# ipc-sim/IPC

Hardware: AMD Instinct MI355X
Metric: newton_iterations_per_sec (higher is better)
Workload: dtype f64

## Files before the change

### ipc_amd/csrc/hip_ipc.h

```cpp
#pragma once
#include "common.h"
#include "mf_numeric.h"
#include "mf_symbolic.h"
#include "nh_kernels.h"
#include "patch_assembly.h"
#include "hip_contact.h"
#include "hip_halfspace.h"
#include "pcg.h"
#include <map>
#include <memory>
#include <string>

struct ipcgpu_ctx;
typedef int (*ipcgpu_allreduce_fn_t)(void* user, void* buf_dev, long long count, int op);
typedef int (*ipcgpu_allreduce_stream_fn_t)(void* user, void* buf_dev, long long count, int op, void* hipStream);

namespace ipcgpu {

class HipMesh {
public:
    int nV = 0, nT = 0;
    int nElemNodes = 0;
    std::vector<double> V_rest;
    std::vector<int> F;
    std::vector<double> restTriInv;
    std::vector<double> triArea, mass, mu, lam;
    std::vector<int> dbcType;
    std::vector<int> nbPtr, nb;
    double avgEdgeLen = 0, bboxDiag2 = 0, bboxLo[3] = { 0, 0, 0 }, bboxHi[3] = { 0, 0, 0 };
    DevBuf<double> d_x, d_xTilde, d_mass, d_A, d_vol, d_mu, d_lam;
    DevBuf<int> d_dbc;
    DevBuf<int4> d_tet;

    unsigned featuresVersion = 0;
    void computeFeatures(int nV, int nT, const double* Vrest, const int* F, double YM, double PR, double density, hipStream_t s);
    std::vector<char> inMesh;
    void addSurfaceEdges(int nSF, const int* SF_colmajor, int nCE = 0, const int* CE_pairs = nullptr);
    void setCodimNodes(int n, const int* ids, const double* nodeMass, hipStream_t s);
    void meshBBox();
    void uploadDBC(hipStream_t s);
    int energyType = 0;
    double density = 0;
    void setComponentMaterial(int nodeBegin, int nodeEnd, int tetBegin, int tetEnd, double rho, double YM, double PR, hipStream_t s);
    bool isDBCVertex(int v) const { return dbcType[v] != 0; }
    bool isProjectDBCVertex(int v, bool projectDBC) const { return dbcType[v] == 1 || (dbcType[v] == 2 && projectDBC); }
};

class HipLinSysSolver {
public:
    explicit HipLinSysSolver(hipStream_t s);
    ~HipLinSysSolver();
    int numRows = 0;
    std::vector<int> ia, ja;
    DevBuf<int> d_ia, d_ja;
    DevBuf<double> d_a;
    DevBuf<double> hostDelta, hostSetVal;
    DevBuf<unsigned char> hostSetMask;
    std::vector<int> rowBase, rowLen;
    DevBuf<int> d_rowBase, d_rowLen, d_edgeP0;
    int solverType = 0;
    int patternVersion = 0;
    hipStream_t stream;

    void set_pattern(const HipMesh& mesh, int nExtra, const int* extraPairs);
    void set_pattern_csr(int nRows, const int* ia, const int* ja);
    void buildElementMap(const HipMesh& mesh);
    void setZero();
    int findEntry(int row, int col) const;
    void analyze_pattern(const HipMesh* meshForCoords);
    bool factorize();
    bool solve(const double* rhs_dev, double* x_dev);
    bool factorizeSolve(const double* rhs_dev, double* x_dev, bool wait = true);
    bool lastPivotsOk() const;
    bool lastSyncOk_ = true;
    void multiply(const double* x_dev, double* y_dev);
    void precondition_diag(const double* in_dev, double* out_dev);
    double pcgRelTol = 1e-5;
    int pcgMaxIter = 1000;
    int pcgPrecond = 0, pcgMaxFactorAge = 1;
    void setIterative(double relTol, int maxIter, int precond, int maxFactorAge);
    void iterStats(double* out6) const;
    void multiplySym(const double* x_dev, double* y_dev);
    int getNumRows() const { return numRows; }
    int getNumNonzeros() const { return (int)ja.size(); }
    const MfSymbolic& symbolic() const { return sym_; }
    void setShard(int rank, int world, ipcgpu_allreduce_fn_t fn, void* user, ipcgpu_allreduce_stream_fn_t sfn = nullptr, void* streamUser = nullptr)
    {
        num_.setShard(rank, world, fn, user, sfn, streamUser);
        analyzed_ = false;
    }
    void setHooks(ipcgpu_allreduce_fn_t fn, void* user, ipcgpu_allreduce_stream_fn_t sfn, void* streamUser) { num_.setHooks(fn, user, sfn, streamUser); }
    void setExchangeHooks(MfNumeric::ExchangeFn fn, void* user, MfNumeric::ExchangeStreamFn sfn, void* streamUser) { num_.setExchangeHooks(fn, user, sfn, streamUser); }
    bool hasExchangeHook() const { return num_.hasExchangeHook(); }
    int solverWorld() const { return num_.world(); }
    void setBulkTuning(double minMB, int block) { num_.setBulkTuning(minMB, block); }
    void entryDestinations(long long* out) const { num_.entryDestinations(out, ja.size()); }
    void nodeOwners(std::vector<int>& o) const { num_.nodeOwners(o); }
    long long exchangedBytes() const { return num_.exchangedBytes(); }
    long long exchangeCalls() const { return num_.exchangeCalls(); }
    long long sentBytes() const { return num_.sentBytes(); }
    long long receivedBytes() const { return num_.receivedBytes(); }
    double exchangeWaitMs() { return num_.exchangeWaitMs(); }
    void criticalPath(double* out5) const { num_.criticalPath(out5); }
    int analysisVersion = 0;
    double sharedFlopFraction() const { return num_.sharedFlopFraction(); }
    bool analyzed() const { return analyzed_; }
    void invalidateAnalysis() { analyzed_ = false; }

private:
    MfSymbolic sym_;
    MfNumeric num_;
    bool analyzed_ = false;
    std::unique_ptr<struct RocsolverCsrrf> rs_;
    PcgPattern pcgPat_;
    PcgWork pcgWork_;
    int pcgPatVersion_ = -1;
    void ensurePcgPattern();
    int runPcg(const double* rhs_dev, double* x_dev, PcgState& out);
    bool haveFactor_ = false, lastConverged_ = true;
    int factorAge_ = 0;
    long long nFactorizations_ = 0;
    struct {
        int iterations = 0, syncs = 0, factorAge = 0;
        double residual = 0.0;
        bool converged = false;
    } pcgLast_;
    friend struct RocsolverCsrrf;
};

class HipOptimizer {
public:
    HipOptimizer(HipMesh& mesh, HipLinSysSolver& lin, hipStream_t s);
    void init(double dt, bool withGravity);
    void setRelGL2Tol(double relTol);
    void setParameterScaling(bool absolute, double dTolRel, double kappaMinMultiplier);
    void setTwist(int nL, const int* left, int nR, const int* right, double angVel);
    void precompute();
    void beginTimestep();
    bool newtonIter();
    void endTimestep();
    int solveTimestep(int maxIter);

    double computeEnergyVal();
    void computeGradient(bool projectDBC);
    void penaltyGradientAdd(bool projectDBC);
    void computePrecondMtr(bool projectDBC, bool withGradient);
    double dampingStiff = 0.0;
    double ctorDt = 0.025;
    double dHatTargetEps = -1.0;
    double kappaConfig = 0.0;
    void setDamping(double stiff);
    void computeDampingMtr();
    void assembleDampingMtr();
    double dampingEnergy();
    void dampingGradientAdd(bool projectDBC, double* grad_dev);
    void computeSearchDir(bool projectDBC);
    void lineSearch(double& stepSize);
    void stepForward(const double* x0_dev, double alpha);
    double filterStepSize(const double* p_dev, double stepSize);
    double fullCcd(double slackness, double stepSize);
    bool checkInversion();
    ElemView view() const;

    HipMesh& mesh;
    HipLinSysSolver& lin;
    hipStream_t stream;
    double dt = 0.025, dtSq = 0, gravity[3] = { 0, 0, 0 };
    double relGL2Tol = 1e-8, targetGRes = 0;
    int timeIntegration = 0;
    int warmStart = 0;
    double warmStepSize = 0.0;
    double betaNM = 0.25, gammaNM = 0.5;
    DevBuf<double> d_acc, d_dxElastic;
    double elasticCoef() const { return timeIntegration == 1 ? dtSq * betaNM : dtSq; }
    void setTimeIntegration(int type, double beta, double gamma);
    void getKinematics(double* vel, double* acc, double* dxElastic);
    void getDbcState(double* out4) const;
    void saveStatus(const std::string& path);
    void loadStatus(const std::string& path);
    DevBuf<double> d_vel, d_xPrev, d_searchDir, d_gradient, d_minusG, d_x0, d_partial, d_scalar;
    DevBuf<double> d_damp, d_xDamp, d_zeroMass, d_dampDx, d_dampAdx;
    unsigned long long dampPatternVersion = ~0ULL;
    DevBuf<int> d_flag, d_handleIds;
    DevBuf<double> d_handleAng;
    int nHandles = 0;
    struct DbcGroup {
        std::vector<int> ids;
        DevBuf<int> d_ids;
        DevBuf<double> d_pos;
        double lin[3], ang[3], t0, t1;
        bool forceNonzero = false, hasCenter = false;
        double center[3] = { 0, 0, 0 };
        bool hasTargets = false;
        DevBuf<double> d_targets;
        bool isZero() const { return !forceNonzero && lin[0] == 0 && lin[1] == 0 && lin[2] == 0 && ang[0] == 0 && ang[1] == 0 && ang[2] == 0; }
    };
    std::vector<std::unique_ptr<DbcGroup>> dbcGroups;
    struct NbcGroup {
        int n = 0;
        DevBuf<int> d_ids;
        double a[3], t0, t1;
    };
    std::vector<std::unique_ptr<NbcGroup>> nbcGroups;
    void addNeumannBC(int n, const int* ids, const double* accel3, double t0, double t1);
    void neumannGradientAdd(double* grad_dev);
    double neumannEnergy();
    std::vector<int> baseDbcType;
    double stepStartTime = 0, stepEndTime = 0;
    std::vector<int> tpIds, tpIdsOnDevice;
    DevBuf<int> d_tpIds;
    DevBuf<double> d_tpPos, d_tpLam, d_tpStage;
    double dist2Tol = 0, completedStep = 1.0, lastMove = 1.0, rhoDBC = 0.0, CN_MBC = 0.0;
    bool projDBC = true;
    MdbcView mdbc() const { return MdbcView{ (int)tpIds.size(), d_tpIds.p, d_tpPos.p, d_tpLam.p, mesh.d_mass.p }; }
    void buildTargetPositions(bool deferTolerance = false);
    void finishTolerance();
    PinnedBuf<double> h_tpStage;
    bool tolPending = false;
    void initSubProblem();
    double computeCompletedStepSize();
    void dirichletPenaltyUpdate();
    void addDirichletBC(int n, const int* ids, const double* lin3, const double* angRad3, double t0, double t1);
    void setDBCVertices();
    bool dbcGroupMotion();
    double rotCenter[3] = { 0, 0, 0 };
    PinnedBuf<double> h_scalar;
    PinnedBuf<int> h_flag;
    int innerIterAmt = 0, globalIterNum = 0, k = 0;
    double lastEnergyVal = 0, lastStepSize = 0, lastAlphaFeasible = 0;
    double timers[16] = { 0 };
    bool initialised = false;
    int rank = 0, worldSize = 1;
    int tetBegin = 0, tetEnd = 0;
    ipcgpu_allreduce_fn_t allreduce = nullptr;
    ipcgpu_allreduce_stream_fn_t allreduceStream = nullptr;
    void hookReduce(double* dev, long long n, int op);
    bool fastPath() const;
    bool cachedDistValid = false, cachedE0Valid = false;
    double cachedDist = 0, cachedE0 = 0, cachedFilter = 0;
    bool cachedTrialValid = false, cachedTrialInverted = false;
    double cachedTrialE = 0, cachedAlpha = 1.0;
    DevBuf<double> d_aSpec, d_gradSpec;
    bool specAsmValid = false, specAsmOn = true;
    void speculativeAssembly();
    hipEvent_t evAsm0 = nullptr, evAsm1 = nullptr, evTail = nullptr;
    bool evAsmPending = false;
    int evAsmWeight = 1;
    unsigned asmLaunches = 0;
    void resolveEventTimers();
    DevBuf<double> d_contactG;
    void* allreduceUser = nullptr;
    void* allreduceStreamUser = nullptr;
    void reduceSum(double* dev, long long n);
    void reduceMin(double* dev, long long n);
    double readScalar(const double* dev);
    PatchPlan patch;
    int patchVersion = -1;
    void ensurePatchPlan();
    void patchShard(int& pb, int& pe) const;
    bool ownerMode() const;
    void ensureOwnerPlan();
    int ownerPlanPatch = -1, ownerPlanAnalysis = -1;
    int nOwnerPatches = 0;
    DevBuf<int> d_ownerPatches;
    DevBuf<unsigned char> d_need, d_mine;
    long long ownerNeededNodes = 0;
    bool matrixComplete = true;
    void maskAndReduceGradient(double* g);
    void completeMatrix();
    long long commBytes = 0, commCalls = 0;
    HipContact* contact = nullptr;
    bool selfCollision = false;
    double dHatEps = 1.0e-3, dHat = 0, kappa = 0, dTol = 0;
    bool absParameters = false;
    double dTolRel = 1.0e-9, kappaMinMultiplier = 1.0e11;
    double lenScale2() const { return absParameters ? 1.0 : mesh.bboxDiag2; }
    std::vector<std::pair<int, int>> curExtra;
    std::vector<std::array<int, 4>> closeID;
    std::vector<double> closeVal;
    int lastCCDPair[2] = { 0, 0 }, nFullCCD = 0, nPatternChanges = 0, dbcIncomplete = 0;
    unsigned long long coverSets = ~0ull;
    int coverPattern = -1;
    bool coverAnswer = false;
    double patternPad = -1.0;
    double lookahead() const { return patternPad >= 0.0 ? patternPad : (mesh.nV > 150000 ? 2.25 : 4.0); }
    std::vector<std::unique_ptr<HipHalfSpace>> planes;
    std::vector<std::pair<int, int>> closeHS;
    std::vector<double> closeHSVal;
    double selfFric = 0.0, epsV = 1.0e-3, fricDHat0 = 0, fricDHat = -1.0;
    double epsVTarget = -1.0, fricDHatTarget = 0;
    int fricIterAmt = 1, fricIterI = 0;
    bool fricLoopForced = false;
    bool solveFric() const;
    void updateFrictionLag();
    bool nextSubproblem();
    bool ipOn() const { return selfCollision || !planes.empty(); }
    size_t nConstraints() const;
    int addHalfSpace(HipContact* c, const double* origin3, const double* normal3, double dHatEps);
    bool anyIntersection();
    void elasticInertiaGradient(bool projectDBC, bool finish = true);
    void barrierGradientAdd(bool projectDBC, double kappa, bool activeOnly, double* grad_dev, int part = 0);
    void enableSelfCollision(HipContact* c, double dHatEps);
    void setVelocity(const double* vel3nV);
    void computeConstraintSets();
    double kappaFloor() const;
    void initKappa();
    void postLineSearch();
    bool isIntersected();
    void computeXTilta();
};

}

struct ipcgpu_ctx {
    int device = 0;
    hipStream_t stream = nullptr;
    std::unique_ptr<ipcgpu::HipMesh> mesh;
    std::unique_ptr<ipcgpu::HipLinSysSolver> lin;
    std::unique_ptr<ipcgpu::HipOptimizer> opt;
    std::unique_ptr<ipcgpu::HipContact> contact;
    int rank = 0, worldSize = 1;
    void* exchange = nullptr;
    void* exchangeUser = nullptr;
    void* exchangeStream = nullptr;
    void* exchangeStreamUser = nullptr;
};
```

### ipc_amd/csrc/hip_linsys.hip

```cpp
#include "hip_ipc.h"
#include <rocsolver/rocsolver.h>
#include <algorithm>
#include <cmath>
#include <thread>
#include <cstdlib>

namespace ipcgpu {

struct RocsolverCsrrf {
    rocblas_handle handle = nullptr;
    rocsolver_rfinfo info = nullptr;
    int n = 0, nnzA = 0, nnzT = 0;
    DevBuf<int> ptrA, indA, ptrT, indT, pivQ, trans, flag;
    DevBuf<double> valA, valT, B;
    bool analyzed = false;
    ~RocsolverCsrrf()
    {
        if (info) rocsolver_destroy_rfinfo(info);
        if (handle) rocblas_destroy_handle(handle);
    }
};

namespace {
__global__ void k_gather(int n, const int* __restrict__ map, const double* __restrict__ src, double* __restrict__ dst)
// ... 128 lines not shown
    analyzed_ = false;
    ++patternVersion;
}

void HipLinSysSolver::set_pattern_csr(int nRows, const int* ia_, const int* ja_)
{
    if (nRows <= 0 || nRows % 3) throw ArgError("set_pattern_csr: rows must be a positive multiple of 3");
    numRows = nRows;
    ia.assign(ia_, ia_ + nRows + 1);
    ja.assign(ja_, ja_ + ia[nRows]);
    for (int r = 0; r < nRows; ++r) {
        if (ia[r + 1] <= ia[r] || ja[ia[r]] != r) throw ArgError("set_pattern_csr: every row must start with its diagonal (upper CSR)");
        for (int k = ia[r] + 1; k < ia[r + 1]; ++k)
            if (ja[k] <= ja[k - 1] || ja[k] >= nRows) throw ArgError("set_pattern_csr: columns must be ascending and in range");
    }
    d_ia.upload(ia, stream);
    d_ja.upload(ja, stream);
    d_a.alloc(ja.size());
    d_a.zero(stream);
    rowBase.clear();
    rowLen.clear();
    HIP_CHECK(hipStreamSynchronize(stream));
    analyzed_ = false;
    ++patternVersion;
}

void HipLinSysSolver::setZero() { d_a.zeroN(ja.size(), stream); }

int HipLinSysSolver::findEntry(int row, int col) const
{
    if (row < 0 || row >= numRows) return -1;
    const int* b = ja.data() + ia[row];
    const int* e = ja.data() + ia[row + 1];
    const int* it = std::lower_bound(b, e, col);
    if (it == e || *it != col) return -1;
    return int(it - ja.data());
}

void HipLinSysSolver::analyze_pattern(const HipMesh* mesh)
{
    if (!numRows) throw StateError("analyze_pattern before set_pattern");
    std::vector<double> coords;
    const double* cptr = nullptr;
    if (mesh && 3 * mesh->nV == numRows) {
        coords.resize(3 * (size_t)mesh->nV);
        for (int v = 0; v < mesh->nV; ++v)
            for (int c = 0; c < 3; ++c) coords[3 * (size_t)v + c] = mesh->V_rest[v + (size_t)mesh->nV * c];
        cptr = coords.data();
    }
    if (solverType == 2) {
        if (num_.world() > 1) throw StateError("the iterative solver is not sharded");
        ensurePcgPattern();
        haveFactor_ = false;
        factorAge_ = 0;
        lastConverged_ = true;
        if (pcgPrecond == 0) {
            analyzed_ = true;
            return;
        }
    }
    const int leaf = 12;
    mf_analyze(numRows, ia.data(), ja.data(), cptr, leaf, sym_, false);
    ++analysisVersion;
    if (solverType == 0 || solverType == 2) {
        num_.setup(sym_, stream, d_ia.p, d_ja.p, (long long)ja.size());
    }
    else {
        rs_.reset(new RocsolverCsrrf);
        RocsolverCsrrf& R = *rs_;
        R.n = numRows;
        if (rocblas_create_handle(&R.handle) != rocblas_status_success) throw HipError("rocblas_create_handle");
        rocblas_set_stream(R.handle, stream);
        if (rocsolver_create_rfinfo(&R.info, R.handle) != rocblas_status_success) throw HipError("rocsolver_create_rfinfo");
        if (rocsolver_set_rfinfo_mode(R.info, rocsolver_rfinfo_mode_cholesky) != rocblas_status_success)
            throw HipError("rocsolver_set_rfinfo_mode");
        const int nnz = (int)ja.size();
        std::vector<int> ptr(numRows + 1, 0), ind(nnz), tr(nnz);
        for (int k = 0; k < nnz; ++k) ptr[ja[k] + 1]++;
        for (int r = 0; r < numRows; ++r) ptr[r + 1] += ptr[r];
        std::vector<int> pos(ptr.begin(), ptr.end() - 1);
        for (int r = 0; r < numRows; ++r)
            for (int k = ia[r]; k < ia[r + 1]; ++k) {
                const int c = ja[k];
                ind[pos[c]] = r;
                tr[pos[c]] = k;
                pos[c]++;
            }
        std::vector<int> pT, iT, q;
        mf_L_pattern_csr(sym_, pT, iT, q);
        R.nnzA = nnz;
        R.nnzT = (int)iT.size();
        R.ptrA.upload(ptr, stream);
        R.indA.upload(ind, stream);
        R.trans.upload(tr, stream);
        R.valA.alloc(nnz);
        R.ptrT.upload(pT, stream);
        R.indT.upload(iT, stream);
        R.pivQ.upload(q, stream);
        R.valT.alloc(iT.size());
        R.B.alloc(numRows);
        R.B.zero(stream);
        R.flag.alloc(1);
        hipLaunchKernelGGL(k_set_diag_one, dim3((numRows + 255) / 256), dim3(256), 0, stream, numRows, R.ptrT.p, R.indT.p, R.valT.p);
        hipLaunchKernelGGL(k_set_diag_one, dim3((numRows + 255) / 256), dim3(256), 0, stream, numRows, R.ptrA.p, R.indA.p, R.valA.p);
        const rocblas_status st = rocsolver_dcsrrf_analysis(R.handle, R.n, 1, R.nnzA, R.ptrA.p, R.indA.p, R.valA.p, R.nnzT, R.ptrT.p, R.indT.p, R.valT.p,
            nullptr, R.pivQ.p, R.B.p, R.n, R.info);
        if (st != rocblas_status_success) throw HipError("rocsolver_dcsrrf_analysis failed (rocblas_status " + std::to_string((int)st) + ")");
        HIP_CHECK(hipStreamSynchronize(stream));
        R.analyzed = true;
    }
    analyzed_ = true;
}

bool HipLinSysSolver::factorize()
{
    if (!analyzed_) throw StateError("factorize before analyze_pattern");
    if (solverType == 0) return num_.factorize(d_a.p);
    if (solverType == 2) {
        if (pcgPrecond == 0) {
            pcgWork_.ensure(numRows);
            pcgWork_.flag.zero(stream);
            launch_pcg_invert_blocks(pcgPat_, d_a.p, pcgWork_.flag.p, stream);
            int f = 0;
            pcgWork_.flag.download(&f, 1, stream);
            return f == 0;
        }
        if (haveFactor_ && lastConverged_ && factorAge_ + 1 < pcgMaxFactorAge) {
            ++factorAge_;
            return true;
        }
        ++nFactorizations_;
        haveFactor_ = num_.factorize(d_a.p);
        factorAge_ = 0;
        lastConverged_ = true;
        return haveFactor_;
    }
    RocsolverCsrrf& R = *rs_;
    hipLaunchKernelGGL(k_gather, dim3((R.nnzA + 255) / 256), dim3(256), 0, stream, R.nnzA, R.trans.p, d_a.p, R.valA.p);
    rocblas_status st = rocsolver_dcsrrf_refactchol(R.handle, R.n, R.nnzA, R.ptrA.p, R.indA.p, R.valA.p, R.nnzT, R.ptrT.p, R.indT.p,
        R.valT.p, R.pivQ.p, R.info);
    if (st != rocblas_status_success) {
        HIP_CHECK(hipStreamSynchronize(stream));
        return false;
    }
    R.flag.zero(stream);
    hipLaunchKernelGGL(k_check_diag, dim3((R.n + 255) / 256), dim3(256), 0, stream, R.n, R.ptrT.p, R.valT.p, R.pivQ.p, d_ia.p, d_a.p,
        R.flag.p);
    int f = 0;
    HIP_CHECK(hipMemcpyAsync(&f, R.flag.p, sizeof(int), hipMemcpyDeviceToHost, stream));
    HIP_CHECK(hipStreamSynchronize(stream));
    return f == 0;
}

bool HipLinSysSolver::factorizeSolve(const double* rhs_dev, double* x_dev, bool wait)
{
    if (!analyzed_) throw StateError("factorize before analyze_pattern");
    lastSyncOk_ = true;
    if (solverType == 0) return lastSyncOk_ = num_.factorizeSolve(d_a.p, rhs_dev, x_dev, wait);
    const bool ok = factorize();
    return lastSyncOk_ = ok && solve(rhs_dev, x_dev);
}
bool HipLinSysSolver::lastPivotsOk() const { return lastSyncOk_ && (solverType != 0 || num_.lastPivotsOk()); }

bool HipLinSysSolver::solve(const double* rhs_dev, double* x_dev)
{
    if (!analyzed_) throw StateError("solve before analyze_pattern");
    if (solverType == 0) {
        num_.solve(rhs_dev, x_dev);
        return true;
    }
    if (solverType == 2) {
        const bool jacobi = pcgPrecond == 0;
        if (!jacobi && !haveFactor_) throw StateError("solve before factorize");
        pcgLast_ = {};
        pcgLast_.factorAge = jacobi ? 0 : factorAge_;
        PcgState st;
        int status = runPcg(rhs_dev, x_dev, st);
        pcgLast_.iterations = st.iter;
        if (status == PCG_MAXITER && !jacobi && factorAge_ > 0) {
            ++nFactorizations_;
            haveFactor_ = num_.factorize(d_a.p);
            factorAge_ = 0;
            if (!haveFactor_) return false;
            pcgLast_.factorAge = 0;
            status = runPcg(rhs_dev, x_dev, st);
            pcgLast_.iterations += st.iter;
        }
        pcgLast_.residual = st.bb > 0.0 ? std::sqrt(st.trueRes2 / st.bb) : 0.0;
        pcgLast_.converged = status == PCG_CONVERGED && st.trueRes2 <= st.tol2;
        lastConverged_ = pcgLast_.converged;
        return status != PCG_BREAKDOWN;
    }
    RocsolverCsrrf& R = *rs_;
    HIP_CHECK(hipMemcpyAsync(x_dev, rhs_dev, sizeof(double) * R.n, hipMemcpyDeviceToDevice, stream));
    if (rocsolver_dcsrrf_solve(R.handle, R.n, 1, R.nnzT, R.ptrT.p, R.indT.p, R.valT.p, nullptr, R.pivQ.p, x_dev, R.n, R.info)
        != rocblas_status_success)
        throw HipError("rocsolver_dcsrrf_solve failed");
    return true;
}

void HipLinSysSolver::setIterative(double relTol, int maxIter, int precond, int maxFactorAge)
{
    if (!(relTol > 0.0) || maxIter < 1 || (precond != 0 && precond != 1) || maxFactorAge < 1)
        throw ArgError("set_iterative: rel_tol > 0, max_iter >= 1, precond 0 | 1, max_factor_age >= 1");
    if (precond != pcgPrecond && solverType == 2) analyzed_ = false;
    pcgRelTol = relTol;
    pcgMaxIter = maxIter;
    pcgPrecond = precond;
    pcgMaxFactorAge = maxFactorAge;
}

void HipLinSysSolver::iterStats(double* o) const
{
    o[0] = pcgLast_.iterations;
    o[1] = pcgLast_.residual;
    o[2] = pcgLast_.converged ? 1.0 : 0.0;
    o[3] = (double)nFactorizations_;
    o[4] = pcgLast_.factorAge;
    o[5] = pcgLast_.syncs;
}

void HipLinSysSolver::ensurePcgPattern()
{
    if (!numRows) throw StateError("no pattern");
    if (pcgPatVersion_ == patternVersion) return;
    pcgPat_.build(numRows, ia, ja, rowBase, rowLen, stream);
    pcgPatVersion_ = patternVersion;
}

void HipLinSysSolver::multiplySym(const double* x_dev, double* y_dev)
{
    ensurePcgPattern();
    launch_pcg_symv(pcgPat_, d_ia.p, d_ja.p, d_rowBase.p, d_rowLen.p, d_a.p, x_dev, nullptr, nullptr, 0, y_dev, nullptr, nullptr, 0, stream);
}

int HipLinSysSolver::runPcg(const double* rhs_dev, double* x_dev, PcgState& out)
{
    const bool jacobi = pcgPrecond == 0;
    PcgWork& W = pcgWork_;
    W.ensure(numRows);
    const int gAp = pcg_symv_grid(pcgPat_);
    double* p[2] = { W.p0.p, W.p1.p };
    int cur = 0, first = 1, restarts = 0, batch = jacobi ? 16 : 1;
    auto precondition = [&](int firstRz) {
        if (jacobi) return;
        num_.solve(W.r.p, W.z.p);
        launch_pcg_rz(numRows, W.r.p, W.z.p, W, firstRz, stream);
    };
    launch_pcg_begin(pcgPat_, jacobi, false, rhs_dev, nullptr, x_dev, W, pcgRelTol, pcgMaxIter, stream);
    precondition(1);
    for (;;) {
        for (int i = 0; i < batch; ++i) {
            launch_pcg_symv(pcgPat_, d_ia.p, d_ja.p, d_rowBase.p, d_rowLen.p, d_a.p, W.z.p, p[cur], p[1 - cur], first, W.Ap.p, W.partial.p, W.state.p, 1, stream);
            cur = 1 - cur;
            first = 0;
            launch_pcg_alpha(W, gAp, stream);
            launch_pcg_update(pcgPat_, jacobi, p[cur], W.Ap.p, x_dev, W, stream);
        }
        launch_pcg_symv(pcgPat_, d_ia.p, d_ja.p, d_rowBase.p, d_rowLen.p, d_a.p, x_dev, nullptr, nullptr, 0, W.Ap.p, nullptr, W.state.p, 2, stream);
        launch_pcg_residual(numRows, rhs_dev, W.Ap.p, W, stream);
        launch_pcg_publish(W, stream);
        HIP_CHECK(hipStreamSynchronize(stream));
        ++pcgLast_.syncs;
        out = *W.hState.p;
        if (out.done == PCG_RUNNING) {
            precondition(0);
            if (jacobi) batch = std::min(64, 2 * batch);
            continue;
        }
        if (out.done == PCG_CONVERGED && out.trueRes2 > out.tol2 && restarts < 3 && out.iter < out.maxIter) {
            ++restarts;
            launch_pcg_begin(pcgPat_, jacobi, true, rhs_dev, W.Ap.p, x_dev, W, pcgRelTol, pcgMaxIter, stream);
            first = 1;
            precondition(1);
            continue;
        }
        return out.done;
    }
}

void HipLinSysSolver::multiply(const double* x_dev, double* y_dev)
{
    launch_csr_symv(numRows, d_ia.p, d_ja.p, d_a.p, x_dev, y_dev, stream);
}
void HipLinSysSolver::precondition_diag(const double* in_dev, double* out_dev)
{
    launch_precond_diag(numRows, d_ia.p, d_a.p, in_dev, out_dev, stream);
}

}
```

### ipc_amd/csrc/hip_optimizer.cpp

```cpp
#include "hip_ipc.h"
#include <fstream>
#include <iomanip>
#include <limits>
#include <sstream>
#include <algorithm>
#include <chrono>
#include <thread>
#include <iterator>
#include <cmath>
#include <cstring>

#ifndef BEGIN_BATCHED
#define BEGIN_BATCHED 1
#endif

namespace ipcgpu {


namespace {
struct Tic {
    double& acc;
    hipStream_t s;
    std::chrono::high_resolution_clock::time_point t0;
    bool nosync = false;
    Tic(double& a, hipStream_t st) : acc(a), s(st), t0(std::chrono::high_resolution_clock::now()) {}
    ~Tic()
    {
        if (!nosync) (void)hipStreamSynchronize(s);
        acc += std::chrono::duration<double>(std::chrono::high_resolution_clock::now() - t0).count();
    }
};
}

HipOptimizer::HipOptimizer(HipMesh& m, HipLinSysSolver& l, hipStream_t s) : mesh(m), lin(l), stream(s) {}

ElemView HipOptimizer::view() const
{
    ElemView v;
    v.nV = mesh.nV;
    v.nT = mesh.nT;
    v.tetBegin = tetBegin;
    v.tetEnd = tetEnd;
    v.energyType = mesh.energyType;
    v.x = mesh.d_x.p;
    v.xTilde = mesh.d_xTilde.p;
    v.mass = mesh.d_mass.p;
    v.dbc = mesh.d_dbc.p;
    v.tet = mesh.d_tet.p;
    v.A = mesh.d_A.p;
    v.vol = mesh.d_vol.p;
    v.mu = mesh.d_mu.p;
    v.lam = mesh.d_lam.p;
    v.rowBase = lin.d_rowBase.p;
    v.rowLen = lin.d_rowLen.p;
    v.edgeP0 = lin.d_edgeP0.p;
    return v;
}

void HipOptimizer::init(double dt_, bool withGravity)
{
    dt = dt_;
    dtSq = dt * dt;
    gravity[0] = gravity[2] = 0.0;
    gravity[1] = withGravity ? -9.80665 : 0.0;
    const size_t n3 = 3 * (size_t)mesh.nV;
    d_vel.alloc(n3);
    d_vel.zero(stream);
    d_acc.alloc(n3);
    d_acc.zero(stream);
    d_dxElastic.alloc(n3);
    d_dxElastic.zero(stream);
    d_xPrev.alloc(n3);
    d_searchDir.alloc(n3);
    d_searchDir.zero(stream);
    d_gradient.alloc(n3);
    d_gradient.zero(stream);
    d_minusG.alloc(n3);
    d_x0.alloc(n3);
    d_partial.alloc((size_t)std::max(mesh.nT, mesh.nV) / 256 + 2);
    d_scalar.alloc(8);
    d_flag.alloc(2);
    h_scalar.alloc(8);
    h_flag.alloc(2);
    HIP_CHECK(hipMemcpyAsync(d_xPrev.p, mesh.d_x.p, n3 * sizeof(double), hipMemcpyDeviceToDevice, stream));
    HIP_CHECK(hipMemcpyAsync(mesh.d_xTilde.p, mesh.d_x.p, n3 * sizeof(double), hipMemcpyDeviceToDevice, stream));
    for (int c = 0; c < 3; ++c) rotCenter[c] = 0.5 * (mesh.bboxLo[c] + mesh.bboxHi[c]);
    tetBegin = (int)((long long)mesh.nT * rank / worldSize);
    tetEnd = (int)((long long)mesh.nT * (rank + 1) / worldSize);
    setRelGL2Tol(1.0e-2);
    innerIterAmt = globalIterNum = k = 0;
    std::memset(timers, 0, sizeof(timers));
    initialised = true;
    HIP_CHECK(hipStreamSynchronize(stream));
    computeXTilta();
}

void HipOptimizer::setRelGL2Tol(double relTol)
{
    relGL2Tol = relTol * relTol;
    targetGRes = std::sqrt(relGL2Tol * (absParameters ? 1.0 : mesh.bboxDiag2 * dtSq));
    CN_MBC = std::sqrt(1.0e-4 * mesh.bboxDiag2 * (ctorDt * ctorDt));
}

void HipOptimizer::setParameterScaling(bool absolute, double dTolRel_, double kappaMinMultiplier_)
{
    if (!(dTolRel_ > 0.0) || !(kappaMinMultiplier_ > 0.0)) throw ArgError("set_parameter_scaling: dTolRel and kappaMinMultiplier must be positive");
    absParameters = absolute;
    dTolRel = dTolRel_;
    kappaMinMultiplier = kappaMinMultiplier_;
    targetGRes = std::sqrt(relGL2Tol * (absParameters ? 1.0 : mesh.bboxDiag2 * dtSq));
    if (ipOn()) {
        dHat = dHatEps * dHatEps * lenScale2();
        dTol = dTolRel * dTolRel * lenScale2();
    }
}

void HipOptimizer::setTwist(int nL, const int* left, int nR, const int* right, double angVel)
{
    std::vector<int> ids;
    std::vector<double> ang;
    for (int i = 0; i < nL; ++i) {
        mesh.dbcType[left[i]] = 2;
        ids.push_back(left[i]);
        ang.push_back(-angVel * dt);
    }
    for (int i = 0; i < nR; ++i) {
        mesh.dbcType[right[i]] = 2;
        ids.push_back(right[i]);
        ang.push_back(angVel * dt);
    }
    nHandles = (int)ids.size();
    if (nHandles) {
        d_handleIds.upload(ids, stream);
        d_handleAng.upload(ang, stream);
    }
    mesh.uploadDBC(stream);
    if (initialised) computeXTilta();
}

void HipOptimizer::addNeumannBC(int n, const int* ids, const double* accel3, double t0, double t1)
{
    std::unique_ptr<NbcGroup> g(new NbcGroup);
    g->n = n;
    g->d_ids.upload(ids, (size_t)n, stream);
    for (int c = 0; c < 3; ++c) g->a[c] = accel3[c];
    g->t0 = t0;
    g->t1 = t1;
    HIP_CHECK(hipStreamSynchronize(stream));
    nbcGroups.push_back(std::move(g));
}

void HipOptimizer::neumannGradientAdd(double* grad_dev)
{
    for (const auto& g : nbcGroups) {
        if (stepStartTime < g->t0 || stepStartTime >= g->t1) continue;
        const double c[3] = { dtSq * g->a[0], dtSq * g->a[1], dtSq * g->a[2] };
        launch_nbc_gradient(g->n, g->d_ids.p, mesh.d_dbc.p, mesh.d_mass.p, c, grad_dev, stream);
    }
}

double HipOptimizer::neumannEnergy()
{
    double E = 0.0;
    for (const auto& g : nbcGroups) {
        if (stepStartTime < g->t0 || stepStartTime >= g->t1) continue;
        const double c[3] = { dtSq * g->a[0], dtSq * g->a[1], dtSq * g->a[2] };
        launch_nbc_energy(g->n, g->d_ids.p, mesh.d_dbc.p, mesh.d_mass.p, mesh.d_x.p, c, d_scalar.p + 5, stream);
        E -= readScalar(d_scalar.p + 5);
    }
    return E;
}

void HipOptimizer::addDirichletBC(int n, const int* ids, const double* lin3, const double* angRad3, double t0, double t1)
{
    std::unique_ptr<DbcGroup> g(new DbcGroup);
    g->ids.assign(ids, ids + n);
    for (int c = 0; c < 3; ++c) {
        g->lin[c] = lin3[c];
        g->ang[c] = angRad3[c];
    }
    g->t0 = t0;
    g->t1 = t1;
    g->d_ids.upload(g->ids, stream);
    g->d_pos.alloc(3 * (size_t)n);
    if (baseDbcType.empty()) baseDbcType = mesh.dbcType;
    dbcGroups.push_back(std::move(g));
    setDBCVertices();
    if (initialised) computeXTilta();
}

void HipOptimizer::setDBCVertices()
{
    if (dbcGroups.empty()) return;
    if (baseDbcType.empty()) baseDbcType = mesh.dbcType;
    std::vector<int> t = baseDbcType;
    for (const auto& g : dbcGroups) {
        if (stepStartTime < g->t0 || stepStartTime >= g->t1) continue;
        const int type = g->isZero() ? 1 : 2;
        for (int v : g->ids) t[v] = std::max(t[v], type);
    }
    if (t != mesh.dbcType) {
        mesh.dbcType = t;
        mesh.uploadDBC(stream);
    }
}

bool HipOptimizer::dbcGroupMotion()
{
    bool any = false;
    std::vector<double> pos;
    for (const auto& g : dbcGroups) {
        if (stepStartTime < g->t0 || stepStartTime >= g->t1 || g->ids.empty() || g->hasTargets) continue;
        const int n = (int)g->ids.size();
        launch_gather3(n, g->d_ids.p, mesh.d_x.p, g->d_pos.p, stream);
        pos.resize(3 * (size_t)n);
        g->d_pos.download(pos.data(), pos.size(), stream);
        HIP_CHECK(hipStreamSynchronize(stream));
        DbcMotion m;
        double lo[3] = { pos[0], pos[1], pos[2] }, hi[3] = { pos[0], pos[1], pos[2] };
        for (int i = 0; i < n; ++i)
            for (int c = 0; c < 3; ++c) {
                lo[c] = std::min(lo[c], pos[3 * (size_t)i + c]);
                hi[c] = std::max(hi[c], pos[3 * (size_t)i + c]);
            }
        for (int c = 0; c < 3; ++c) {
            m.c[c] = g->hasCenter ? g->center[c] : (lo[c] + hi[c]) / 2;
            m.linDt[c] = g->lin[c] * dt;
        }
        const double ax = g->ang[0] * dt, ay = g->ang[1] * dt, az = g->ang[2] * dt;
        const double cx = std::cos(ax), sx = std::sin(ax), cy = std::cos(ay), sy = std::sin(ay), cz = std::cos(az), sz = std::sin(az);
        const double Rx[9] = { 1, 0, 0, 0, cx, -sx, 0, sx, cx }, Ry[9] = { cy, 0, sy, 0, 1, 0, -sy, 0, cy }, Rz[9] = { cz, -sz, 0, sz, cz, 0, 0, 0, 1 };
        double T[9];
// ... 21 lines not shown
    if (worldSize > 1) hookReduce(dev, n, 1);
}
void HipOptimizer::hookReduce(double* dev, long long n, int op)
{
    commBytes += 8 * n;
    commCalls++;
    if (allreduceStream) {
        if (allreduceStream(allreduceStreamUser, dev, n, op, (void*)stream) != 0) throw HipError("all-reduce hook failed");
        return;
    }
    if (!allreduce) throw StateError("sharded context without an all-reduce hook");
    HIP_CHECK(hipStreamSynchronize(stream));
    if (allreduce(allreduceUser, dev, n, op) != 0) throw HipError("all-reduce hook failed");
}
double HipOptimizer::readScalar(const double* dev)
{
    launch_publish(dev, h_scalar.dev, 2, stream);
    HIP_CHECK(hipStreamSynchronize(stream));
    return h_scalar.p[0];
}

double HipOptimizer::computeEnergyVal()
{
    launch_energy(view(), elasticCoef(), true, rank == 0, d_partial.p, (int)d_partial.n, d_scalar.p, stream);
    reduceSum(d_scalar.p, 1);
    const bool contactQueued = selfCollision && contact->energyEnqueue(mesh.d_x.p, dHat, kappa, d_partial, d_scalar.p + 4, d_scalar.p, h_scalar.dev, 10);
    if (!(contactQueued && contact->publishedByEnergy())) launch_publish(d_scalar.p, h_scalar.dev, 10, stream);
    HIP_CHECK(hipStreamSynchronize(stream));
    double E = h_scalar.p[0];
    const double Econtact = contactQueued ? h_scalar.p[4] : 0.0;
    if (!nbcGroups.empty()) E += neumannEnergy();
    for (auto& h : planes) E += h->energy(mesh.d_x.p, dHat, kappa);
    if (selfCollision) E += Econtact;
    if (fricDHat > 0.0) {
        for (auto& h : planes)
            if (h->friction > 0.0) E += h->frictionEnergy(mesh.d_x.p, d_xPrev.p, fricDHat);
        if (selfCollision && selfFric > 0.0) E += contact->frictionEnergy(mesh.d_x.p, d_xPrev.p, fricDHat, selfFric, d_partial, d_scalar.p + 4);
    }
    if (dampingStiff > 0.0) E += dampingEnergy();
    if (rhoDBC && !tpIds.empty()) {
        launch_mdbc_reduce(mdbc(), mesh.d_x.p, rhoDBC, 0, d_scalar.p + 5, stream);
        E += readScalar(d_scalar.p + 5);
    }
    return E;
}

void HipOptimizer::setDamping(double stiff)
{
    dampingStiff = stiff > 0.0 ? stiff : 0.0;
}
void HipOptimizer::computeDampingMtr()
{
    if (!(dampingStiff > 0.0)) return;
    d_xDamp.ensure(3 * (size_t)mesh.nV);
    HIP_CHECK(hipMemcpyAsync(d_xDamp.p, mesh.d_x.p, sizeof(double) * 3 * (size_t)mesh.nV, hipMemcpyDeviceToDevice, stream));
    assembleDampingMtr();
}
void HipOptimizer::assembleDampingMtr()
{
    const size_t nnz = lin.ja.size();
    d_damp.ensure(nnz);
    if (d_zeroMass.n < (size_t)mesh.nV) {
        d_zeroMass.alloc(mesh.nV);
        d_zeroMass.zero(stream);
    }
    ensurePatchPlan();
    int pb, pe;
    patchShard(pb, pe);
    ElemView v = view();
    v.x = d_xDamp.p;
    v.xTilde = d_xDamp.p;
    v.mass = d_zeroMass.p;
    if (worldSize > 1) HIP_CHECK(hipMemsetAsync(d_damp.p, 0, sizeof(double) * nnz, stream));
    launch_assemble_patches(v, patch, pb, pe, dampingStiff / dt, 1, nullptr, d_damp.p, stream);
    if (worldSize > 1) reduceSum(d_damp.p, (long long)nnz);
    launch_damp_clear_diag(mesh.nV, mesh.d_dbc.p, lin.d_ia.p, d_damp.p, stream);
    dampPatternVersion = lin.patternVersion;
}
double HipOptimizer::dampingEnergy()
{
    if (dampPatternVersion != lin.patternVersion) assembleDampingMtr();
    const int n3 = 3 * mesh.nV;
    d_dampDx.ensure(n3);
    d_dampAdx.ensure(n3);
    launch_damp_dx(mesh.nV, mesh.d_dbc.p, 0, 1, mesh.d_x.p, d_xPrev.p, d_dampDx.p, stream);
    launch_csr_symv(n3, lin.d_ia.p, lin.d_ja.p, d_damp.p, d_dampDx.p, d_dampAdx.p, stream);
    launch_dot_scaled(n3, d_dampDx.p, d_dampAdx.p, 0.5, d_scalar.p + 6, stream);
    return readScalar(d_scalar.p + 6);
}
void HipOptimizer::dampingGradientAdd(bool projectDBC, double* grad_dev)
{
    if (dampPatternVersion != lin.patternVersion) assembleDampingMtr();
    const int n3 = 3 * mesh.nV;
    d_dampDx.ensure(n3);
    d_dampAdx.ensure(n3);
    launch_damp_dx(mesh.nV, mesh.d_dbc.p, 1, projectDBC ? 1 : 0, mesh.d_x.p, d_xPrev.p, d_dampDx.p, stream);
    launch_csr_symv(n3, lin.d_ia.p, lin.d_ja.p, d_damp.p, d_dampDx.p, d_dampAdx.p, stream);
    launch_axpy(n3, 1.0, d_dampAdx.p, grad_dev, stream);
}

bool HipOptimizer::solveFric() const
{
    if (fricLoopForced) return true;
    if (selfCollision && selfFric > 0.0) return true;
    for (const auto& h : planes)
        if (h->friction > 0.0) return true;
    return false;
}

void HipOptimizer::updateFrictionLag()
{
    if (!solveFric()) return;
    for (auto& h : planes)
        if (h->friction > 0.0) h->lagUpdate(mesh.d_x.p, dHat, kappa);
    if (selfCollision && selfFric > 0.0) contact->frictionLagUpdate(mesh.d_x.p, dHat, kappa);
}

bool HipOptimizer::nextSubproblem()
{
    specAsmValid = false;
    if (!ipOn()) return false;
    const double dHatTarget = dHatTargetEps > 0.0 ? dHatTargetEps * dHatTargetEps * lenScale2() : dHat;
    const bool fric = solveFric(), homotopy = dHat > dHatTarget;
    if (!fric && !homotopy) return false;
    fricIterI++;
    if (fric) updateFrictionLag();
    if (!nConstraints()) return false;
    bool updateDHat = true;
    {
        double dMax = 0.0, dMin = 1.0e300;
        std::vector<double> d;
        for (auto& h : planes) {
            h->evalDist2(h->set, mesh.d_x.p, d);
            for (size_t i = 0; i < h->set.size(); ++i) {
                dMax = std::max(dMax, d[i]);
                dMin = std::min(dMin, d[i]);
            }
        }
        if (selfCollision) {
            std::vector<std::array<int, 4>> ids;
            contact->closeStencils(mesh.d_x.p, 1.0e300, ids, d);
            for (size_t i = 0; i < ids.size(); ++i) {
                dMax = std::max(dMax, d[i]);
                dMin = std::min(dMin, d[i]);
            }
        }
        if (dMax < dHatTarget) updateDHat = false;
        else if (dMin < dTol) return false;
    }
    bool updateFricDHat = fric;
    if (fric && fricDHat <= fricDHatTarget) {
        computePrecondMtr(true, true);
        computeSearchDir(true);
        launch_fill(d_scalar.p + 3, 1, 0.0, stream);
        launch_max_abs(3 * mesh.nV, d_searchDir.p, d_scalar.p + 3, stream);
        if (readScalar(d_scalar.p + 3) < targetGRes) updateFricDHat = false;
        if (fricIterAmt > 0 && fricIterI >= fricIterAmt) updateFricDHat = false;
    }
    if (!updateDHat && !updateFricDHat) return false;
    if (updateDHat) {
        dHat = std::max(0.5 * dHat, dHatTarget);
        computeConstraintSets();
        initKappa();
    }
    if (updateFricDHat && fricDHat > 0.0) fricDHat = std::max(0.5 * fricDHat, fricDHatTarget);
    initSubProblem();
    closeID.clear();
    closeVal.clear();
    closeHS.clear();
    closeHSVal.clear();
    k = 0;
    return true;
}

size_t HipOptimizer::nConstraints() const
{
    size_t n = selfCollision ? (size_t)contact->nActive() : 0;
    for (const auto& h : planes) n += h->set.size();
    return n;
}

int HipOptimizer::addHalfSpace(HipContact* c, const double* origin3, const double* normal3, double eps)
{
    if (!c || !c->surfaceSet) throw StateError("opt_add_half_space before set_surface");
    if ((selfCollision || !planes.empty()) && eps != dHatEps) throw ArgError("all collision objects of a context share one dHat (Config.cpp:41-45): got a different dHatEps");
    contact = c;
    planes.emplace_back(new HipHalfSpace(stream, origin3, normal3));
    dHatEps = eps;
    dHat = eps * eps * lenScale2();
    dTol = dTolRel * dTolRel * lenScale2();
    return (int)planes.size() - 1;
}

bool HipOptimizer::anyIntersection()
{
    for (auto& h : planes)
        if (h->intersected(mesh.nV, mesh.d_x.p, mesh.d_dbc.p)) return true;
    return selfCollision && isIntersected();
}

void HipOptimizer::enableSelfCollision(HipContact* c, double eps)
{
    if (!c || !c->surfaceSet) throw StateError("opt_enable_self_collision before set_surface");
    if (!planes.empty() && eps != dHatEps) throw ArgError("all collision objects of a context share one dHat (Config.cpp:41-45): got a different dHatEps");
    contact = c;
    selfCollision = true;
    dHatEps = eps;
    dHat = eps * eps * lenScale2();
    dTol = dTolRel * dTolRel * lenScale2();
}

void HipOptimizer::computeXTilta()
{
    const size_t n3 = 3 * (size_t)mesh.nV;
    std::vector<double> xp(n3), vel(n3), xt(n3), acc(n3, 0.0);
    d_xPrev.download(xp.data(), n3, stream);
    d_vel.download(vel.data(), n3, stream);
    d_acc.download(acc.data(), n3, stream);
    for (int v = 0; v < mesh.nV; ++v)
        for (int c = 0; c < 3; ++c) {
            const size_t i = 3 * (size_t)v + c;
            if (mesh.isDBCVertex(v)) xt[i] = xp[i];
            else if (timeIntegration == 1) xt[i] = xp[i] + (vel[i] * dt + betaNM * (dtSq * gravity[c]) + (0.5 - betaNM) * (dtSq * acc[i]));
            else xt[i] = xp[i] + (vel[i] * dt + dtSq * gravity[c]);
        }
    mesh.d_xTilde.upload(xt, stream);
    HIP_CHECK(hipStreamSynchronize(stream));
}

void HipOptimizer::setTimeIntegration(int type, double beta, double gamma)
{
    timeIntegration = type;
    betaNM = beta;
    gammaNM = gamma;
    computeXTilta();
}

void HipOptimizer::getDbcState(double* out4) const
{
    out4[0] = completedStep;
    out4[1] = rhoDBC;
    out4[2] = projDBC ? 1.0 : 0.0;
    out4[3] = (double)tpIds.size();
}

void HipOptimizer::getKinematics(double* vel, double* acc, double* dxElastic)
{
    const size_t n3 = 3 * (size_t)mesh.nV;
    if (vel) d_vel.download(vel, n3, stream);
    if (acc) d_acc.download(acc, n3, stream);
    if (dxElastic) d_dxElastic.download(dxElastic, n3, stream);
    HIP_CHECK(hipStreamSynchronize(stream));
}

void HipOptimizer::saveStatus(const std::string& path)
{
    const size_t n3 = 3 * (size_t)mesh.nV;
    std::vector<double> x(n3), vel(n3), acc(n3), dx(n3);
    mesh.d_x.download(x.data(), n3, stream);
    getKinematics(vel.data(), acc.data(), dx.data());
    std::ofstream out(path, std::ios::out);
    if (!out.is_open()) throw StateError("unable to create status file " + path);
    out << std::setprecision(std::numeric_limits<long double>::digits10 + 2);
    out << "timestep " << globalIterNum << "\n\n";
    auto rows = [&](const char* name, const std::vector<double>& a) {
        out << name << " " << mesh.nV << " 3\n";
        for (int v = 0; v < mesh.nV; ++v) out << a[3 * (size_t)v] << " " << a[3 * (size_t)v + 1] << " " << a[3 * (size_t)v + 2] << "\n";
    };
    rows("position", x);
    out << "\n";
    out << "velocity " << n3 << "\n";
    for (size_t i = 0; i < n3; ++i) out << vel[i] << "\n";
    out << "\n";
    rows("acceleration", acc);
    out << "\n";
    rows("dx_Elastic", dx);
    if (!out.good()) throw StateError("write error on status file " + path);
}

void HipOptimizer::loadStatus(const std::string& path)
{
    specAsmValid = false;
    std::ifstream in(path);
    if (!in.is_open()) throw StateError("unable to open status file " + path);
    const size_t n3 = 3 * (size_t)mesh.nV;
    std::vector<double> x(n3), vel(n3, 0.0), acc(n3, 0.0), dx(n3, 0.0);
    mesh.d_x.download(x.data(), n3, stream);
    HIP_CHECK(hipStreamSynchronize(stream));
    auto readRows = [&](std::stringstream& ss, std::vector<double>& dst, bool zeroFirst) {
        int rowsIn = 0, dimIn = 0;
        ss >> rowsIn >> dimIn;
        if (rowsIn < 0 || rowsIn > mesh.nV || dimIn != 3) throw StateError("status file does not match the mesh");
        if (ss.fail()) throw StateError("malformed section header in status file " + path);
        if (zeroFirst) std::fill(dst.begin(), dst.end(), 0.0);
        for (int v = 0; v < rowsIn; ++v) in >> dst[3 * (size_t)v] >> dst[3 * (size_t)v + 1] >> dst[3 * (size_t)v + 2];
        if (in.fail()) throw StateError("truncated or malformed section in status file " + path);
    };
    std::string line;
    while (std::getline(in, line)) {
        std::stringstream ss(line);
        std::string token;
        ss >> token;
        if (token == "timestep") ss >> globalIterNum;
        else if (token == "position") readRows(ss, x, false);
        else if (token == "velocity") {
            long long n = 0;
            ss >> n;
// ... 276 lines not shown
        const auto now = std::chrono::steady_clock::now();
        fprintf(stderr, "pattern change: %-34s %.2f ms\n", what, std::chrono::duration<double, std::milli>(now - tLap).count());
        tLap = now;
    };
    const bool coverCached = selfCollision && coverSets == contact->setsVersion && coverPattern == lin.patternVersion;
    if (selfCollision && (frictionPairs || !(coverCached ? coverAnswer : contact->patternCovers(lin)))) {
        lap("coverage check");
        std::vector<std::pair<int, int>> extra, fresh;
        const bool liveOnHost = frictionPairs || lookahead() < 1.0;
        if (liveOnHost) {
            if (contact->nActive() + contact->nPara()) contact->connectivity(extra);
            if (fricDHat > 0.0 && selfFric > 0.0) contact->frictionConnectivity(extra);
            for (const auto& e : extra) {
                const int* b = mesh.nb.data() + mesh.nbPtr[e.first];
                const int* en = mesh.nb.data() + mesh.nbPtr[e.first + 1];
                if (!std::binary_search(b, en, e.second)) fresh.push_back(e);
            }
            std::sort(fresh.begin(), fresh.end());
            fresh.erase(std::unique(fresh.begin(), fresh.end()), fresh.end());
        }
        lap("connectivity of the live sets");
        if (!liveOnHost || !std::includes(curExtra.begin(), curExtra.end(), fresh.begin(), fresh.end())) {
            std::vector<std::pair<int, int>> padded = fresh;
            const double pad = lookahead();
            if (pad >= 1.0) {
                std::vector<std::pair<int, int>> ahead;
                if (pad > 1.0) contact->buildConstraintSet(mesh, mesh.d_x.p, mesh.d_dbc.p, pad * dHat);
                contact->candidateConnectivitySorted(ahead);
                if (pad > 1.0) contact->buildConstraintSet(mesh, mesh.d_x.p, mesh.d_dbc.p, dHat);
                std::vector<std::pair<int, int>> aheadNew;
                aheadNew.reserve(ahead.size());
                for (const auto& e : ahead) {
                    const int* b = mesh.nb.data() + mesh.nbPtr[e.first];
                    const int* en = mesh.nb.data() + mesh.nbPtr[e.first + 1];
                    if (!std::binary_search(b, en, e.second)) aheadNew.push_back(e);
                }
                padded.clear();
                std::set_union(fresh.begin(), fresh.end(), aheadNew.begin(), aheadNew.end(), std::back_inserter(padded));
            }
            lap("look-ahead sets + connectivity");
            std::vector<std::pair<int, int>> merged;
            std::set_union(curExtra.begin(), curExtra.end(), padded.begin(), padded.end(), std::back_inserter(merged));
            if (merged.size() > 3 * padded.size() + 4096) merged = padded;
            curExtra.swap(merged);
            nPatternChanges++;
            std::vector<int> flat;
            flat.reserve(2 * curExtra.size());
            for (const auto& e : curExtra) {
                flat.push_back(e.first);
                flat.push_back(e.second);
            }
            lap("union + flatten");
            {
                Tic t(timers[1], stream);
                lin.set_pattern(mesh, (int)curExtra.size(), flat.data());
            }
            lap("set_pattern");
            {
                int dev = 0;
                HIP_CHECK(hipGetDevice(&dev));
                std::exception_ptr planErr;
                std::thread planThread([&] {
                    try {
                        HIP_CHECK(hipSetDevice(dev));
                        ensurePatchPlan();
                    }
                    catch (...) {
                        planErr = std::current_exception();
                    }
                });
                std::exception_ptr anaErr;
                try {
                    Tic t(timers[2], stream);
                    lin.analyze_pattern(&mesh);
                }
                catch (...) {
                    anaErr = std::current_exception();
                }
                planThread.join();
                if (anaErr) std::rethrow_exception(anaErr);
                if (planErr) std::rethrow_exception(planErr);
            }
            lap("analyze_pattern + patch plan");
        }
    }
    const bool planStale = !(patchVersion == lin.patternVersion && patch.valid);
    ensurePatchPlan();
    if (planStale) lap("patch plan");
    if (ownerMode()) {
        ensureOwnerPlan();
        lin.setZero();
        if (withGradient) d_gradient.zero(stream);
        launch_assemble_patches(view(), patch, 0, nOwnerPatches, elasticCoef(), projectDBC, withGradient ? d_gradient.p : nullptr, lin.d_a.p, stream,
            d_ownerPatches.p);
        matrixComplete = false;
        if (ipOn() && selfCollision) contact->hessianAdd(mesh.d_x.p, mesh.d_dbc.p, lin, dHat, kappa, projectDBC, lin.d_a.p, d_need.p, true);
        if (withGradient) {
            if (ipOn()) barrierGradientAdd(projectDBC, kappa, false, d_gradient.p, 1);
            maskAndReduceGradient(d_gradient.p);
            neumannGradientAdd(d_gradient.p);
            if (ipOn()) barrierGradientAdd(projectDBC, kappa, false, d_gradient.p, 2);
        }
        if (ipOn()) {
            for (auto& h : planes)
                h->hessianAdd(mesh.d_x.p, mesh.d_dbc.p, lin.d_rowBase.p, lin.d_rowLen.p, dHat, kappa, projectDBC, lin.d_a.p);
            if (fricDHat > 0.0) {
                for (auto& h : planes)
                    if (h->friction > 0.0)
                        h->frictionHessianAdd(mesh.d_x.p, d_xPrev.p, mesh.d_dbc.p, lin.d_rowBase.p, lin.d_rowLen.p, fricDHat, projectDBC, lin.d_a.p);
                if (selfCollision && selfFric > 0.0)
                    contact->frictionHessianAdd(mesh.d_x.p, d_xPrev.p, mesh.d_dbc.p, lin, fricDHat, selfFric, projectDBC, lin.d_a.p);
            }
        }
        if (withGradient) penaltyGradientAdd(projectDBC);
        if (!projectDBC && rhoDBC && !tpIds.empty()) launch_mdbc_hessian(mdbc(), lin.d_ia.p, rhoDBC, lin.d_a.p, stream);
        return;
    }
    int pb, pe;
    patchShard(pb, pe);
    if (worldSize > 1) {
        lin.setZero();
        if (withGradient) d_gradient.zero(stream);
    }
    launch_assemble_patches(view(), patch, pb, pe, elasticCoef(), projectDBC, withGradient ? d_gradient.p : nullptr,
        lin.d_a.p, stream);
    matrixComplete = true;
    const bool contactSharded = false;
    if (worldSize > 1) {
        reduceSum(lin.d_a.p, (long long)lin.ja.size());
        if (withGradient) reduceSum(d_gradient.p, 3LL * mesh.nV);
    }
    if (withGradient) neumannGradientAdd(d_gradient.p);
    if (ipOn()) {
        if (withGradient) barrierGradientAdd(projectDBC, kappa, false, d_gradient.p);
        for (auto& h : planes)
            h->hessianAdd(mesh.d_x.p, mesh.d_dbc.p, lin.d_rowBase.p, lin.d_rowLen.p, dHat, kappa, projectDBC, lin.d_a.p);
        if (selfCollision && !contactSharded) contact->hessianAdd(mesh.d_x.p, mesh.d_dbc.p, lin, dHat, kappa, projectDBC, lin.d_a.p, nullptr, true);
        if (fricDHat > 0.0) {
            for (auto& h : planes)
                if (h->friction > 0.0)
                    h->frictionHessianAdd(mesh.d_x.p, d_xPrev.p, mesh.d_dbc.p, lin.d_rowBase.p, lin.d_rowLen.p, fricDHat, projectDBC, lin.d_a.p);
            if (selfCollision && selfFric > 0.0)
                contact->frictionHessianAdd(mesh.d_x.p, d_xPrev.p, mesh.d_dbc.p, lin, fricDHat, selfFric, projectDBC, lin.d_a.p);
        }
    }
    if (dampingStiff > 0.0) {
        if (dampPatternVersion != lin.patternVersion) assembleDampingMtr();
        launch_axpy((long long)lin.ja.size(), 1.0, d_damp.p, lin.d_a.p, stream);
    }
    if (withGradient) penaltyGradientAdd(projectDBC);
    if (!projectDBC && rhoDBC && !tpIds.empty()) launch_mdbc_hessian(mdbc(), lin.d_ia.p, rhoDBC, lin.d_a.p, stream);
}

bool HipOptimizer::checkInversion()
{
    if (mesh.energyType == 1) return true;
    d_flag.zero(stream);
    launch_check_inversion(view(), d_flag.p, stream);
    launch_publish(d_flag.p, h_flag.dev, 1, stream);
    HIP_CHECK(hipStreamSynchronize(stream));
    int f = h_flag.p[0];
    if (worldSize > 1) {
        h_scalar.p[1] = (double)f;
        HIP_CHECK(hipMemcpyAsync(d_scalar.p + 1, h_scalar.p + 1, sizeof(double), hipMemcpyHostToDevice, stream));
        reduceSum(d_scalar.p + 1, 1);
        f = readScalar(d_scalar.p + 1) != 0.0;
    }
    return f == 0;
}

double HipOptimizer::fullCcd(double slackness, double stepSize)
{
    if (contact->ccdMode == 1) {
        int arg3[3];
        const double a = contact->ccdFullReference(mesh, mesh.d_x.p, d_searchDir.p, mesh.d_dbc.p, slackness, stepSize, nullptr, arg3, nullptr);
        lastCCDPair[0] = arg3[1];
        lastCCDPair[1] = arg3[2];
        return a;
    }
    return contact->ccdFull(mesh, mesh.d_x.p, d_searchDir.p, mesh.d_dbc.p, slackness, stepSize, lastCCDPair, nullptr);
}

double HipOptimizer::filterStepSize(const double* p_dev, double stepSize)
{
    if (mesh.energyType == 1) return stepSize;
    launch_fill(d_scalar.p + 2, 1, 1e20, stream);
    launch_inversion_step(view(), p_dev, 0.2, stepSize, d_scalar.p + 2, stream);
    reduceMin(d_scalar.p + 2, 1);
    const double t = readScalar(d_scalar.p + 2);
    if (t > 0.0 && t < stepSize) stepSize = t;
    return stepSize;
}

void HipOptimizer::stepForward(const double* x0_dev, double alpha)
{
    launch_step_forward(3 * mesh.nV, x0_dev, d_searchDir.p, alpha, mesh.d_x.p, stream);
}

#ifndef ASM_TIME_EVERY
#define ASM_TIME_EVERY 8
#endif
void HipOptimizer::speculativeAssembly()
{
    specAsmValid = false;
    if (!specAsmOn || !fastPath() || !projDBC || lin.rowBase.empty()) return;
    ensurePatchPlan();
    d_aSpec.alloc(lin.d_a.n);
    d_gradSpec.alloc(d_gradient.n);
    const bool timeIt = (asmLaunches++ % ASM_TIME_EVERY) == 0;
    if (timeIt) {
        resolveEventTimers();
        HIP_CHECK(hipEventRecord(evAsm0, stream));
    }
    launch_assemble_patches(view(), patch, 0, patch.nPatches, elasticCoef(), 1, d_gradSpec.p, d_aSpec.p, stream);
    if (timeIt) {
        HIP_CHECK(hipEventRecord(evAsm1, stream));
        evAsmPending = true;
        evAsmWeight = ASM_TIME_EVERY;
    }
    specAsmValid = true;
}

void HipOptimizer::computeSearchDir(bool projectDBC)
{
    (void)projectDBC;
    bool ok;
    const bool twoCalls = false;
    launch_negate(3 * mesh.nV, d_gradient.p, d_minusG.p, stream);
    const bool noSpec = false;
    cachedTrialValid = false;
    cachedDistValid = false;
    if (fastPath() && !twoCalls && !noSpec) {
        Tic t(timers[3], stream);
        const size_t bytes = 3 * (size_t)mesh.nV * sizeof(double);
        if (lin.factorizeSolve(d_minusG.p, d_searchDir.p, false)) {
            launch_iter_reset(d_scalar.p, d_flag.p, stream);
            launch_max_abs(3 * mesh.nV, d_searchDir.p, d_scalar.p + 3, stream);
            if (mesh.energyType != 1) launch_inversion_step(view(), d_searchDir.p, 0.2, 1.0, d_scalar.p + 2, stream);
            launch_energy(view(), elasticCoef(), true, true, d_partial.p, (int)d_partial.n, d_scalar.p, stream);
            launch_trial_step_fused(3 * mesh.nV, mesh.d_x.p, d_x0.p, d_searchDir.p, d_scalar.p + 2, mesh.energyType != 1, d_scalar.p + 6, stream);
            if (mesh.energyType != 1) launch_check_inversion(view(), d_flag.p, stream);
            launch_energy(view(), elasticCoef(), true, true, d_partial.p, (int)d_partial.n, d_scalar.p + 1, stream);
            launch_publish2(d_flag.p, h_flag.dev, 1, d_scalar.p, h_scalar.dev, 14, stream);
            if (!evTail) HIP_CHECK(hipEventCreateWithFlags(&evTail, hipEventDisableTiming));
            HIP_CHECK(hipEventRecord(evTail, stream));
            speculativeAssembly();
            HIP_CHECK(hipEventSynchronize(evTail));
            t.nosync = specAsmValid;
            if (lin.lastPivotsOk()) {
                cachedE0 = h_scalar.p[0];
                cachedTrialE = h_scalar.p[1];
                cachedFilter = h_scalar.p[2];
                cachedDist = h_scalar.p[3];
                cachedAlpha = h_scalar.p[6];
                cachedTrialInverted = mesh.energyType != 1 && h_flag.p[0] != 0;
                cachedDistValid = cachedE0Valid = cachedTrialValid = true;
                return;
            }
            HIP_CHECK(hipMemcpyAsync(mesh.d_x.p, d_x0.p, bytes, hipMemcpyDeviceToDevice, stream));
            specAsmValid = false;
            t.nosync = false;
        }
        ok = false;
    }
    else {
        Tic t(timers[3], stream);
        if (twoCalls) ok = lin.factorize();
        else if (worldSize == 1) {
            ok = lin.factorizeSolve(d_minusG.p, d_searchDir.p, false);
            if (ok) {
                launch_fill(d_scalar.p + 3, 1, 0.0, stream);
                launch_max_abs(3 * mesh.nV, d_searchDir.p, d_scalar.p + 3, stream);
                launch_publish(d_scalar.p + 3, h_scalar.dev + 3, 2, stream);
                HIP_CHECK(hipStreamSynchronize(stream));
                ok = lin.lastPivotsOk();
                if (ok) {
                    cachedDist = h_scalar.p[3];
                    cachedDistValid = true;
                }
            }
        }
        else ok = lin.factorizeSolve(d_minusG.p, d_searchDir.p);
    }
    Tic t(timers[4], stream);
    if (!ok) {
        completeMatrix();
        lin.precondition_diag(d_minusG.p, d_searchDir.p);
    }
    else if (twoCalls) lin.solve(d_minusG.p, d_searchDir.p);
    if (fastPath()) {
        launch_fill(d_scalar.p + 3, 1, 0.0, stream);
        launch_max_abs(3 * mesh.nV, d_searchDir.p, d_scalar.p + 3, stream);
        launch_fill(d_scalar.p + 2, 1, 1e20, stream);
        if (mesh.energyType != 1) launch_inversion_step(view(), d_searchDir.p, 0.2, 1.0, d_scalar.p + 2, stream);
        launch_energy(view(), elasticCoef(), true, true, d_partial.p, (int)d_partial.n, d_scalar.p, stream);
        launch_publish(d_scalar.p, h_scalar.dev, 8, stream);
        HIP_CHECK(hipStreamSynchronize(stream));
        cachedE0 = h_scalar.p[0];
        cachedFilter = h_scalar.p[2];
        cachedDist = h_scalar.p[3];
        cachedDistValid = cachedE0Valid = true;
    }
    else {
        if (!cachedDistValid) {
            launch_fill(d_scalar.p + 3, 1, 0.0, stream);
            launch_max_abs(3 * mesh.nV, d_searchDir.p, d_scalar.p + 3, stream);
            launch_publish(d_scalar.p + 3, h_scalar.dev + 3, 2, stream);
            HIP_CHECK(hipStreamSynchronize(stream));
            cachedDist = h_scalar.p[3];
            cachedDistValid = true;
        }
        if (selfCollision) contact->takeHessianError();
    }
}

bool HipOptimizer::fastPath() const
{
    return worldSize == 1 && !ipOn() && nbcGroups.empty() && !(dampingStiff > 0.0) && !(rhoDBC && !tpIds.empty()) && lin.solverType != 2;
}

void HipOptimizer::resolveEventTimers()
{
    if (!evAsmPending) return;
    HIP_CHECK(hipEventSynchronize(evAsm1));
    float ms = 0.0f;
    HIP_CHECK(hipEventElapsedTime(&ms, evAsm0, evAsm1));
    timers[0] += 1.0e-3 * (double)ms * evAsmWeight;
    evAsmPending = false;
}

void HipOptimizer::lineSearch(double& stepSize)
{
    const size_t bytes = 3 * (size_t)mesh.nV * sizeof(double);
    if (cachedTrialValid && fastPath()) {
        cachedTrialValid = cachedE0Valid = false;
        lastEnergyVal = cachedE0;
        if (!cachedTrialInverted && !(cachedTrialE > lastEnergyVal)) {
            lastEnergyVal = cachedTrialE;
            return;
        }
        HIP_CHECK(hipMemcpyAsync(mesh.d_x.p, d_x0.p, bytes, hipMemcpyDeviceToDevice, stream));
        specAsmValid = false;
    }
    else if (cachedE0Valid && fastPath()) {
        cachedE0Valid = false;
        lastEnergyVal = cachedE0;
        bool done = false;
        double testingE = 0.0;
        {
            Tic t(timers[5], stream);
            HIP_CHECK(hipMemcpyAsync(d_x0.p, mesh.d_x.p, bytes, hipMemcpyDeviceToDevice, stream));
            stepForward(d_x0.p, stepSize);
            int inverted = 0;
            if (mesh.energyType != 1) {
                d_flag.zero(stream);
                launch_check_inversion(view(), d_flag.p, stream);
                launch_publish(d_flag.p, h_flag.dev, 1, stream);
            }
            launch_energy(view(), elasticCoef(), true, true, d_partial.p, (int)d_partial.n, d_scalar.p, stream);
            launch_publish(d_scalar.p, h_scalar.dev, 2, stream);
            HIP_CHECK(hipStreamSynchronize(stream));
            if (mesh.energyType != 1) inverted = h_flag.p[0];
            testingE = h_scalar.p[0];
            done = !inverted && !(testingE > lastEnergyVal);
        }
        if (done) {
            lastEnergyVal = testingE;
            return;
        }
        HIP_CHECK(hipMemcpyAsync(mesh.d_x.p, d_x0.p, bytes, hipMemcpyDeviceToDevice, stream));
    }
    {
        Tic t(timers[9], stream);
        lastEnergyVal = computeEnergyVal();
    }
    {
        Tic t(timers[5], stream);
        HIP_CHECK(hipMemcpyAsync(d_x0.p, mesh.d_x.p, bytes, hipMemcpyDeviceToDevice, stream));
        stepForward(d_x0.p, stepSize);
        while (!checkInversion()) {
            stepSize /= 2.0;
            if (stepSize == 0.0) break;
            stepForward(d_x0.p, stepSize);
        }
        if (ipOn())
            while (anyIntersection()) {
                stepSize /= 2.0;
                stepForward(d_x0.p, stepSize);
            }
    }
    computeConstraintSets();
    double testingE;
    {
        Tic t(timers[9], stream);
        testingE = computeEnergyVal();
    }
    const double LFStepSize = stepSize;
    while (testingE > lastEnergyVal && stepSize > 0.0) {
        stepSize /= 2.0;
        if (stepSize == 0.0) break;
        {
            Tic t(timers[5], stream);
            stepForward(d_x0.p, stepSize);
        }
        computeConstraintSets();
        Tic t(timers[9], stream);
        testingE = computeEnergyVal();
    }
    if (stepSize < LFStepSize && ipOn()) {
        bool needRecomputeCS = false;
        while (anyIntersection()) {
            stepSize /= 2.0;
            stepForward(d_x0.p, stepSize);
            needRecomputeCS = true;
        }
        if (needRecomputeCS) computeConstraintSets();
    }
    lastEnergyVal = testingE;
}

void HipOptimizer::precompute()
{
    specAsmValid = false;
    if (!initialised) throw StateError("opt_precompute before opt_init");
    if (anyIntersection()) throw StateError("intersection detected in initial configuration");
    {
        Tic t(timers[1], stream);
        lin.set_pattern(mesh, 0, nullptr);
        curExtra.clear();
    }
    computeConstraintSets();
    computeDampingMtr();
    {
        Tic t(timers[0], stream);
        computePrecondMtr(true, false);
    }
    if (!lin.analyzed()) {
        Tic t(timers[2], stream);
        lin.analyze_pattern(&mesh);
    }
    lastEnergyVal = computeEnergyVal();
}

void HipOptimizer::beginTimestep()
{
    specAsmValid = false;
    if (!initialised) throw StateError("opt_begin_timestep before opt_init");
    if (!lin.analyzed()) throw StateError("opt_begin_timestep before opt_precompute");
    Tic t(timers[11], stream);
    const bool batched = BEGIN_BATCHED && fastPath() && nHandles && dbcGroups.empty() && !selfCollision && planes.empty() && !(warmStart >= 1 && warmStart <= 5);
    if (batched) {
        const bool guard = mesh.energyType != 1;
        d_flag.zero(stream);
        if (guard) launch_check_inversion(view(), d_flag.p, stream);
        d_searchDir.zero(stream);
        stepStartTime = stepEndTime;
        stepEndTime += dt;
        setDBCVertices();
        launch_twist_dir(nHandles, d_handleIds.p, d_handleAng.p, rotCenter[1], rotCenter[2], mesh.d_x.p, d_searchDir.p, stream);
        buildTargetPositions(true);
        launch_fill(d_scalar.p + 2, 1, 1e20, stream);
        if (guard) launch_inversion_step(view(), d_searchDir.p, 0.2, 1.0, d_scalar.p + 2, stream);
        launch_trial_step_fused(3 * mesh.nV, mesh.d_x.p, d_x0.p, d_searchDir.p, d_scalar.p + 2, guard, d_scalar.p + 6, stream);
        if (guard) launch_check_inversion(view(), d_flag.p + 1, stream);
        launch_energy(view(), elasticCoef(), true, true, d_partial.p, (int)d_partial.n, d_scalar.p, stream);
        launch_publish2(d_flag.p, h_flag.dev, 2, d_scalar.p, h_scalar.dev, 14, stream);
        HIP_CHECK(hipStreamSynchronize(stream));
        if (h_flag.p[0]) throw StateError("element inversion before scripted motion (Optimizer.cpp:517-522)");
        finishTolerance();
        double stepSize = h_scalar.p[6];
        bool energyKnown = true;
        if (h_flag.p[1]) {
            energyKnown = false;
            do {
                stepSize /= 2.0;
                stepForward(d_x0.p, stepSize);
            } while (!checkInversion());
        }
        if (stepSize < 1.0) dbcIncomplete++;
        completedStep = stepSize;
        d_searchDir.zero(stream);
        initSubProblem();
        lastEnergyVal = energyKnown ? h_scalar.p[0] : computeEnergyVal();
        k = 0;
        return;
    }
    if (!checkInversion()) throw StateError("element inversion before scripted motion (Optimizer.cpp:517-522)");
    d_searchDir.zero(stream);
    stepStartTime = stepEndTime;
    stepEndTime += dt;
    setDBCVertices();
    if (nHandles) launch_twist_dir(nHandles, d_handleIds.p, d_handleAng.p, rotCenter[1], rotCenter[2], mesh.d_x.p, d_searchDir.p, stream);
    const bool groupMotion = dbcGroupMotion();
    buildTargetPositions();
    completedStep = 1.0;
    if (nHandles || groupMotion) {
        double stepSize = filterStepSize(d_searchDir.p, 1.0);
        if (selfCollision)
            stepSize = fullCcd(0.5, stepSize);
        HIP_CHECK(hipMemcpyAsync(d_x0.p, mesh.d_x.p, 3 * (size_t)mesh.nV * sizeof(double), hipMemcpyDeviceToDevice, stream));
        stepForward(d_x0.p, stepSize);
        while (!checkInversion()) {
            stepSize /= 2.0;
            stepForward(d_x0.p, stepSize);
        }
        if (ipOn())
            while (anyIntersection()) {
                stepSize /= 2.0;
                stepForward(d_x0.p, stepSize);
            }
        if (stepSize < 1.0) dbcIncomplete++;
        completedStep = stepSize;
        d_searchDir.zero(stream);
    }
    if (warmStart >= 1 && warmStart <= 5) {
        if (warmStart == 5) {
            computeGradient(true);
            computePrecondMtr(false, false);
            launch_negate(3 * mesh.nV, d_gradient.p, d_minusG.p, stream);
            completeMatrix();
            lin.precondition_diag(d_minusG.p, d_searchDir.p);
            launch_clear_projected(mesh.nV, mesh.d_dbc.p, 1, d_searchDir.p, stream);
        }
        else {
        static const double CG[2][5] = { { 0, 0, 1, 1, 1 }, { 0, 0, 0.5, 0.5, 0.5 } }, CE[2][5] = { { 0, 0, 0, 1, 0.5 }, { 0, 0, 0, 2, 1 } };
        const double cg = CG[timeIntegration][warmStart], ce = CE[timeIntegration][warmStart];
        const double g3[3] = { cg * (dtSq * gravity[0]), cg * (dtSq * gravity[1]), cg * (dtSq * gravity[2]) };
        launch_warm_dir(mesh.nV, mesh.d_dbc.p, d_vel.p, d_dxElastic.p, dt, g3, ce, d_searchDir.p, stream);
        }
        double stepSize = filterStepSize(d_searchDir.p, 1.0);
        if (ipOn()) {
            for (auto& h : planes) stepSize = h->stepBound(contact->nSVI, contact->d_SVI.p, mesh.d_x.p, mesh.d_dbc.p, d_searchDir.p, 0.9, stepSize);
            if (selfCollision) stepSize = fullCcd(0.8, stepSize);
        }
        HIP_CHECK(hipMemcpyAsync(d_x0.p, mesh.d_x.p, 3 * (size_t)mesh.nV * sizeof(double), hipMemcpyDeviceToDevice, stream));
        stepForward(d_x0.p, stepSize);
        while (!checkInversion()) {
            stepSize /= 2.0;
            stepForward(d_x0.p, stepSize);
        }
        if (ipOn())
            while (anyIntersection()) {
                stepSize /= 2.0;
                stepForward(d_x0.p, stepSize);
            }
        warmStepSize = stepSize;
    }
    if (ipOn()) {
        dHat = dHatEps * dHatEps * lenScale2();
        computeConstraintSets();
        kappa = kappaConfig > 0.0 ? std::min(kappaConfig, 100 * kappaFloor()) : kappaFloor();
        initKappa();
        closeHS.clear();
        closeHSVal.clear();
        closeID.clear();
        closeVal.clear();
        if (contact) contact->frictionLagClear();
        for (auto& h : planes) h->lagClear();
        fricDHat0 = epsV * epsV * (ctorDt * ctorDt) * lenScale2();
        fricDHatTarget = epsVTarget > 0.0 ? epsVTarget * epsVTarget * (ctorDt * ctorDt) * lenScale2() : fricDHat0;
        fricDHat = solveFric() ? fricDHat0 : -1.0;
        fricIterI = 0;
        updateFrictionLag();
    }
    initSubProblem();
    lastEnergyVal = computeEnergyVal();
    k = 0;
}

void HipOptimizer::initSubProblem()
{
    specAsmValid = false;
    projDBC = true;
    rhoDBC = 0.0;
    lastMove = completedStep;
}

void HipOptimizer::buildTargetPositions(bool deferTolerance)
{
    tpIds.clear();
    for (int v = 0; v < mesh.nV; ++v)
        if (mesh.dbcType[v] != 0) tpIds.push_back(v);
    dist2Tol = 0.0;
    tolPending = false;
    if (tpIds.empty()) return;
    const int n = (int)tpIds.size();
    if (tpIds != tpIdsOnDevice) {
        d_tpIds.uploadGrow(tpIds, stream);
        tpIdsOnDevice = tpIds;
    }
    d_tpPos.ensure(3 * (size_t)n);
    d_tpLam.ensure(3 * (size_t)n);
    d_tpLam.zeroN(3 * (size_t)n, stream);
    if (h_tpStage.n < 3 * (size_t)n) h_tpStage.alloc(3 * (size_t)n + 3 * (size_t)n / 2 + 16);
    d_tpStage.ensure(3 * (size_t)n);
    launch_target_positions(n, d_tpIds.p, mesh.d_x.p, d_searchDir.p, d_tpPos.p, d_tpStage.p, stream);
    HIP_CHECK(hipMemcpyAsync(h_tpStage.p, d_tpStage.p, 3 * (size_t)n * sizeof(double), hipMemcpyDeviceToHost, stream));
    tolPending = true;
    if (!deferTolerance) {
        HIP_CHECK(hipStreamSynchronize(stream));
        finishTolerance();
    }
}

void HipOptimizer::finishTolerance()
{
    if (!tolPending) return;
    tolPending = false;
    double sq = 0.0;
    for (size_t i = 0, m = 3 * tpIds.size(); i < m; ++i) sq += h_tpStage.p[i] * h_tpStage.p[i];
    dist2Tol = sq * 1.0e-6;
}

double HipOptimizer::computeCompletedStepSize()
{
    if (dist2Tol == 0.0 || tpIds.empty()) return completedStep = 1.0;
    launch_mdbc_reduce(mdbc(), mesh.d_x.p, 0.0, 1, d_scalar.p + 5, stream);
    const double sqNorm = readScalar(d_scalar.p + 5);
    return completedStep = 1.0 - std::sqrt(sqNorm / (dist2Tol * 1.0e6));
}

void HipOptimizer::dirichletPenaltyUpdate()
{
    if (projDBC) {
        if (completedStep < 1.0 - 1.0e-3) {
            projDBC = false;
            rhoDBC = 1.0e6;
        }
        return;
    }
    const double completed = computeCompletedStepSize();
    if (completed > 1.0 - 1.0e-3) projDBC = true;
    else if (completed < lastMove && rhoDBC < 1.0e8) rhoDBC *= 2.0;
    else {
        launch_fill(d_scalar.p + 3, 1, 0.0, stream);
        launch_max_abs(3 * mesh.nV, d_searchDir.p, d_scalar.p + 3, stream);
        if (readScalar(d_scalar.p + 3) < CN_MBC) {
            if (completed < 0.99 && rhoDBC < 1.0e8) rhoDBC *= 2.0;
            else launch_mdbc_lambda(mdbc(), mesh.d_x.p, rhoDBC, stream);
        }
    }
}

bool HipOptimizer::newtonIter()
{
    double distToOpt_PN;
    if (k && cachedDistValid) distToOpt_PN = cachedDist;
    else if (k) {
        launch_fill(d_scalar.p + 3, 1, 0.0, stream);
        launch_max_abs(3 * mesh.nV, d_searchDir.p, d_scalar.p + 3, stream);
        distToOpt_PN = readScalar(d_scalar.p + 3);
    }
    else distToOpt_PN = 0.0;
    cachedDistValid = false;
    if (k && distToOpt_PN < targetGRes && completedStep > 1.0 - 1.0e-3) {
        specAsmValid = false;
        Tic t(timers[12], stream);
        t.nosync = fastPath();
        computeGradient(projDBC);
        return true;
    }
    innerIterAmt++;
    if (fastPath()) {
        if (!evAsm0) {
            HIP_CHECK(hipEventCreate(&evAsm0));
            HIP_CHECK(hipEventCreate(&evAsm1));
        }
        if (specAsmValid && projDBC && d_aSpec.n == lin.d_a.n && d_gradSpec.n == d_gradient.n) {
            std::swap(lin.d_a.p, d_aSpec.p);
            std::swap(d_gradient.p, d_gradSpec.p);
            matrixComplete = true;
        }
        else {
            resolveEventTimers();
            HIP_CHECK(hipEventRecord(evAsm0, stream));
            computePrecondMtr(projDBC, true);
            HIP_CHECK(hipEventRecord(evAsm1, stream));
            evAsmPending = true;
            evAsmWeight = 1;
        }
        specAsmValid = false;
    }
    else {
        specAsmValid = false;
        Tic t(timers[0], stream);
        computePrecondMtr(projDBC, true);
    }
    cachedE0Valid = false;
    computeSearchDir(projDBC);
    double alpha = 1.0;
    {
        Tic t(timers[13], stream);
        t.nosync = specAsmValid && cachedTrialValid;
        const bool batchedBounds = !cachedTrialValid && !cachedE0Valid && selfCollision && planes.empty() && worldSize == 1;
        if (cachedTrialValid) alpha = cachedAlpha;
        else if (cachedE0Valid) {
            if (mesh.energyType != 1 && cachedFilter > 0.0 && cachedFilter < alpha) alpha = cachedFilter;
        }
        else if (!batchedBounds)
        alpha = filterStepSize(d_searchDir.p, alpha);
        for (auto& h : planes)
            alpha = h->stepBound(contact->nSVI, contact->d_SVI.p, mesh.d_x.p, mesh.d_dbc.p, d_searchDir.p, 0.9, alpha);
        if (selfCollision) {
            const double slackness_m = 0.8;
            double pMax;
            if (batchedBounds) {
                const bool filter = mesh.energyType != 1;
                if (filter) {
                    launch_fill(d_scalar.p + 2, 1, 1e20, stream);
                    launch_inversion_step(view(), d_searchDir.p, 0.2, alpha, d_scalar.p + 2, stream);
                }
                contact->stepBounds(mesh.d_x.p, d_searchDir.p, slackness_m, alpha, filter ? d_scalar.p + 2 : nullptr, &alpha, lastCCDPair, &pMax);
            }
            else {
                alpha = contact->ccdPartial(mesh.d_x.p, d_searchDir.p, slackness_m, alpha, lastCCDPair);
                pMax = contact->maxSurfaceSpeed(d_searchDir.p);
            }
            const double alpha_CFL = std::sqrt(dHat) / (pMax * 2.0);
            if ((!k && alpha > alpha_CFL) || alpha > 2.0 * alpha_CFL) {
                alpha = fullCcd(slackness_m, alpha);
                nFullCCD++;
                if (alpha < alpha_CFL) alpha = alpha_CFL;
            }
            else alpha = std::min(alpha, alpha_CFL);
        }
    }
    lastAlphaFeasible = alpha;
    lineSearch(alpha);
    lastStepSize = alpha;
    postLineSearch();
    dirichletPenaltyUpdate();
    ++k;
    return false;
}

void HipOptimizer::endTimestep()
{
    specAsmValid = false;
    Tic t(timers[11], stream);
    t.nosync = fastPath();
    if (timeIntegration == 1)
        launch_nm_update(mesh.nV, mesh.d_dbc.p, mesh.d_x.p, d_xPrev.p, d_vel.p, d_acc.p, d_dxElastic.p, mesh.d_xTilde.p, dt, betaNM, gammaNM,
            gravity[0], gravity[1], gravity[2], stream);
    else
        launch_be_update(mesh.nV, mesh.d_dbc.p, mesh.d_x.p, d_xPrev.p, d_vel.p, d_acc.p, d_dxElastic.p, mesh.d_xTilde.p, dt, gravity[0],
            gravity[1], gravity[2], stream);
    computeDampingMtr();
    globalIterNum++;
}

int HipOptimizer::solveTimestep(int maxIter)
{
    beginTimestep();
    int it = 0;
    for (;;) {
        while (it < maxIter) {
            if (newtonIter()) break;
            ++it;
        }
        if (it >= maxIter || !nextSubproblem()) break;
    }
    endTimestep();
    return it;
}

}
```

### ipc_amd/csrc/mf_numeric.h

```cpp
#pragma once
#include "common.h"
#include "mf_plan.h"
#include "mf_symbolic.h"

namespace ipcgpu {

class MfNumeric {
public:
    MfNumeric() = default;
    ~MfNumeric();
    MfNumeric(const MfNumeric&) = delete;
    MfNumeric& operator=(const MfNumeric&) = delete;

    void setup(const MfSymbolic& sym, hipStream_t stream, const int* ia_dev, const int* ja_dev, long long nnzPattern);
    typedef int (*AllreduceFn)(void* user, void* buf_dev, long long count, int op);
    typedef int (*AllreduceStreamFn)(void* user, void* buf_dev, long long count, int op, void* hipStream);
    struct P2POp {
        void* buf_dev;
        long long count;
        int peer;
        int send;
    };
    typedef int (*ExchangeFn)(void* user, int nOps, const P2POp* ops);
    typedef int (*ExchangeStreamFn)(void* user, int nOps, const P2POp* ops, void* hipStream);
    void setShard(int rank, int world, AllreduceFn fn, void* user, AllreduceStreamFn sfn = nullptr, void* streamUser = nullptr)
    {
        rank_ = rank;
        world_ = world;
        setHooks(fn, user, sfn, streamUser);
    }
    void setBulkTuning(double minMB, int block)
    {
        tune_.bulkMinMB = minMB;
        tune_.bulkBlock = block < 64 ? 64 : (block / 32) * 32;
    }
    void setExchangeHooks(ExchangeFn fn, void* user, ExchangeStreamFn sfn, void* streamUser)
    {
        exchange_ = fn;
        exchangeUser_ = user;
        exchangeStream_ = sfn;
        exchangeStreamUser_ = streamUser;
    }
    bool hasExchangeHook() const { return exchange_ || exchangeStream_; }
    void setHooks(AllreduceFn fn, void* user, AllreduceStreamFn sfn, void* streamUser)
    {
        allreduce_ = fn;
        allreduceUser_ = user;
        allreduceStream_ = sfn;
        allreduceStreamUser_ = streamUser;
    }
    int world() const { return world_; }
    void nodeOwners(std::vector<int>& ownerOfNode) const;
    long long exchangedBytes() const { return commBytes_; }
    long long exchangeCalls() const { return commCalls_; }
    long long sentBytes() const { return sentBytes_; }
    long long receivedBytes() const { return recvBytes_; }
    double exchangeWaitMs();
    void criticalPath(double* out5) const;
    double sharedFlopFraction() const { return mp_.sharedFlops; }
    bool factorize(const double* a_dev);
    void solve(const double* rhs_dev, double* x_dev);
    bool factorizeSolve(const double* a_dev, const double* rhs_dev, double* x_dev, bool wait = true);
    bool lastPivotsOk() const { return pivotsOk(); }
    bool pivotsOk() const;
    bool ready() const { return ns_ > 0; }
    void entryDestinations(long long* out, size_t nnz) const { entryDst_.download(out, nnz, stream_); }
    size_t front_bytes() const { return fronts_.n * sizeof(double); }

private:
    void enqueueFactor(const double* a_dev, bool overlapForward = false);
    void enqueueSolve(const double* rhs_dev, double* x_dev);
    typedef MfRange Range;
    typedef MfLevelPlan LevelPlan;
    typedef MfXinvLevel XinvLevel;
    int rank_ = 0, world_ = 1;
    MfPlanTuning tune_;
    MfPlan mp_;
    AllreduceFn allreduce_ = nullptr;
    AllreduceStreamFn allreduceStream_ = nullptr;
    void* allreduceUser_ = nullptr;
    void* allreduceStreamUser_ = nullptr;
    ExchangeFn exchange_ = nullptr;
    ExchangeStreamFn exchangeStream_ = nullptr;
    void* exchangeUser_ = nullptr;
    void* exchangeStreamUser_ = nullptr;
    long long commBytes_ = 0, commCalls_ = 0, sentBytes_ = 0, recvBytes_ = 0;
    double waitMs_ = 0.0;
    std::vector<std::pair<hipEvent_t, hipEvent_t>> waitPending_, waitFree_;
    struct Xchg {
        std::vector<P2POp> opsM, opsW, opsX;
    };
    std::vector<Xchg> xchg_;
    DevBuf<int4> xchgDesc_;
    DevBuf<double> xchgBuf_;
    DevBuf<int> nodeExec_;
    void allreduceSum(double* dev, long long count);
    void exchange(const std::vector<P2POp>& ops);
    void exchangeUpdateMatrices(int level);
    void exchangeUpdateVectors(int level);
    void reduceSolution();
    void allreduceFlag();
    void configureSweepKernels(size_t maxSolveLds, size_t maxBwdLds, size_t maxTriLds);
    void enqueuePermuteRhs(const double* rhs_dev, hipStream_t st);
    const MfSymbolic* sym_ = nullptr;
    hipStream_t stream_ = nullptr;
    int ns_ = 0, nLevels_ = 0;
    DevBuf<double> fronts_, w_, yperm_, bperm_, xsol_;
    DevBuf<double> xinvX_, xinvT_;
    DevBuf<long long> xinvOff_;
    DevBuf<int4> xinvDesc_;
    DevBuf<int> triList_;
    hipStream_t side_ = nullptr;
    int fwdStride_ = 4;
    bool fwdJoined_ = false;
    hipStream_t fwd_ = nullptr;
    hipEvent_t evRhs_ = nullptr, evFwdDone_ = nullptr;
    std::vector<hipEvent_t> evFactLevel_;
    void enqueueForwardLevel(int l, hipStream_t st);
    void enqueueBackward(double* x_dev);
    hipEvent_t evSide_ = nullptr;
    std::vector<hipEvent_t> evLevel_, evInvDone_;
    bool sidePending_ = false;
    void enqueueInverses(int level, hipStream_t st);
    DevBuf<double> dinv_;
    DevBuf<int> idx_, idxPtr_, firstNode_, childPtr_, child_, invPtr_, inv_, newOf_, flag_;
    DevBuf<long long> frontOff_, wOff_, dinvOff_;
    DevBuf<int> aSrc_, aLoc_;
    DevBuf<double> aPerm_;
    int nFusedA_ = 0;
    DevBuf<int> bigFd_;
    DevBuf<int> fdesc_;
    DevBuf<int> bigASrc_;
    DevBuf<long long> bigADst_;
    DevBuf<long long> entryDst_;
    DevBuf<int> entryBucket_, bucketHist_, bucketStart_, nodeFront_;
    DevBuf<int4> frontInfo_;
    DevBuf<int> eaAPtr_;
    DevBuf<int4> eaDesc_;
    DevBuf<int> smallList_, bigList_;
    DevBuf<int4> desc_;
    PinnedBuf<int> hflag_;
};

}
```

### ipc_amd/csrc/mf_numeric.hip

```cpp
#include <climits>
#include "mf_kernels.h"
#include <algorithm>
#include <chrono>
#include <cstdio>
#include <cstdlib>
#include <cstring>
#include <thread>

namespace ipcgpu {

namespace {

__global__ void k_publish_flag(const int* __restrict__ flag, int* __restrict__ mapped) { mapped[0] = flag[0]; }

__global__ void k_gather_a(int cnt, const int* __restrict__ src, const double* __restrict__ a, double* __restrict__ aP, int* __restrict__ flag)
{
    int k = blockIdx.x * blockDim.x + threadIdx.x;
    if (k == 0) flag[0] = 0;
    if (k < cnt) aP[k] = a[src[k]];
}


struct EntryView {
    const int *ia, *ja;
// ... 1314 lines not shown
    sidePending_ = false;

    auto planning = [](auto&& step) {
        try {
            step();
        }
        catch (const MfPlanError& e) {
            throw StateError(e.what());
        }
    };
    mp_.rank = rank_;
    mp_.world = world_;
    mp_.tune = tune_;
    planning([&] { mf_plan_fronts(sym, mp_); });
    dinvOff_.upload(mp_.dinvOff, stream);
    dinv_.alloc((size_t)mp_.dinvOff[ns_] * NB * NB);
    const size_t nnz = (size_t)nnzPattern;
    const int nBuckets = ns_ + mp_.nEaTiles;
    uploadRecs(frontInfo_, mp_.frontInfo, stream);
    nodeFront_.upload(mp_.nodeFront, stream);
    entryDst_.ensure(nnz + 1);
    entryBucket_.ensure(nnz + 1);
    bucketHist_.ensure(2 * (size_t)nBuckets + 2);
    bucketStart_.ensure((size_t)nBuckets + 2);
    bucketHist_.zeroN(2 * (size_t)nBuckets + 2, stream);
    EntryView ev{ ia_dev, ja_dev, sym.n, ns_, newOf_.p, nodeFront_.p, firstNode_.p, idxPtr_.p, idx_.p, frontOff_.p, frontInfo_.p };
    hipLaunchKernelGGL(k_entry_dst, dim3((sym.n + 3) / 4), dim3(256), 0, stream, ev, entryDst_.p, entryBucket_.p, bucketHist_.p);
    hipLaunchKernelGGL(k_scan_exclusive, dim3(1), dim3(1024), 0, stream, nBuckets, bucketHist_.p, bucketStart_.p);
    std::vector<int> start((size_t)nBuckets + 1);
    bucketStart_.download(start.data(), start.size(), stream);
    const size_t nFused = (size_t)start[ns_], nBig = (size_t)(start[nBuckets] - start[ns_]);
    nFusedA_ = (int)nFused;
    aPerm_.ensure(std::max<size_t>(nFused, 1));
    aSrc_.ensure(nFused + 1);
    aLoc_.ensure(nFused + 1);
    bigASrc_.ensure(nBig + 1);
    bigADst_.ensure(nBig + 1);
    if (nnz)
        hipLaunchKernelGGL(k_entry_scatter, dim3((unsigned)((nnz + 255) / 256)), dim3(256), 0, stream, (int)nnz, ns_, entryDst_.p, entryBucket_.p, bucketStart_.p,
            bucketHist_.p + nBuckets + 1, frontOff_.p, aSrc_.p, aLoc_.p, bigASrc_.p, bigADst_.p);
    lap("A-entry lists");
    planning([&] { mf_plan_launches(sym, start.data(), mp_); });
    lap("level plans");
    eaAPtr_.upload(mp_.eaAPtr, stream);
    fdesc_.uploadGrow(mp_.fdesc, stream);
    lap("fused descriptors");
    triList_.upload(mp_.triList, stream);
    uploadRecs(xinvDesc_, mp_.xinvDesc, stream);
    xinvOff_.upload(mp_.xinvOff, stream);
    xinvX_.alloc((size_t)std::max<long long>(mp_.xTot, 1));
    xinvT_.alloc((size_t)std::max<long long>(mp_.xTot, 1));
    xinvX_.zero(stream);
    xinvT_.zero(stream);
    lap("inverse plan + buffers");
    smallList_.upload(mp_.smallList, stream);
    bigList_.upload(mp_.bigList, stream);
    uploadRecs(eaDesc_, mp_.ea, stream);
    bigFd_.uploadGrow(mp_.bigFd, stream);
    uploadRecs(desc_, mp_.desc, stream);
    if (world_ > 1) {
        xchgBuf_.ensure((size_t)mp_.xchgStaging + 1);
        uploadRecs(xchgDesc_, mp_.xchgDesc, stream);
        nodeExec_.upload(mp_.nodeExec, stream);
        auto resolve = [](const std::vector<MfXchgOp>& ops, double* base, std::vector<P2POp>& out) {
            for (const MfXchgOp& o : ops) out.push_back(P2POp{ base + o.off, o.count, o.peer, o.send });
        };
        xchg_.assign(nLevels_, Xchg());
        for (int l = 0; l < nLevels_; ++l) {
            resolve(mp_.xchg[l].opsM, xchgBuf_.p, xchg_[l].opsM);
            resolve(mp_.xchg[l].opsW, xchgBuf_.p, xchg_[l].opsW);
            resolve(mp_.xchg[l].opsX, xsol_.p, xchg_[l].opsX);
        }
    }
    if (mp_.maxSmallLds > 48 * 1024) {
        HIP_CHECK(hipFuncSetAttribute((const void*)k_front_fused<256>, hipFuncAttributeMaxDynamicSharedMemorySize, (int)mp_.maxSmallLds));
        HIP_CHECK(hipFuncSetAttribute((const void*)k_front_fused<512>, hipFuncAttributeMaxDynamicSharedMemorySize, (int)mp_.maxSmallLds));
    }
    configureSweepKernels(mp_.maxSolveLds, mp_.maxBwdLds, mp_.maxTriLds);
    HIP_CHECK(hipStreamSynchronize(stream));
    lap("uploads + attributes");
}

void MfNumeric::nodeOwners(std::vector<int>& ownerOfNode) const
{
    if (!sym_) throw StateError("nodeOwners before analyze_pattern");
    const MfSymbolic& sym = *sym_;
    ownerOfNode.assign(sym.nn, -1);
    if (world_ <= 1) return;
    std::vector<int> perm(sym.nn, -1);
    for (int s = 0; s < ns_; ++s)
        for (int v = sym.firstNode[s]; v < sym.firstNode[s + 1]; ++v) perm[v] = mp_.owner[s];
    for (int v = 0; v < sym.nn; ++v) ownerOfNode[v] = perm[sym.newOf[v]];
}

MfNumeric::~MfNumeric()
{
    if (side_) (void)hipStreamSynchronize(side_);
    if (fwd_) (void)hipStreamSynchronize(fwd_);
    for (hipEvent_t e : evFactLevel_) (void)hipEventDestroy(e);
    if (evRhs_) (void)hipEventDestroy(evRhs_);
    if (evFwdDone_) (void)hipEventDestroy(evFwdDone_);
    if (fwd_) (void)hipStreamDestroy(fwd_);
    for (hipEvent_t e : evLevel_) (void)hipEventDestroy(e);
    for (hipEvent_t e : evInvDone_) (void)hipEventDestroy(e);
    if (evSide_) (void)hipEventDestroy(evSide_);
    if (side_) (void)hipStreamDestroy(side_);
}

bool MfNumeric::factorize(const double* a_dev)
{
    if (!sym_) throw StateError("factorize before analyze_pattern");
    enqueueFactor(a_dev);
    if (world_ > 1) {
        allreduceFlag();
    }
    hipLaunchKernelGGL(k_publish_flag, dim3(1), dim3(1), 0, stream_, flag_.p, hflag_.dev);
    HIP_CHECK(hipStreamSynchronize(stream_));
#ifdef MF_FUSED_PROBE
    {
        static int calls = 0;
        if (++calls == 3) {
            std::vector<unsigned long long> h(16 << 16);
            HIP_CHECK(hipMemcpyFromSymbol(h.data(), HIP_SYMBOL(g_probe), h.size() * sizeof(unsigned long long)));
            const char* names[7] = { "maps", "children", "A", "panels", "store", "schur", "total" };
            for (int l = 0; l < nLevels_; ++l) {
                const LevelPlan& P = mp_.level[l];
                if (!P.small.cnt) continue;
                double sum[16] = { 0 }, mx = 0;
                for (int b = 0; b < P.small.cnt; ++b) {
                    const unsigned long long* r = h.data() + 16 * (size_t)((P.small.off + b) & 0xffff);
                    for (int k = 0; k < 6; ++k) sum[k] += (double)(r[k + 1] - r[k]);
                    sum[6] += (double)(r[6] - r[0]);
                    mx = std::max(mx, (double)(r[6] - r[0]));
                    for (int k = 8; k < 16; ++k) sum[k] += (double)r[k];
                }
                const double c = 0.01 / P.small.cnt;
                std::fprintf(stderr, "[fused probe] level %d: %d fronts, %d threads, N %.0f nc %.0f kids %.1f |", l, P.small.cnt, P.smallThreads, sum[12] / P.small.cnt, sum[13] / P.small.cnt,
                    sum[14] / P.small.cnt);
                for (int k = 0; k < 7; ++k) std::fprintf(stderr, " %s %.2f", names[k], sum[k] * c);
                std::fprintf(stderr, " us (max %.2f) | inside panels: pivot %.2f rows %.2f trailing %.2f | inside schur (wave 0): gathers %.2f products + stores %.2f\n", mx * 0.01, sum[8] * c, sum[9] * c,
                    sum[10] * c, sum[11] * c, sum[15] * c);
            }
        }
    }
#endif
    return pivotsOk();
}

bool MfNumeric::pivotsOk() const
{
    return hflag_.p[0] == 0;
}

bool MfNumeric::factorizeSolve(const double* a_dev, const double* rhs_dev, double* x_dev, bool wait)
{
    if (!sym_) throw StateError("factorize before analyze_pattern");
    if (world_ > 1 || !fwd_) {
        const bool ok = factorize(a_dev);
        if (ok) solve(rhs_dev, x_dev);
        return ok;
    }
    HIP_CHECK(hipEventRecord(evRhs_, stream_));
    HIP_CHECK(hipStreamWaitEvent(fwd_, evRhs_, 0));
    enqueuePermuteRhs(rhs_dev, fwd_);
    fwdJoined_ = false;
    enqueueFactor(a_dev, true);
    if (!fwdJoined_) HIP_CHECK(hipEventRecord(evFwdDone_, fwd_));
    hipLaunchKernelGGL(k_publish_flag, dim3(1), dim3(1), 0, stream_, flag_.p, hflag_.dev);
    if (!fwdJoined_) HIP_CHECK(hipStreamWaitEvent(stream_, evFwdDone_, 0));
    enqueueBackward(x_dev);
    if (!wait) return true;
    HIP_CHECK(hipStreamSynchronize(stream_));
    return pivotsOk();
}

void MfNumeric::enqueueFactor(const double* a_dev, bool overlapForward)
{
    TreeView tv{ frontOff_.p, idxPtr_.p, firstNode_.p, childPtr_.p, child_.p, invPtr_.p, inv_.p, idx_.p, dinvOff_.p };
    XinvView xvF{ xinvOff_.p, xinvX_.p, xinvT_.p };
    if (sidePending_) HIP_CHECK(hipStreamWaitEvent(stream_, evSide_, 0));
    bool sideUsed = false;
    int fwdNext = 0;
#ifdef MF_FUSED_PROBE
    {
        const int* base = fdesc_.p;
        HIP_CHECK(hipMemcpyToSymbolAsync(HIP_SYMBOL(g_probeBase), &base, sizeof(base), 0, hipMemcpyHostToDevice, stream_));
    }
#endif
    if (nFusedA_) hipLaunchKernelGGL(k_gather_a, dim3((nFusedA_ + 255) / 256), dim3(256), 0, stream_, nFusedA_, aSrc_.p, a_dev, aPerm_.p, flag_.p);
    else flag_.zero(stream_);
    for (int l = 0; l < nLevels_; ++l) {
        const LevelPlan& P = mp_.level[l];
        if (P.small.cnt)
        {
            const int* fd = fdesc_.p + (size_t)P.small.off * FD_STRIDE;
            if (P.smallThreads == 512)
                hipLaunchKernelGGL(k_front_fused<512>, dim3(P.small.cnt), dim3(512), P.smallLds, stream_, fd, inv_.p, aLoc_.p, aPerm_.p, fronts_.p,
                    dinv_.p, flag_.p);
            else
                hipLaunchKernelGGL(k_front_fused<256>, dim3(P.small.cnt), dim3(256), P.smallLds, stream_, fd, inv_.p, aLoc_.p, aPerm_.p, fronts_.p,
                    dinv_.p, flag_.p);
        }
        if (P.ea.cnt) {
            hipLaunchKernelGGL(k_extend_add, dim3(P.ea.cnt), dim3(WG), 0, stream_, eaDesc_.p + P.ea.off, bigFd_.p, inv_.p, fronts_.p, P.fuseEA ? 1 : 0, eaAPtr_.p,
                bigASrc_.p, bigADst_.p, a_dev);
        }
        for (const Range& R : P.step) {
            if (!R.cnt) continue;
            if (P.stepTop) hipLaunchKernelGGL(k_big_step<true>, dim3(R.cnt), dim3(WGB), 0, stream_, desc_.p + R.off, tv, fronts_.p, dinv_.p, flag_.p, xvF);
            else hipLaunchKernelGGL(k_big_step<false>, dim3(R.cnt), dim3(WGB), 0, stream_, desc_.p + R.off, tv, fronts_.p, dinv_.p, flag_.p, xvF);
            const Range& U = P.bulk[&R - P.step.data()];
            if (U.cnt) hipLaunchKernelGGL(k_big_bulk, dim3(U.cnt), dim3(WG), 0, stream_, desc_.p + U.off, fronts_.p);
        }
        if (P.schur.cnt) {
            if (P.fuseEA) hipLaunchKernelGGL(k_big_schur64_ea, dim3(P.schur.cnt), dim3(WG), 0, stream_, desc_.p + P.schur.off, bigFd_.p, inv_.p, fronts_.p);
            else if (P.schur64) hipLaunchKernelGGL(k_big_schur64, dim3(P.schur.cnt), dim3(WG), 0, stream_, desc_.p + P.schur.off, fronts_.p);
            else hipLaunchKernelGGL(k_big_schur, dim3(P.schur.cnt), dim3(WG), 0, stream_, desc_.p + P.schur.off, fronts_.p);
        }
        if (world_ > 1) exchangeUpdateMatrices(l);
        if (mp_.xinvLevel[l].blocks.cnt) {
            if (side_) {
                HIP_CHECK(hipEventRecord(evLevel_[l], stream_));
                HIP_CHECK(hipStreamWaitEvent(side_, evLevel_[l], 0));
                enqueueInverses(l, side_);
                HIP_CHECK(hipEventRecord(evInvDone_[l], side_));
                sideUsed = true;
            }
            else enqueueInverses(l, stream_);
        }
        if (overlapForward) {
            if (l == nLevels_ - 1 && !sideUsed) {
                HIP_CHECK(hipEventRecord(evFwdDone_, fwd_));
                HIP_CHECK(hipStreamWaitEvent(stream_, evFwdDone_, 0));
                enqueueForwardLevel(l, stream_);
                fwdJoined_ = true;
            }
            else if (l >= nLevels_ - 2 || (l + 1) % fwdStride_ == 0) {
                HIP_CHECK(hipEventRecord(evFactLevel_[l], stream_));
                HIP_CHECK(hipStreamWaitEvent(fwd_, evFactLevel_[l], 0));
                for (; fwdNext <= l; ++fwdNext) {
                    if (mp_.level[fwdNext].xinvFwd.cnt && sideUsed) HIP_CHECK(hipStreamWaitEvent(fwd_, evInvDone_[fwdNext], 0));
                    enqueueForwardLevel(fwdNext, fwd_);
                }
            }
        }
    }
    if (sideUsed) HIP_CHECK(hipEventRecord(evSide_, side_));
    sidePending_ = sideUsed;
}

void MfNumeric::enqueueInverses(int l, hipStream_t st)
{
    const XinvLevel& XL = mp_.xinvLevel[l];
    TreeView tv{ frontOff_.p, idxPtr_.p, firstNode_.p, childPtr_.p, child_.p, invPtr_.p, inv_.p, idx_.p, dinvOff_.p };
    XinvView xv{ xinvOff_.p, xinvX_.p, xinvT_.p };
    hipLaunchKernelGGL(k_xinv_init, dim3(XL.init.cnt), dim3(256), 0, st, xinvDesc_.p + XL.init.off, tv, xv, dinv_.p);
    for (const auto& R : XL.rounds) {
        if (R.first.cnt) hipLaunchKernelGGL(k_xinv_gemm, dim3(R.first.cnt), dim3(256), 0, st, xinvDesc_.p + 2 * (size_t)R.first.off, tv, xv, fronts_.p);
        if (R.second.cnt) hipLaunchKernelGGL(k_xinv_gemm, dim3(R.second.cnt), dim3(256), 0, st, xinvDesc_.p + 2 * (size_t)R.second.off, tv, xv, fronts_.p);
    }
}

}
```

### ipc_amd/csrc/mf_sweeps.hip

```cpp
#include "mf_kernels.h"
#include <string>
#include <vector>
#include <algorithm>

#ifndef FWD_NARROW
#define FWD_NARROW 1
#endif
#ifndef BWD_NARROW_MAX_N
#define BWD_NARROW_MAX_N 160
#endif

namespace ipcgpu {

namespace {

__global__ void k_permute_rhs(int nn, const int* __restrict__ newOf, const double* __restrict__ b, double* __restrict__ bp)
{
    int i = blockIdx.x * blockDim.x + threadIdx.x;
    if (i < 3 * nn) {
        int v = i / 3, d = i - 3 * v;
        bp[3 * newOf[v] + d] = b[i];
    }
}
__global__ void k_unpermute_x(int nn, const int* __restrict__ newOf, const double* __restrict__ xp, double* __restrict__ x)
{
    int i = blockIdx.x * blockDim.x + threadIdx.x;
    if (i < 3 * nn) {
        int v = i / 3, d = i - 3 * v;
        x[i] = xp[3 * newOf[v] + d];
    }
}

__device__ __forceinline__ double gather_w(const TreeView& tv, const long long* __restrict__ wOff, const double* __restrict__ wbuf,
    const double* __restrict__ bperm, int s, int nc, int I)
{
    const int cb = tv.childPtr[s], ce = tv.childPtr[s + 1];
    double val = (I < nc) ? bperm[3 * tv.firstNode[s] + I] : 0.0;
    const int In = I / 3, Id = I - 3 * In;
    for (int c0 = cb; c0 < ce; c0 += 4) {
        int ip[4];
        long long base[4];
#pragma unroll
        for (int q = 0; q < 4; ++q) {
            const int c = tv.child[min(c0 + q, ce - 1)];
            ip[q] = tv.invPtr[c];
            base[q] = wOff[c] + frontNc(tv, c) + Id;
        }
        int ic[4];
#pragma unroll
        for (int q = 0; q < 4; ++q) ic[q] = tv.inv[ip[q] + In];
        double v[4];
#pragma unroll
        for (int q = 0; q < 4; ++q) v[q] = wbuf[base[q] + 3 * max(ic[q], 0)];
#pragma unroll
        for (int q = 0; q < 4; ++q)
            if (c0 + q < ce && ic[q] >= 0) val += v[q];
    }
    return val;
}

template <int NT>
__device__ __forceinline__ void fwd_triangle(const double* __restrict__ L, int N, int nc, int rowEnd, const double* __restrict__ dblk,
    double* w1, int tid)
{
    double dn[NB], ln[NB];
    auto fetch = [&](int kb, const double* blk) {
        const int wd = min(NB, nc - kb);
        if (tid < NB) {
#pragma unroll
            for (int c = 0; c < NB; ++c) dn[c] = blk[c * NB + tid];
        }
        const int i = kb + wd + tid;
        if (i < rowEnd) {
#pragma unroll
            for (int k = 0; k < NB; ++k) ln[k] = (k < wd) ? L[i + (long long)N * (kb + k)] : 0.0;
        }
    };
    if (nc > 0) fetch(0, dblk);
    for (int kb = 0; kb < nc; kb += NB, dblk += NB * NB) {
        const int wd = min(NB, nc - kb);
        double y = 0.0;
        if (tid < NB) {
            double p0 = 0.0, p1 = 0.0, p2 = 0.0, p3 = 0.0;
#pragma unroll
            for (int c = 0; c < NB; c += 4) {
                p0 += dn[c] * ((c < wd) ? w1[kb + c] : 0.0);
                p1 += dn[c + 1] * ((c + 1 < wd) ? w1[kb + c + 1] : 0.0);
                p2 += dn[c + 2] * ((c + 2 < wd) ? w1[kb + c + 2] : 0.0);
                p3 += dn[c + 3] * ((c + 3 < wd) ? w1[kb + c + 3] : 0.0);
            }
            y = (p0 + p1) + (p2 + p3);
        }
        __syncthreads();
        if (tid < wd) w1[kb + tid] = y;
        __syncthreads();
        const int i0 = kb + wd + tid;
        double acc0 = 0.0;
        if (i0 < rowEnd) {
            double p0 = 0.0, p1 = 0.0, p2 = 0.0, p3 = 0.0;
#pragma unroll
            for (int k = 0; k < NB; k += 4) {
                p0 += ln[k] * ((k < wd) ? w1[kb + k] : 0.0);
                p1 += ln[k + 1] * ((k + 1 < wd) ? w1[kb + k + 1] : 0.0);
                p2 += ln[k + 2] * ((k + 2 < wd) ? w1[kb + k + 2] : 0.0);
                p3 += ln[k + 3] * ((k + 3 < wd) ? w1[kb + k + 3] : 0.0);
            }
            acc0 = (p0 + p1) + (p2 + p3);
        }
        if (kb + NB < nc) fetch(kb + NB, dblk + NB * NB);
        if (i0 < rowEnd) w1[i0] -= acc0;
        for (int i = i0 + NT; i < rowEnd; i += NT) {
            double acc = 0.0;
#pragma unroll 8
            for (int k = 0; k < wd; ++k) acc += L[i + (long long)N * (kb + k)] * w1[kb + k];
            w1[i] -= acc;
        }
        __syncthreads();
    }
}

template <int NT>
__device__ __forceinline__ void bwd_triangle(const double* __restrict__ L, int N, int nc, const double* __restrict__ dblk0, double* t,
    double* invs , int tid)
{
    const int nblk = (nc + NB - 1) / NB;
    for (int b = nblk - 1; b >= 0; --b) {
        const int kb = b * NB;
        const int wd = min(NB, nc - kb);
        const double* dblk = dblk0 + (long long)b * (NB * NB);
        for (int e = tid; e < NB * NB; e += NT) invs[(e >> 5) * LDP + (e & 31)] = dblk[e];
        __syncthreads();
        double x = 0.0;
        if (tid < NB) {
            double p0 = 0.0, p1 = 0.0, p2 = 0.0, p3 = 0.0;
#pragma unroll
            for (int r = 0; r < NB; r += 4) {
                p0 += invs[tid * LDP + r] * ((r < wd) ? t[kb + r] : 0.0);
                p1 += invs[tid * LDP + r + 1] * ((r + 1 < wd) ? t[kb + r + 1] : 0.0);
                p2 += invs[tid * LDP + r + 2] * ((r + 2 < wd) ? t[kb + r + 2] : 0.0);
                p3 += invs[tid * LDP + r + 3] * ((r + 3 < wd) ? t[kb + r + 3] : 0.0);
            }
            x = (p0 + p1) + (p2 + p3);
        }
        __syncthreads();
        if (tid < wd) t[kb + tid] = x;
        __syncthreads();
        for (int c = tid; c < kb; c += NT) {
            const double* Lc = L + (long long)N * c + kb;
            double p0 = 0.0, p1 = 0.0;
#pragma unroll 8
            for (int k = 0; k + 1 < wd; k += 2) {
                p0 += Lc[k] * t[kb + k];
                p1 += Lc[k + 1] * t[kb + k + 1];
            }
            if (wd & 1) p0 += Lc[wd - 1] * t[kb + wd - 1];
            t[c] -= p0 + p1;
        }
        __syncthreads();
    }
}

template <int NT>
__global__ __launch_bounds__(NT) void k_fwd_level(const int* __restrict__ list, TreeView tv, const long long* __restrict__ wOff,
    const double* __restrict__ fronts, const double* __restrict__ dinv, double* __restrict__ wbuf, const double* __restrict__ bperm,
    double* __restrict__ yperm)
{
    extern __shared__ double w[];
    const int s = list[blockIdx.x];
    const int N = frontN(tv, s), nc = frontNc(tv, s);
    const double* L = fronts + tv.frontOff[s];
    const int tid = threadIdx.x;
    const int col0 = 3 * tv.firstNode[s];
    for (int I = tid; I < N; I += NT) w[I] = gather_w(tv, wOff, wbuf, bperm, s, nc, I);
    __syncthreads();
    fwd_triangle<NT>(L, N, nc, N, dinv + tv.dinvOff[s] * (NB * NB), w, tid);
    double* wo = wbuf + wOff[s];
    for (int I = tid; I < N; I += NT) {
        wo[I] = w[I];
        if (I < nc) yperm[col0 + I] = w[I];
    }
}

// ... 148 lines not shown
    }
    __syncthreads();
    for (int r0 = 0; r0 < m; r0 += 128) {
        const int ra = r0 + lane, rb = r0 + 64 + lane;
        const double xa = (ra < m) ? x2[min(ra, m - 1)] : 0.0, xb = (rb < m) ? x2[min(rb, m - 1)] : 0.0;
        double va[4], vb[4];
#pragma unroll
        for (int q = 0; q < 4; ++q) {
            const double* Lc = L + (long long)N * min(cq[q], nc - 1) + nc;
            va[q] = Lc[min(ra, m - 1)];
            vb[q] = Lc[min(rb, m - 1)];
        }
#pragma unroll
        for (int q = 0; q < 4; ++q) acc[q] += va[q] * xa + vb[q] * xb;
    }
#pragma unroll
    for (int q = 0; q < 4; ++q) {
        double t = acc[q];
#pragma unroll
        for (int off = 32; off > 0; off >>= 1) t += __shfl_down(t, off, 64);
        if (lane == 0 && cq[q] < min(nc, d.y + 16)) yperm[col0 + cq[q]] = yold[q] - t;
    }

}
__global__ __launch_bounds__(WGT) void k_big_bwd_tri(const int* __restrict__ list, TreeView tv, const double* __restrict__ fronts,
    const double* __restrict__ dinv, const double* __restrict__ yperm, double* __restrict__ xsol)
{
    extern __shared__ double t[];
    __shared__ double invs[NB * LDP];
    const int s = list[blockIdx.x];
    const int N = frontN(tv, s), nc = frontNc(tv, s);
    const double* L = fronts + tv.frontOff[s];
    const int tid = threadIdx.x;
    const int col0 = 3 * tv.firstNode[s];
    for (int I = tid; I < nc; I += WGT) t[I] = yperm[col0 + I];
    __syncthreads();
    bwd_triangle<WGT>(L, N, nc, dinv + tv.dinvOff[s] * (NB * NB), t, invs, tid);
    for (int I = tid; I < nc; I += WGT) xsol[col0 + I] = t[I];
}

__global__ __launch_bounds__(WG) void k_xinv_fwd(const int4* __restrict__ desc, TreeView tv, XinvView xv, const long long* __restrict__ wOff,
    const double* __restrict__ wbuf, const double* __restrict__ bperm, double* __restrict__ yperm)
{
    extern __shared__ double w1[];
    __shared__ double part[WG];
    const int4 d = desc[blockIdx.x];
    const int s = d.x, r0 = d.y;
    const int nc = frontNc(tv, s);
    const double* X = xv.X + xv.xOff[s];
    const int tid = threadIdx.x, lane = tid & (MV_ROWS - 1), cg = tid / MV_ROWS;
    constexpr int NCG = WG / MV_ROWS;
    const int cols = min(nc, r0 + MV_ROWS);
    for (int I = tid; I < cols; I += WG) w1[I] = gather_w(tv, wOff, wbuf, bperm, s, nc, I);
    __syncthreads();
    const int r = r0 + lane;
    double acc0 = 0.0, acc1 = 0.0;
    if (r < nc) {
        const int per = (cols + NCG - 1) / NCG, cb = cg * per, ce = min(min(cols, cb + per), r + 1);
        const double* Xr = X + r;
        int c = cb;
        for (; c + 15 < ce; c += 16) {
            double x[16];
#pragma unroll
            for (int u = 0; u < 16; ++u) x[u] = Xr[(long long)nc * (c + u)];
#pragma unroll
            for (int u = 0; u < 16; u += 2) {
                acc0 += x[u] * w1[c + u];
                acc1 += x[u + 1] * w1[c + u + 1];
            }
        }
        for (; c + 3 < ce; c += 4) {
            double x[4];
#pragma unroll
            for (int u = 0; u < 4; ++u) x[u] = Xr[(long long)nc * (c + u)];
#pragma unroll
            for (int u = 0; u < 4; u += 2) {
                acc0 += x[u] * w1[c + u];
                acc1 += x[u + 1] * w1[c + u + 1];
            }
        }
        for (; c < ce; ++c) acc0 += Xr[(long long)nc * c] * w1[c];
    }
    part[tid] = acc0 + acc1;
    __syncthreads();
    if (cg == 0 && r < nc) {
        double tot = 0.0;
#pragma unroll
        for (int g = 0; g < NCG; ++g) tot += part[g * MV_ROWS + lane];
        yperm[3 * tv.firstNode[s] + r] = tot;
    }
}

__global__ __launch_bounds__(WG) void k_xinv_bwd(const int4* __restrict__ desc, TreeView tv, XinvView xv, const double* __restrict__ yperm,
    double* __restrict__ xsol)
{
    extern __shared__ double tt[];
    const int4 d = desc[blockIdx.x];
    const int s = d.x, c0 = d.y;
    const int nc = frontNc(tv, s);
    const double* X = xv.X + xv.xOff[s];
    const int col0 = 3 * tv.firstNode[s];
    const int lane = threadIdx.x & 63, wave = threadIdx.x >> 6;
    for (int r = c0 + threadIdx.x; r < nc; r += WG) tt[r - c0] = yperm[col0 + r];
    __syncthreads();
    int cq[4];
    double acc[4] = { 0.0, 0.0, 0.0, 0.0 };
#pragma unroll
    for (int q = 0; q < 4; ++q) cq[q] = c0 + wave + 4 * q;
    for (int r0 = c0 + wave; r0 < nc; r0 += 128) {
        const int ra = r0 + lane, rb = r0 + 64 + lane;
        const double ta = (ra < nc) ? tt[min(ra, nc - 1) - c0] : 0.0, tb = (rb < nc) ? tt[min(rb, nc - 1) - c0] : 0.0;
        double va[4], vb[4];
#pragma unroll
        for (int q = 0; q < 4; ++q) {
            const double* Xc = X + (long long)nc * min(cq[q], nc - 1);
            va[q] = Xc[min(ra, nc - 1)];
            vb[q] = Xc[min(rb, nc - 1)];
        }
#pragma unroll
        for (int q = 0; q < 4; ++q) acc[q] += ((ra >= cq[q]) ? va[q] * ta : 0.0) + ((rb >= cq[q]) ? vb[q] * tb : 0.0);
    }
#pragma unroll
    for (int q = 0; q < 4; ++q) {
        double t = acc[q];
#pragma unroll
        for (int off = 32; off > 0; off >>= 1) t += __shfl_down(t, off, 64);
        if (lane == 0 && cq[q] < min(nc, c0 + 16)) xsol[col0 + cq[q]] = t;
    }
}

}

void MfNumeric::configureSweepKernels(size_t maxSolveLds, size_t maxBwdLds, size_t maxTriLds)
{
    if (mp_.xinvLds > 48 * 1024) {
        HIP_CHECK(hipFuncSetAttribute((const void*)k_xinv_fwd, hipFuncAttributeMaxDynamicSharedMemorySize, (int)mp_.xinvLds));
        HIP_CHECK(hipFuncSetAttribute((const void*)k_xinv_bwd, hipFuncAttributeMaxDynamicSharedMemorySize, (int)mp_.xinvLds));
    }
    if (maxSolveLds > 48 * 1024) {
        HIP_CHECK(hipFuncSetAttribute((const void*)k_fwd_level<256>, hipFuncAttributeMaxDynamicSharedMemorySize, (int)maxSolveLds));
        HIP_CHECK(hipFuncSetAttribute((const void*)k_fwd_level<128>, hipFuncAttributeMaxDynamicSharedMemorySize, (int)maxSolveLds));
        HIP_CHECK(hipFuncSetAttribute((const void*)k_bwd_level<256>, hipFuncAttributeMaxDynamicSharedMemorySize, (int)maxSolveLds));
        HIP_CHECK(hipFuncSetAttribute((const void*)k_bwd_level<128>, hipFuncAttributeMaxDynamicSharedMemorySize, (int)maxSolveLds));
    }
    if (maxBwdLds > 48 * 1024)
        HIP_CHECK(hipFuncSetAttribute((const void*)k_big_bwd_init, hipFuncAttributeMaxDynamicSharedMemorySize, (int)maxBwdLds));
    if (maxTriLds > 48 * 1024) {
        if (maxTriLds > 150 * 1024) throw StateError("a separator front is too wide for the single-workgroup triangular sweep");
        HIP_CHECK(hipFuncSetAttribute((const void*)k_big_fwd_tri, hipFuncAttributeMaxDynamicSharedMemorySize, (int)maxTriLds));
        HIP_CHECK(hipFuncSetAttribute((const void*)k_big_bwd_tri, hipFuncAttributeMaxDynamicSharedMemorySize, (int)maxTriLds));
    }
}

void MfNumeric::enqueuePermuteRhs(const double* rhs_dev, hipStream_t st)
{
    const int n3 = sym_->n;
    hipLaunchKernelGGL(k_permute_rhs, dim3((n3 + 255) / 256), dim3(256), 0, st, sym_->nn, newOf_.p, rhs_dev, bperm_.p);
}

void MfNumeric::solve(const double* rhs_dev, double* x_dev)
{
    if (!sym_) throw StateError("solve before analyze_pattern");
    enqueueSolve(rhs_dev, x_dev);
}

void MfNumeric::enqueueSolve(const double* rhs_dev, double* x_dev)
{
    enqueuePermuteRhs(rhs_dev, stream_);
    for (int l = 0; l < nLevels_; ++l) {
        const LevelPlan& P = mp_.level[l];
        if (P.xinvFwd.cnt && sidePending_) HIP_CHECK(hipStreamWaitEvent(stream_, evInvDone_[l], 0));
        enqueueForwardLevel(l, stream_);
        if (world_ > 1) exchangeUpdateVectors(l);
    }
    enqueueBackward(x_dev);
}

void MfNumeric::enqueueForwardLevel(int l, hipStream_t st)
{
    TreeView tv{ frontOff_.p, idxPtr_.p, firstNode_.p, childPtr_.p, child_.p, invPtr_.p, inv_.p, idx_.p, dinvOff_.p };
    XinvView xv{ xinvOff_.p, xinvX_.p, xinvT_.p };
    const LevelPlan& P = mp_.level[l];
    if (P.small.cnt)
    {
        if (FWD_NARROW && P.solveLds <= BWD_NARROW_MAX_N * sizeof(double))
            hipLaunchKernelGGL(k_fwd_level<128>, dim3(P.small.cnt), dim3(128), P.solveLds, st, smallList_.p + P.small.off, tv, wOff_.p, fronts_.p, dinv_.p, w_.p,
                bperm_.p, yperm_.p);
        else
            hipLaunchKernelGGL(k_fwd_level<256>, dim3(P.small.cnt), dim3(WG), P.solveLds, st, smallList_.p + P.small.off, tv, wOff_.p, fronts_.p, dinv_.p, w_.p,
                bperm_.p, yperm_.p);
    }
    if (P.bigTri.cnt)
        hipLaunchKernelGGL(k_big_fwd_tri, dim3(P.bigTri.cnt), dim3(WGT), P.triLds, st, triList_.p + P.bigTri.off, tv, wOff_.p, fronts_.p, dinv_.p, w_.p,
            bperm_.p, yperm_.p);
    if (P.xinvFwd.cnt)
        hipLaunchKernelGGL(k_xinv_fwd, dim3(P.xinvFwd.cnt), dim3(WG), mp_.xinvLds, st, xinvDesc_.p + P.xinvFwd.off, tv, xv, wOff_.p, w_.p, bperm_.p, yperm_.p);
    if (P.fwdRect.cnt)
        hipLaunchKernelGGL(k_big_fwd_rect, dim3(P.fwdRect.cnt), dim3(WG), 0, st, desc_.p + P.fwdRect.off, tv, wOff_.p, fronts_.p, w_.p, yperm_.p);
}

void MfNumeric::enqueueBackward(double* x_dev)
{
    const MfSymbolic& sym = *sym_;
    TreeView tv{ frontOff_.p, idxPtr_.p, firstNode_.p, childPtr_.p, child_.p, invPtr_.p, inv_.p, idx_.p, dinvOff_.p };
    XinvView xv{ xinvOff_.p, xinvX_.p, xinvT_.p };
    const int n3 = sym.n;
#ifdef MF_BWD_PROBE
    static int probeCall = 0;
    const bool probe = ++probeCall == 40;
    std::vector<hipEvent_t> pe;
    std::vector<std::string> pn;
    auto mark = [&](const char* what, int l) {
        if (!probe) return;
        hipEvent_t e;
        HIP_CHECK(hipEventCreate(&e));
        HIP_CHECK(hipEventRecord(e, stream_));
        pe.push_back(e);
        pn.push_back(std::string(what) + " L" + std::to_string(l));
    };
    mark("start", nLevels_);
#else
    auto mark = [](const char*, int) {};
#endif
    for (int l = nLevels_ - 1; l >= 0; --l) {
        const LevelPlan& P = mp_.level[l];
        if (P.bwdInit.cnt)
            hipLaunchKernelGGL(k_big_bwd_init, dim3(P.bwdInit.cnt), dim3(WG), P.bwdLds, stream_, desc_.p + P.bwdInit.off, tv, fronts_.p, yperm_.p,
                xsol_.p);
        if (P.bwdInit.cnt) mark("bwd_init", l);
        if (P.bigTri.cnt)
            hipLaunchKernelGGL(k_big_bwd_tri, dim3(P.bigTri.cnt), dim3(WGT), P.triLds, stream_, triList_.p + P.bigTri.off, tv, fronts_.p,
                dinv_.p, yperm_.p, xsol_.p);
        if (P.bigTri.cnt) mark("bwd_tri", l);
        if (P.xinvBwd.cnt)
            hipLaunchKernelGGL(k_xinv_bwd, dim3(P.xinvBwd.cnt), dim3(WG), mp_.xinvLds, stream_, xinvDesc_.p + P.xinvBwd.off, tv, xv, yperm_.p,
                xsol_.p);
        if (P.small.cnt) {
            if (P.solveLds <= BWD_NARROW_MAX_N * sizeof(double))
                hipLaunchKernelGGL(k_bwd_level<128>, dim3(P.small.cnt), dim3(128), P.solveLds, stream_, smallList_.p + P.small.off, tv, fronts_.p, dinv_.p,
                    yperm_.p, xsol_.p);
            else
                hipLaunchKernelGGL(k_bwd_level<256>, dim3(P.small.cnt), dim3(WG), P.solveLds, stream_, smallList_.p + P.small.off, tv, fronts_.p, dinv_.p,
                    yperm_.p, xsol_.p);
        }
        if (P.xinvBwd.cnt || P.small.cnt) mark("xinv/small", l);
        if (world_ > 1) exchange(xchg_[l].opsX);
    }
#ifdef MF_BWD_PROBE
    if (probe) {
        HIP_CHECK(hipStreamSynchronize(stream_));
        for (size_t i = 1; i < pe.size(); ++i) {
            float ms = 0;
            HIP_CHECK(hipEventElapsedTime(&ms, pe[i - 1], pe[i]));
            fprintf(stderr, "bwd probe: %-16s %7.1f us\n", pn[i].c_str(), 1e3 * ms);
        }
    }
#endif
    if (world_ > 1) reduceSolution();
    hipLaunchKernelGGL(k_unpermute_x, dim3((n3 + 255) / 256), dim3(256), 0, stream_, sym.nn, newOf_.p, xsol_.p, x_dev);
}

}
```

### ipc_amd/csrc/nh_kernels.h

```cpp
#pragma once
#include <hip/hip_runtime.h>

namespace ipcgpu {

struct ElemView {
    int nV, nT;
    int tetBegin, tetEnd;
    int energyType;
    const double* x;
    const double* xTilde;
    const double* mass;
    const int* dbc;
    const int4* tet;
    const double* A;
    const double* vol;
    const double* mu;
    const double* lam;
    const int* rowBase;
    const int* rowLen;
    const int* edgeP0;
};

void launch_node_init(const ElemView& v, int projectDBC, bool ownerRank, double* a, double* grad, hipStream_t s);

void launch_assemble(const ElemView& v, double coef, int projectDBC, double* grad ,
    double* a , hipStream_t s);
const char* assemble_kernel_name();

void launch_energy(const ElemView& v, double coef, bool withInertia, bool ownerRank, double* partial, int partialCap,
    double* out, hipStream_t s);
void launch_energy_per_elem(const ElemView& v, double* perElem, hipStream_t s);

void launch_check_inversion(const ElemView& v, int* flag, hipStream_t s);
void launch_inversion_step(const ElemView& v, const double* p, double slackness, double tMax, double* outMin, hipStream_t s);

void launch_step_forward(int n3, const double* x0, const double* p, double alpha, double* x, hipStream_t s);
void launch_trial_step(int n3, const double* x0, const double* p, const double* filterMin, bool useFilter, double* alphaOut, double* x, hipStream_t s);
void launch_max_abs(int n, const double* v, double* out , hipStream_t s);
void launch_trial_step_fused(int n3, double* x, double* x0, const double* p, const double* filterMin, bool useFilter, double* alphaOut, hipStream_t s);
void launch_iter_reset(double* scalar, int* flag, hipStream_t s);
void launch_publish2(const void* a, void* da, int na, const void* b, void* db, int nb, hipStream_t s);
void launch_fill(double* p, size_t n, double v, hipStream_t s);
void launch_negate(int n, const double* in, double* out, hipStream_t s);
void launch_publish(const void* src_dev, void* dst_mapped, int nWords, hipStream_t s);
void launch_colmajor_to_aos(int nV, const double* src, double* dst, hipStream_t s);
void launch_aos_to_colmajor(int nV, const double* src, double* dst, hipStream_t s);
void launch_csr_symv(int nRows, const int* ia, const int* ja, const double* a, const double* x, double* y, hipStream_t s);
void launch_apply_host_updates(long long nnz, const double* delta, const unsigned char* mask, const double* setVal, double* a, hipStream_t s);
void launch_precond_diag(int nRows, const int* ia, const double* a, const double* in, double* out, hipStream_t s);
void launch_be_update(int nV, const int* dbc, const double* x, double* xPrev, double* vel, double* acc, double* dxElastic, double* xTilde,
    double dt, double gx, double gy, double gz, hipStream_t s);
void launch_nm_update(int nV, const int* dbc, const double* x, double* xPrev, double* vel, double* acc, double* dxElastic, double* xTilde,
    double dt, double beta, double gamma, double gx, double gy, double gz, hipStream_t s);
struct DbcMotion {
    double R[9];
    double c[3];
    double linDt[3];
};
void launch_gather3(int n, const int* ids, const double* x, double* out, hipStream_t s);
void launch_target_positions(int n, const int* ids, const double* x, const double* p, double* pos, double* pOut, hipStream_t s);
void launch_dbc_motion(int n, const int* ids, const DbcMotion& m, const double* x, double* p, hipStream_t s);
void launch_dbc_targets(int n, const int* ids, const double* target_3n, const double* x, double* p, hipStream_t s);
void launch_nbc_gradient(int n, const int* ids, const int* dbc, const double* mass, const double* dtSqA3, double* g, hipStream_t s);
void launch_nbc_energy(int n, const int* ids, const int* dbc, const double* mass, const double* x, const double* dtSqA3, double* out, hipStream_t s);
struct MdbcView {
    int n;
    const int* ids;
    const double* pos;
    double* lam;
    const double* mass;
};
void launch_clear_projected(int nV, const int* dbc, int projectDBC, double* g, hipStream_t s);
void launch_keep_mine3(int nV, const unsigned char* mine, double* g, hipStream_t s);
void launch_keep_mine_rows(int nRows, const unsigned char* mine, const int* ia, double* a, hipStream_t s);
void launch_damp_dx(int nV, const int* dbc, int mode, int projectDBC, const double* x, const double* xPrev, double* dx, hipStream_t s);
void launch_damp_clear_diag(int nV, const int* dbc, const int* ia, double* d, hipStream_t s);
void launch_axpy(long long n, double alpha, const double* x, double* y, hipStream_t s);
void launch_dot_scaled(int n, const double* x, const double* y, double scale, double* out, hipStream_t s);
void launch_dot2(int n, const double* g, const double* e, double* partial, int partialCap, double* out2, hipStream_t s);
void launch_mdbc_reduce(const MdbcView& m, const double* x, double rho, int mode , double* out, hipStream_t s);
void launch_mdbc_gradient(const MdbcView& m, const double* x, double rho, double* g, hipStream_t s);
void launch_mdbc_hessian(const MdbcView& m, const int* ia, double rho, double* a, hipStream_t s);
void launch_mdbc_lambda(const MdbcView& m, const double* x, double rho, hipStream_t s);
void launch_warm_dir(int nV, const int* dbc, const double* vel, const double* dx, double dt, const double* cgDtSqG3, double ce, double* p,
    hipStream_t s);
void launch_twist_dir(int nH, const int* ids, const double* ang, double cy, double cz, const double* x, double* p, hipStream_t s);

}
```

### ipc_amd/csrc/nh_kernels.hip

```cpp
#include "nh_device.h"
#include <algorithm>
#include <cfloat>
#include <cstdlib>

namespace ipcgpu {

namespace {

constexpr int BLOCK = 256;

using namespace dev;

struct GlobalAtomicSink {
    const ElemView& v;
    int t;
    int vid[4];
    double* gptr;
    double* a;
    __device__ __forceinline__ void grad(int k, int i, double g) { atomicAdd(&gptr[3 * (size_t)vid[k] + i], g); }
    __device__ __forceinline__ bool wantPair(int, int, int) const { return true; }
    __device__ __forceinline__ void diagBlock(int ka, const double H[3][3])
    {
        const int base = v.rowBase[vid[ka]], Lr = v.rowLen[vid[ka]];
        atomicAdd(&a[base + 0], H[0][0]);
        atomicAdd(&a[base + 1], H[0][1]);
        atomicAdd(&a[base + 2], H[0][2]);
        atomicAdd(&a[base + Lr + 0], H[1][1]);
        atomicAdd(&a[base + Lr + 1], H[1][2]);
        atomicAdd(&a[base + 2 * Lr - 1], H[2][2]);
    }
    __device__ __forceinline__ void offBlock(int e, int ka, int kc, bool aFirst, const double H[3][3])
    {
        const int p0 = v.edgeP0[(size_t)e * v.nT + t];
        const int Lr = v.rowLen[vid[aFirst ? ka : kc]];
#pragma unroll
        for (int r = 0; r < 3; ++r) {
            const int rowOff = (r == 0) ? 0 : (r == 1 ? (Lr - 1) : (2 * Lr - 3));
#pragma unroll
            for (int c = 0; c < 3; ++c) atomicAdd(&a[p0 + rowOff + c], aFirst ? H[r][c] : H[c][r]);
        }
    }
};

template <bool HESS>
__global__ __launch_bounds__(BLOCK) void k_assemble(ElemView v, double coef, int projectDBC, double* __restrict__ grad,
    double* __restrict__ a)
{
    const int t = v.tetBegin + blockIdx.x * BLOCK + threadIdx.x;
    if (t >= v.tetEnd) return;
    const int4 tv = v.tet[t];
    GlobalAtomicSink sink{ v, t, { tv.x, tv.y, tv.z, tv.w }, grad, a };
    assemble_element<HESS>(v, t, coef, projectDBC, grad != nullptr, sink);
}

__global__ __launch_bounds__(BLOCK) void k_node_init(ElemView v, int projectDBC, int owner, double* __restrict__ a,
    double* __restrict__ grad)
{
    const int n = blockIdx.x * BLOCK + threadIdx.x;
    if (n >= v.nV) return;
    const int type = v.dbc[n];
    const bool proj = projected_dbc(type, projectDBC);
    if (grad) {
        double g[3] = { 0, 0, 0 };
        if (!proj && owner) {
            const double m = v.mass[n];
#pragma unroll
            for (int i = 0; i < 3; ++i) g[i] = m * (v.x[3 * (size_t)n + i] - v.xTilde[3 * (size_t)n + i]);
        }
#pragma unroll
        for (int i = 0; i < 3; ++i) grad[3 * (size_t)n + i] = g[i];
    }
    if (a && owner) {
        const int base = v.rowBase[n], Lr = v.rowLen[n];
        const double d = proj ? 1.0 : v.mass[n];
        a[base] = d;
        a[base + Lr] = d;
        a[base + 2 * Lr - 1] = d;
    }
}

__device__ __forceinline__ double block_sum(double x, double* sm)
{
#pragma unroll
    for (int off = 32; off > 0; off >>= 1) x += __shfl_down(x, off, 64);
    const int lane = threadIdx.x & 63, wv = threadIdx.x >> 6;
    if (lane == 0) sm[wv] = x;
    __syncthreads();
    double r = 0.0;
    if (threadIdx.x == 0) {
        for (int i = 0; i < BLOCK / 64; ++i) r += sm[i];
    }
    return r;
}

__device__ __forceinline__ double nh_psi(const double F[9], double mu, double lam)
{
    if (mu == 0.0 && lam == 0.0) return 0.0;
    double I1 = 0.0;
#pragma unroll
    for (int i = 0; i < 9; ++i) I1 += F[i] * F[i];
    const double lJ = log(det3(F));
    return mu / 2.0 * (I1 - 3.0) - (mu - lam / 2.0 * lJ) * lJ;
}

__device__ __forceinline__ double elem_psi(const ElemView& v, const double F[9], double mu, double lam)
{
    if (v.energyType != 1) return nh_psi(F, mu, lam);
    if (mu == 0.0 && lam == 0.0) return 0.0;
    double U[9], s[3], V[9];
    svd3(F, U, s, V);
    return fcr_psi(s, mu, lam);
}

__global__ __launch_bounds__(BLOCK) void k_energy(ElemView v, double coef, int withInertia, int owner, double* __restrict__ partial)
{
    __shared__ double sm[BLOCK / 64];
    const int gid = blockIdx.x * BLOCK + threadIdx.x;
    double e = 0.0;
    const int t = v.tetBegin + gid;
    if (t < v.tetEnd) {
        const int4 tv = v.tet[t];
        double A[9], F[9];
        load_A(v, t, A);
        deformation_gradient(ld3(v.x, tv.x), ld3(v.x, tv.y), ld3(v.x, tv.z), ld3(v.x, tv.w), A, F);
        e = coef * v.vol[t] * elem_psi(v, F, v.mu[t], v.lam[t]);
    }
    if (withInertia && owner && gid < v.nV) {
        double d2 = 0.0;
#pragma unroll
        for (int i = 0; i < 3; ++i) {
            double d = v.x[3 * (size_t)gid + i] - v.xTilde[3 * (size_t)gid + i];
            d2 += d * d;
        }
        e += d2 * v.mass[gid] / 2.0;
    }
    double r = block_sum(e, sm);
    if (threadIdx.x == 0) partial[blockIdx.x] = r;
}

__global__ __launch_bounds__(BLOCK) void k_reduce_partials(const double* __restrict__ partial, int n, double* __restrict__ out)
{
    __shared__ double sm[BLOCK / 64];
    double x = 0.0;
    for (int i = threadIdx.x; i < n; i += BLOCK) x += partial[i];
    double r = block_sum(x, sm);
    if (threadIdx.x == 0) out[0] = r;
}

__global__ __launch_bounds__(BLOCK) void k_energy_per_elem(ElemView v, double* __restrict__ out)
{
    const int t = blockIdx.x * BLOCK + threadIdx.x;
    if (t >= v.nT) return;
    const int4 tv = v.tet[t];
    double A[9], F[9];
    load_A(v, t, A);
    deformation_gradient(ld3(v.x, tv.x), ld3(v.x, tv.y), ld3(v.x, tv.z), ld3(v.x, tv.w), A, F);
    out[t] = v.vol[t] * elem_psi(v, F, v.mu[t], v.lam[t]);
}

__global__ __launch_bounds__(BLOCK) void k_check_inversion(ElemView v, int* flag)
{
    const int t = v.tetBegin + blockIdx.x * BLOCK + threadIdx.x;
    if (t >= v.tetEnd) return;
    if (!(v.mu[t] != 0.0 && v.lam[t] != 0.0)) return;
    const int4 tv = v.tet[t];
    const d3 x0 = ld3(v.x, tv.x), x1 = ld3(v.x, tv.y), x2 = ld3(v.x, tv.z), x3 = ld3(v.x, tv.w);
    const double e[9] = { x1.x - x0.x, x1.y - x0.y, x1.z - x0.z, x2.x - x0.x, x2.y - x0.y, x2.z - x0.z, x3.x - x0.x,
        x3.y - x0.y, x3.z - x0.z };
    if (det3(e) < 0.0) atomicOr(flag, 1);
}

struct cplx {
    double re, im;
};
__device__ __forceinline__ cplx cmul(cplx a, cplx b) { return { a.re * b.re - a.im * b.im, a.re * b.im + a.im * b.re }; }
__device__ __forceinline__ cplx cadd(cplx a, cplx b) { return { a.re + b.re, a.im + b.im }; }
__device__ __forceinline__ cplx csub(cplx a, cplx b) { return { a.re - b.re, a.im - b.im }; }
__device__ __forceinline__ cplx cscale(cplx a, double s) { return { a.re * s, a.im * s }; }
__device__ __forceinline__ cplx cdiv(cplx a, cplx b)
{
    double d = b.re * b.re + b.im * b.im;
    return { (a.re * b.re + a.im * b.im) / d, (a.im * b.re - a.re * b.im) / d };
}
__device__ __forceinline__ double cabs_(cplx a) { return hypot(a.re, a.im); }
__device__ __forceinline__ cplx csqrt_(cplx z)
{
    if (z.re == 0.0 && z.im == 0.0) return { 0.0, 0.0 };
    double m = cabs_(z);
    double t = sqrt(0.5 * (m + fabs(z.re)));
    if (z.re >= 0.0) return { t, z.im / (2.0 * t) };
    return { fabs(z.im) / (2.0 * t), copysign(t, z.im) };
}
__device__ __forceinline__ cplx cpow_third(cplx z)
{
    if (z.re == 0.0 && z.im == 0.0) return { 0.0, 0.0 };
    if (z.im == 0.0 && z.re > 0.0) return { cbrt(z.re), 0.0 };
    double r = cbrt(cabs_(z)), th = atan2(z.im, z.re) / 3.0;
    return { r * cos(th), r * sin(th) };
}
__device__ double quad_root(double a, double b, double c, double tol)
{
    double t;
    if (fabs(a) <= tol) t = -c / b;
    else {
        double desc = b * b - 4 * a * c;
        if (desc > 0) {
            t = (-b - sqrt(desc)) / (2 * a);
            if (t < 0) t = (-b + sqrt(desc)) / (2 * a);
        }
        else t = -1;
    }
    return t;
}
__device__ double cubic_root(double a, double b, double c, double d, double tol)
{
    double t = -1;
    if (fabs(a) <= tol) return quad_root(b, c, d, tol);
    cplx delta0 = { b * b - 3 * a * c, 0 };
    cplx delta1 = { 2 * b * b * b - 9 * a * b * c + 27 * a * a * d, 0 };
    cplx disc = csqrt_(csub(cmul(delta1, delta1), cscale(cmul(cmul(delta0, delta0), delta0), 4.0)));
    cplx C = cpow_third(cscale(cadd(delta1, disc), 0.5));
    if (cabs_(C) == 0.0) C = cpow_third(cscale(csub(delta1, disc), 0.5));
    const double h = sqrt(3.0) / 2.0;
    cplx u2 = { -0.5, h }, u3 = { -0.5, -h };
    cplx bb = { b, 0 };
    double m3a = -3.0 * a;
    cplx t1 = cscale(cadd(cadd(bb, C), cdiv(delta0, C)), 1.0 / m3a);
    cplx u2C = cmul(u2, C), u3C = cmul(u3, C);
    cplx t2 = cscale(cadd(cadd(bb, u2C), cdiv(delta0, u2C)), 1.0 / m3a);
    cplx t3 = cscale(cadd(cadd(bb, u3C), cdiv(delta0, u3C)), 1.0 / m3a);
    if ((fabs(t1.im) < tol) && (t1.re > 0)) t = t1.re;
    if ((fabs(t2.im) < tol) && (t2.re > 0) && ((t2.re < t) || (t < 0))) t = t2.re;
    if ((fabs(t3.im) < tol) && (t3.re > 0) && ((t3.re < t) || (t < 0))) t = t3.re;
    return t;
}

__global__ __launch_bounds__(BLOCK) void k_inversion_step(ElemView v, const double* __restrict__ p, double slackness, double tMax,
    unsigned long long* __restrict__ outMin)
{
    const int t = v.tetBegin + blockIdx.x * BLOCK + threadIdx.x;
    double res = 1e20;
    if (t < v.tetEnd) {
        const int4 tv = v.tet[t];
        const d3 x0 = ld3(v.x, tv.x), x1 = ld3(v.x, tv.y), x2 = ld3(v.x, tv.z), x3 = ld3(v.x, tv.w);
        const d3 p0 = ld3(p, tv.x), p1 = ld3(p, tv.y), p2 = ld3(p, tv.z), p3 = ld3(p, tv.w);
        const double v0[3] = { x1.x - x0.x, x1.y - x0.y, x1.z - x0.z }, v1[3] = { x2.x - x0.x, x2.y - x0.y, x2.z - x0.z },
                     v2[3] = { x3.x - x0.x, x3.y - x0.y, x3.z - x0.z };
        const double q0[3] = { p1.x - p0.x, p1.y - p0.y, p1.z - p0.z }, q1[3] = { p2.x - p0.x, p2.y - p0.y, p2.z - p0.z },
                     q2[3] = { p3.x - p0.x, p3.y - p0.y, p3.z - p0.z };
        auto cross = [](const double* x, const double* y, double* z) {
            z[0] = x[1] * y[2] - x[2] * y[1];
            z[1] = x[2] * y[0] - x[0] * y[2];
            z[2] = x[0] * y[1] - x[1] * y[0];
        };
        auto dot = [](const double* x, const double* y) { return x[0] * y[0] + x[1] * y[1] + x[2] * y[2]; };
        double pxp[3], vxp[3], pxv[3], vxv[3], mix[3];
        cross(q0, q1, pxp);
        cross(v0, q1, vxp);
        cross(q0, v1, pxv);
        cross(v0, v1, vxv);
        for (int c = 0; c < 3; ++c) mix[c] = vxp[c] + pxv[c];
        const double a = dot(q2, pxp);
        const double b = dot(v2, pxp) + dot(q2, mix);
        const double c = dot(q2, vxv) + dot(v2, mix);
        const double d = (1.0 - slackness) * dot(v2, vxv);
        const double lower = d + tMax * (fmin(c, 0.0) + tMax * (fmin(b, 0.0) + tMax * fmin(a, 0.0)));
        if (!(lower > 0.01 * d)) {
            const double r = cubic_root(a, b, c, d, 1.0e-6);
            res = (r >= 0) ? r : 1e20;
        }
    }
#pragma unroll
    for (int off = 32; off > 0; off >>= 1) res = fmin(res, __shfl_down(res, off, 64));
    if ((threadIdx.x & 63) == 0 && res < 1e20) atomicMin(outMin, (unsigned long long)__double_as_longlong(res));
}

__global__ void k_step_forward(int n, const double* __restrict__ x0, const double* __restrict__ p, double alpha, double* __restrict__ x)
{
    int i = blockIdx.x * blockDim.x + threadIdx.x;
    if (i < n) x[i] = x0[i] + alpha * p[i];
}
__global__ void k_trial_alpha(const double* __restrict__ filterMin, int useFilter, double* __restrict__ alphaOut)
{
    double alpha = 1.0;
    const double t = filterMin[0];
    if (useFilter && t > 0.0 && t < alpha) alpha = t;
    alphaOut[0] = alpha;
}
__global__ void k_step_forward_dev(int n, const double* __restrict__ x0, const double* __restrict__ p, const double* __restrict__ alphaPtr,
    double* __restrict__ x)
{
    const double alpha = alphaPtr[0];
    int i = blockIdx.x * blockDim.x + threadIdx.x;
    if (i < n) x[i] = x0[i] + alpha * p[i];
}
__global__ void k_trial_step_fused(int n, double* __restrict__ x, double* __restrict__ x0, const double* __restrict__ p, const double* __restrict__ filterMin,
    int useFilter, double* __restrict__ alphaOut)
{
    double alpha = 1.0;
    const double t = filterMin[0];
    if (useFilter && t > 0.0 && t < alpha) alpha = t;
    const int i = blockIdx.x * blockDim.x + threadIdx.x;
    if (i == 0) alphaOut[0] = alpha;
    if (i < n) {
        const double xi = x[i];
        x0[i] = xi;
        x[i] = xi + alpha * p[i];
    }
}
__global__ void k_iter_reset(double* __restrict__ scalar, int* __restrict__ flag)
{
    scalar[3] = 0.0;
    scalar[2] = 1e20;
    flag[0] = 0;
}
__global__ void k_publish2(const unsigned* __restrict__ a, unsigned* __restrict__ da, int na, const unsigned* __restrict__ b, unsigned* __restrict__ db, int nb)
{
    const int i = threadIdx.x;
    if (i < na) da[i] = a[i];
    if (i < nb) db[i] = b[i];
}
__global__ __launch_bounds__(BLOCK) void k_max_abs(int n, const double* __restrict__ v, unsigned long long* __restrict__ out)
{
    __shared__ double sm[BLOCK / 64];
    double m = 0.0;
    for (int i = blockIdx.x * BLOCK + threadIdx.x; i < n; i += gridDim.x * BLOCK) m = fmax(m, fabs(v[i]));
#pragma unroll
    for (int off = 32; off > 0; off >>= 1) m = fmax(m, __shfl_down(m, off, 64));
    if ((threadIdx.x & 63) == 0) sm[threadIdx.x >> 6] = m;
    __syncthreads();
    if (threadIdx.x == 0) {
        for (int w = 1; w < BLOCK / 64; ++w) m = fmax(m, sm[w]);
        atomicMax(out, (unsigned long long)__double_as_longlong(m));
    }
}
__global__ void k_fill(double* p, size_t n, double v)
{
    size_t i = (size_t)blockIdx.x * blockDim.x + threadIdx.x;
    if (i < n) p[i] = v;
}
__global__ void k_negate(int n, const double* __restrict__ in, double* __restrict__ out)
{
    int i = blockIdx.x * blockDim.x + threadIdx.x;
    if (i < n) out[i] = -in[i];
}
__global__ void k_colmajor_to_aos(int nV, const double* __restrict__ src, double* __restrict__ dst)
{
    int i = blockIdx.x * blockDim.x + threadIdx.x;
    if (i < 3 * nV) {
        int v = i / 3, c = i % 3;
        dst[i] = src[v + (size_t)nV * c];
    }
}
__global__ void k_aos_to_colmajor(int nV, const double* __restrict__ src, double* __restrict__ dst)
{
    int i = blockIdx.x * blockDim.x + threadIdx.x;
    if (i < 3 * nV) {
        int c = i / nV, v = i % nV;
        dst[i] = src[3 * (size_t)v + c];
    }
}
__global__ void k_csr_symv_zero(int n, double* y)
{
    int i = blockIdx.x * blockDim.x + threadIdx.x;
    if (i < n) y[i] = 0.0;
}
__global__ void k_csr_symv(int nRows, const int* __restrict__ ia, const int* __restrict__ ja, const double* __restrict__ a,
    const double* __restrict__ x, double* __restrict__ y)
{
    int r = blockIdx.x * blockDim.x + threadIdx.x;
    if (r >= nRows) return;
    double acc = 0.0;
    const double xr = x[r];
    for (int k = ia[r]; k < ia[r + 1]; ++k) {
        const int c = ja[k];
        acc += a[k] * x[c];
        if (c != r) atomicAdd(&y[c], a[k] * xr);
    }
    atomicAdd(&y[r], acc);
}
__global__ void k_precond_diag(int nRows, const int* __restrict__ ia, const double* __restrict__ a, const double* __restrict__ in,
    double* __restrict__ out)
{
    int r = blockIdx.x * blockDim.x + threadIdx.x;
    if (r < nRows) out[r] = in[r] / a[ia[r]];
}
__global__ void k_nm_update(int nV, const int* __restrict__ dbc, const double* __restrict__ x, double* __restrict__ xPrev,
    double* __restrict__ vel, double* __restrict__ acc, double* __restrict__ dxElastic, double* __restrict__ xTilde, double dt, double beta,
    double gamma, double gx, double gy, double gz)
{
    int i = blockIdx.x * blockDim.x + threadIdx.x;
    if (i >= 3 * nV) return;
    const int v = i / 3, c = i - 3 * v;
    const double g = c == 0 ? gx : (c == 1 ? gy : gz);
    const double dtSq = dt * dt;
    double vl = vel[i] + dt * (1 - gamma) * acc[i];
    const double dx = x[i] - xTilde[i];
    dxElastic[i] = dx;
    double a = dx / (dtSq * beta);
    a += g;
    vl += dt * gamma * a;
    vel[i] = vl;
    acc[i] = a;
    const double xp = x[i];
    xPrev[i] = xp;
    xTilde[i] = dbc[v] != 0 ? xp : xp + (vl * dt + beta * (dtSq * g) + (0.5 - beta) * (dtSq * a));
}
__global__ void k_be_update(int nV, const int* __restrict__ dbc, const double* __restrict__ x, double* __restrict__ xPrev,
    double* __restrict__ vel, double* __restrict__ acc, double* __restrict__ dxElastic, double* __restrict__ xTilde, double dt, double gx,
    double gy, double gz)
{
    int i = blockIdx.x * blockDim.x + threadIdx.x;
    if (i >= 3 * nV) return;
    const int v = i / 3, c = i % 3;
    const double g = (c == 0) ? gx : (c == 1 ? gy : gz);
    const double xi = x[i];
    const double vi = (xi - xPrev[i]) / dt;
    dxElastic[i] = xi - xTilde[i];
    acc[i] = (vi - vel[i]) / dt;
    vel[i] = vi;
    xPrev[i] = xi;
    xTilde[i] = (dbc[v] != 0) ? xi : (xi + (vi * dt + dt * dt * g));
}
__global__ void k_twist_dir(int nH, const int* __restrict__ ids, const double* __restrict__ ang, double cy, double cz,
    const double* __restrict__ x, double* __restrict__ p)
{
    int i = blockIdx.x * blockDim.x + threadIdx.x;
    if (i >= nH) return;
    const int v = ids[i];
    const double cs = cos(ang[i]), sn = sin(ang[i]);
    const double y = x[3 * (size_t)v + 1] - cy, z = x[3 * (size_t)v + 2] - cz;
    p[3 * (size_t)v + 0] = 0.0;
    p[3 * (size_t)v + 1] = (cs * y - sn * z + cy) - x[3 * (size_t)v + 1];
    p[3 * (size_t)v + 2] = (sn * y + cs * z + cz) - x[3 * (size_t)v + 2];
}

__global__ void k_warm_dir(int nV, const int* __restrict__ dbc, const double* __restrict__ vel, const double* __restrict__ dx, double dt,
    double gx, double gy, double gz, double ce, double* __restrict__ p)
{
    const int i = blockIdx.x * blockDim.x + threadIdx.x;
    if (i >= 3 * nV) return;
    const int v = i / 3, c = i - 3 * v;
    const double g = c == 0 ? gx : (c == 1 ? gy : gz);
    p[i] = (dbc[v] != 0) ? 0.0 : dt * vel[i] + g + ce * dx[i];
}

__global__ void k_gather3(int n, const int* __restrict__ ids, const double* __restrict__ x, double* __restrict__ out)
{
    int i = blockIdx.x * blockDim.x + threadIdx.x;
    if (i >= 3 * n) return;
    const int k = i / 3, c = i - 3 * k;
    out[i] = x[3 * (size_t)ids[k] + c];
}
__global__ void k_target_positions(int n, const int* __restrict__ ids, const double* __restrict__ x, const double* __restrict__ p, double* __restrict__ pos,
    double* __restrict__ pOut)
{
    int i = blockIdx.x * blockDim.x + threadIdx.x;
    if (i >= 3 * n) return;
    const int k = i / 3, c = i - 3 * k;
    const size_t j = 3 * (size_t)ids[k] + c;
    const double pi = p[j];
    pOut[i] = pi;
    pos[i] = x[j] + pi;
}
__global__ void k_dbc_motion(int n, const int* __restrict__ ids, DbcMotion m, const double* __restrict__ x, double* __restrict__ p)
{
    int i = blockIdx.x * blockDim.x + threadIdx.x;
    if (i >= n) return;
    const size_t v = (size_t)ids[i];
    const double d0 = x[3 * v] - m.c[0], d1 = x[3 * v + 1] - m.c[1], d2 = x[3 * v + 2] - m.c[2];
#pragma unroll
    for (int c = 0; c < 3; ++c) p[3 * v + c] += (m.R[3 * c] * d0 + m.R[3 * c + 1] * d1 + m.R[3 * c + 2] * d2) + m.c[c] + m.linDt[c] - x[3 * v + c];
}
// ... 55 lines not shown
        const size_t v = (size_t)ids[t];
        double dot = 0.0, sq = 0.0;
#pragma unroll
        for (int c = 0; c < 3; ++c) {
            const double d = x[3 * v + c] - pos[3 * (size_t)t + c];
            dot += lam[3 * (size_t)t + c] * d;
            sq += d * d;
        }
        acc += mode == 0 ? (rho / 2.0 * mass[v] * sq - sqrt(mass[v]) * dot) : sq;
    }
    const double r = block_sum(acc, sm);
    if (threadIdx.x == 0) out[0] = r;
}
__global__ void k_damp_dx(int nV, const int* __restrict__ dbc, int mode, int projectDBC, const double* __restrict__ x, const double* __restrict__ xPrev,
    double* __restrict__ dx)
{
    int i = blockIdx.x * blockDim.x + threadIdx.x;
    if (i >= 3 * nV) return;
    const int t = dbc[i / 3];
    const bool zero = mode == 0 ? t != 0 : projected_dbc(t, projectDBC);
    dx[i] = zero ? 0.0 : x[i] - xPrev[i];
}
__global__ void k_damp_clear_diag(int nV, const int* __restrict__ dbc, const int* __restrict__ ia, double* __restrict__ d)
{
    int i = blockIdx.x * blockDim.x + threadIdx.x;
    if (i < 3 * nV && projected_dbc(dbc[i / 3], 1)) d[ia[i]] = 0.0;
}
__global__ void k_axpy(long long n, double alpha, const double* __restrict__ x, double* __restrict__ y)
{
    long long i = (long long)blockIdx.x * blockDim.x + threadIdx.x;
    if (i < n) y[i] += alpha * x[i];
}
__global__ __launch_bounds__(BLOCK) void k_dot_scaled(int n, const double* __restrict__ x, const double* __restrict__ y, double scale, double* __restrict__ out)
{
    __shared__ double sm[BLOCK / 64];
    double acc = 0.0;
    for (int t = threadIdx.x; t < n; t += BLOCK) acc += x[t] * y[t];
    const double r = block_sum(acc, sm);
    if (threadIdx.x == 0) out[0] = scale * r;
}
__global__ __launch_bounds__(BLOCK) void k_dot2_partial(int n, const double* __restrict__ g, const double* __restrict__ e, double* __restrict__ partial)
{
    __shared__ double sm[BLOCK / 64];
    const int chunk = (n + gridDim.x - 1) / gridDim.x, i0 = blockIdx.x * chunk, i1 = min(n, i0 + chunk);
    double a1 = 0.0, a2 = 0.0;
    for (int i = i0 + threadIdx.x; i < i1; i += BLOCK) {
        const double gi = g[i];
        a1 += gi * e[i];
        a2 += gi * gi;
    }
    const double r1 = block_sum(a1, sm);
    __syncthreads();
    const double r2 = block_sum(a2, sm);
    if (threadIdx.x == 0) {
        partial[blockIdx.x] = r1;
        partial[gridDim.x + blockIdx.x] = r2;
    }
}
__global__ void k_dot2_final(int nb, const double* __restrict__ partial, double* __restrict__ out2)
{
    if (threadIdx.x < 2) {
        double s = 0.0;
        for (int b = 0; b < nb; ++b) s += partial[threadIdx.x * nb + b];
        out2[threadIdx.x] = s;
    }
}
__global__ void k_mdbc_gradient(int n, const int* __restrict__ ids, const double* __restrict__ pos, const double* __restrict__ lam,
    const double* __restrict__ mass, const double* __restrict__ x, double rho, double* __restrict__ g)
{
    int i = blockIdx.x * blockDim.x + threadIdx.x;
    if (i >= 3 * n) return;
    const int t = i / 3, c = i - 3 * t;
    const size_t v = (size_t)ids[t];
    double gi = g[3 * v + c];
    gi -= sqrt(mass[v]) * lam[i];
    gi += rho * mass[v] * (x[3 * v + c] - pos[i]);
    g[3 * v + c] = gi;
}
__global__ void k_mdbc_hessian(int n, const int* __restrict__ ids, const double* __restrict__ mass, const int* __restrict__ ia, double rho,
    double* __restrict__ a)
{
    int i = blockIdx.x * blockDim.x + threadIdx.x;
    if (i >= 3 * n) return;
    const int t = i / 3, c = i - 3 * t;
    const int v = ids[t];
    a[ia[3 * v + c]] += rho * mass[v];
}
__global__ void k_mdbc_lambda(int n, const int* __restrict__ ids, const double* __restrict__ pos, double* __restrict__ lam,
    const double* __restrict__ mass, const double* __restrict__ x, double rho)
{
    int i = blockIdx.x * blockDim.x + threadIdx.x;
    if (i >= 3 * n) return;
    const int t = i / 3, c = i - 3 * t;
    const size_t v = (size_t)ids[t];
    lam[i] -= rho * sqrt(mass[v]) * (x[3 * v + c] - pos[i]);
}

inline int nblk(long long n, int b = BLOCK) { return (int)((n + b - 1) / b); }

}

void launch_node_init(const ElemView& v, int projectDBC, bool ownerRank, double* a, double* grad, hipStream_t s)
{
    if (v.nV) hipLaunchKernelGGL(k_node_init, dim3(nblk(v.nV)), dim3(BLOCK), 0, s, v, projectDBC, ownerRank ? 1 : 0, a, grad);
}

void launch_assemble(const ElemView& v, double coef, int projectDBC, double* grad, double* a, hipStream_t s)
{
    const int n = v.tetEnd - v.tetBegin;
    if (n <= 0) return;
    if (a) hipLaunchKernelGGL(k_assemble<true>, dim3(nblk(n)), dim3(BLOCK), 0, s, v, coef, projectDBC, grad, a);
    else hipLaunchKernelGGL(k_assemble<false>, dim3(nblk(n)), dim3(BLOCK), 0, s, v, coef, projectDBC, grad, a);
}
const char* assemble_kernel_name() { return "k_assemble"; }

void launch_energy(const ElemView& v, double coef, bool withInertia, bool ownerRank, double* partial, int partialCap, double* out,
    hipStream_t s)
{
    const int n = std::max(v.tetEnd - v.tetBegin, withInertia ? v.nV : 0);
    const int nb = std::max(1, nblk(n));
    (void)partialCap;
    hipLaunchKernelGGL(k_energy, dim3(nb), dim3(BLOCK), 0, s, v, coef, withInertia ? 1 : 0, ownerRank ? 1 : 0, partial);
    hipLaunchKernelGGL(k_reduce_partials, dim3(1), dim3(BLOCK), 0, s, partial, nb, out);
}
void launch_energy_per_elem(const ElemView& v, double* perElem, hipStream_t s)
{
    if (v.nT) hipLaunchKernelGGL(k_energy_per_elem, dim3(nblk(v.nT)), dim3(BLOCK), 0, s, v, perElem);
}
void launch_check_inversion(const ElemView& v, int* flag, hipStream_t s)
{
    const int n = v.tetEnd - v.tetBegin;
    if (n > 0) hipLaunchKernelGGL(k_check_inversion, dim3(nblk(n)), dim3(BLOCK), 0, s, v, flag);
}
void launch_inversion_step(const ElemView& v, const double* p, double slackness, double tMax, double* outMin, hipStream_t s)
{
    const int n = v.tetEnd - v.tetBegin;
    if (n > 0)
        hipLaunchKernelGGL(k_inversion_step, dim3(nblk(n)), dim3(BLOCK), 0, s, v, p, slackness, tMax, (unsigned long long*)outMin);
}
void launch_step_forward(int n3, const double* x0, const double* p, double alpha, double* x, hipStream_t s)
{
    if (n3) hipLaunchKernelGGL(k_step_forward, dim3(nblk(n3)), dim3(BLOCK), 0, s, n3, x0, p, alpha, x);
}
void launch_trial_step(int n3, const double* x0, const double* p, const double* filterMin, bool useFilter, double* alphaOut, double* x, hipStream_t s)
{
    hipLaunchKernelGGL(k_trial_alpha, dim3(1), dim3(1), 0, s, filterMin, useFilter ? 1 : 0, alphaOut);
    if (n3) hipLaunchKernelGGL(k_step_forward_dev, dim3(nblk(n3)), dim3(BLOCK), 0, s, n3, x0, p, (const double*)alphaOut, x);
}
void launch_trial_step_fused(int n3, double* x, double* x0, const double* p, const double* filterMin, bool useFilter, double* alphaOut, hipStream_t s)
{
    hipLaunchKernelGGL(k_trial_step_fused, dim3(std::max(nblk(n3), 1)), dim3(BLOCK), 0, s, n3, x, x0, p, filterMin, useFilter ? 1 : 0, alphaOut);
}
void launch_iter_reset(double* scalar, int* flag, hipStream_t s) { hipLaunchKernelGGL(k_iter_reset, dim3(1), dim3(1), 0, s, scalar, flag); }
void launch_publish2(const void* a, void* da, int na, const void* b, void* db, int nb, hipStream_t s)
{
    hipLaunchKernelGGL(k_publish2, dim3(1), dim3(64), 0, s, (const unsigned*)a, (unsigned*)da, na, (const unsigned*)b, (unsigned*)db, nb);
}
void launch_max_abs(int n, const double* v, double* out, hipStream_t s)
{
    if (n) hipLaunchKernelGGL(k_max_abs, dim3(std::min(nblk(n), 256)), dim3(BLOCK), 0, s, n, v, (unsigned long long*)out);
}
void launch_fill(double* p, size_t n, double v, hipStream_t s)
{
    if (n) hipLaunchKernelGGL(k_fill, dim3(nblk((long long)n)), dim3(BLOCK), 0, s, p, n, v);
}
void launch_negate(int n, const double* in, double* out, hipStream_t s)
{
    if (n) hipLaunchKernelGGL(k_negate, dim3(nblk(n)), dim3(BLOCK), 0, s, n, in, out);
}
void launch_colmajor_to_aos(int nV, const double* src, double* dst, hipStream_t s)
{
    if (nV) hipLaunchKernelGGL(k_colmajor_to_aos, dim3(nblk(3LL * nV)), dim3(BLOCK), 0, s, nV, src, dst);
}
void launch_aos_to_colmajor(int nV, const double* src, double* dst, hipStream_t s)
{
    if (nV) hipLaunchKernelGGL(k_aos_to_colmajor, dim3(nblk(3LL * nV)), dim3(BLOCK), 0, s, nV, src, dst);
}
void launch_csr_symv(int nRows, const int* ia, const int* ja, const double* a, const double* x, double* y, hipStream_t s)
{
    if (!nRows) return;
    hipLaunchKernelGGL(k_csr_symv_zero, dim3(nblk(nRows)), dim3(BLOCK), 0, s, nRows, y);
    hipLaunchKernelGGL(k_csr_symv, dim3(nblk(nRows)), dim3(BLOCK), 0, s, nRows, ia, ja, a, x, y);
}
__global__ void k_apply_host_updates(long long nnz, const double* __restrict__ delta, const unsigned char* __restrict__ mask,
    const double* __restrict__ setVal, double* __restrict__ a)
{
    const long long k = (long long)blockIdx.x * blockDim.x + threadIdx.x;
    if (k < nnz) a[k] = (mask && mask[k]) ? setVal[k] + delta[k] : a[k] + delta[k];
}
void launch_apply_host_updates(long long nnz, const double* delta, const unsigned char* mask, const double* setVal, double* a, hipStream_t s)
{
    if (nnz) hipLaunchKernelGGL(k_apply_host_updates, dim3(nblk(nnz)), dim3(BLOCK), 0, s, nnz, delta, mask, setVal, a);
}
void launch_precond_diag(int nRows, const int* ia, const double* a, const double* in, double* out, hipStream_t s)
{
    if (nRows) hipLaunchKernelGGL(k_precond_diag, dim3(nblk(nRows)), dim3(BLOCK), 0, s, nRows, ia, a, in, out);
}
void launch_nm_update(int nV, const int* dbc, const double* x, double* xPrev, double* vel, double* acc, double* dxElastic, double* xTilde,
    double dt, double beta, double gamma, double gx, double gy, double gz, hipStream_t s)
{
    hipLaunchKernelGGL(k_nm_update, dim3((3 * nV + 255) / 256), dim3(256), 0, s, nV, dbc, x, xPrev, vel, acc, dxElastic, xTilde, dt, beta, gamma,
        gx, gy, gz);
}
void launch_be_update(int nV, const int* dbc, const double* x, double* xPrev, double* vel, double* acc, double* dxElastic, double* xTilde,
    double dt, double gx, double gy, double gz, hipStream_t s)
{
    if (nV)
        hipLaunchKernelGGL(k_be_update, dim3(nblk(3LL * nV)), dim3(BLOCK), 0, s, nV, dbc, x, xPrev, vel, acc, dxElastic, xTilde, dt, gx, gy,
            gz);
}
void launch_warm_dir(int nV, const int* dbc, const double* vel, const double* dx, double dt, const double* cgDtSqG3, double ce, double* p,
    hipStream_t s)
{
    if (nV) hipLaunchKernelGGL(k_warm_dir, dim3(nblk(3LL * nV)), dim3(BLOCK), 0, s, nV, dbc, vel, dx, dt, cgDtSqG3[0], cgDtSqG3[1], cgDtSqG3[2], ce, p);
}
void launch_twist_dir(int nH, const int* ids, const double* ang, double cy, double cz, const double* x, double* p, hipStream_t s)
{
    if (nH) hipLaunchKernelGGL(k_twist_dir, dim3(nblk(nH)), dim3(BLOCK), 0, s, nH, ids, ang, cy, cz, x, p);
}

void launch_nbc_gradient(int n, const int* ids, const int* dbc, const double* mass, const double* dtSqA3, double* g, hipStream_t s)
{
    if (n) hipLaunchKernelGGL(k_nbc_gradient, dim3(nblk(n)), dim3(BLOCK), 0, s, n, ids, dbc, mass, dtSqA3[0], dtSqA3[1], dtSqA3[2], g);
}
void launch_nbc_energy(int n, const int* ids, const int* dbc, const double* mass, const double* x, const double* dtSqA3, double* out, hipStream_t s)
{
    hipLaunchKernelGGL(k_nbc_energy, dim3(1), dim3(BLOCK), 0, s, n, ids, dbc, mass, x, dtSqA3[0], dtSqA3[1], dtSqA3[2], out);
}
void launch_damp_dx(int nV, const int* dbc, int mode, int projectDBC, const double* x, const double* xPrev, double* dx, hipStream_t s)
{
    if (nV) hipLaunchKernelGGL(k_damp_dx, dim3(nblk(3LL * nV)), dim3(BLOCK), 0, s, nV, dbc, mode, projectDBC, x, xPrev, dx);
}
void launch_damp_clear_diag(int nV, const int* dbc, const int* ia, double* d, hipStream_t s)
{
    if (nV) hipLaunchKernelGGL(k_damp_clear_diag, dim3(nblk(3LL * nV)), dim3(BLOCK), 0, s, nV, dbc, ia, d);
}
void launch_axpy(long long n, double alpha, const double* x, double* y, hipStream_t s)
{
    if (n) hipLaunchKernelGGL(k_axpy, dim3(nblk(n)), dim3(BLOCK), 0, s, n, alpha, x, y);
}
void launch_dot_scaled(int n, const double* x, const double* y, double scale, double* out, hipStream_t s)
{
    hipLaunchKernelGGL(k_dot_scaled, dim3(1), dim3(BLOCK), 0, s, n, x, y, scale, out);
}
void launch_dot2(int n, const double* g, const double* e, double* partial, int partialCap, double* out2, hipStream_t s)
{
    const int nb = std::max(1, std::min(std::min(128, partialCap / 2), (n + BLOCK - 1) / BLOCK));
    hipLaunchKernelGGL(k_dot2_partial, dim3(nb), dim3(BLOCK), 0, s, n, g, e, partial);
    hipLaunchKernelGGL(k_dot2_final, dim3(1), dim3(64), 0, s, nb, partial, out2);
}
void launch_keep_mine3(int nV, const unsigned char* mine, double* g, hipStream_t s)
{
    if (nV) hipLaunchKernelGGL(k_keep_mine3, dim3(nblk(3LL * nV)), dim3(BLOCK), 0, s, nV, mine, g);
}
void launch_keep_mine_rows(int nRows, const unsigned char* mine, const int* ia, double* a, hipStream_t s)
{
    if (nRows) hipLaunchKernelGGL(k_keep_mine_rows, dim3(nRows), dim3(64), 0, s, nRows, mine, ia, a);
}
void launch_clear_projected(int nV, const int* dbc, int projectDBC, double* g, hipStream_t s)
{
    if (nV) hipLaunchKernelGGL(k_clear_projected, dim3(nblk(3LL * nV)), dim3(BLOCK), 0, s, nV, dbc, projectDBC, g);
}
void launch_mdbc_reduce(const MdbcView& m, const double* x, double rho, int mode, double* out, hipStream_t s)
{
    hipLaunchKernelGGL(k_mdbc_reduce, dim3(1), dim3(BLOCK), 0, s, m.n, m.ids, m.pos, m.lam, m.mass, x, rho, mode, out);
}
void launch_mdbc_gradient(const MdbcView& m, const double* x, double rho, double* g, hipStream_t s)
{
    if (m.n) hipLaunchKernelGGL(k_mdbc_gradient, dim3(nblk(3LL * m.n)), dim3(BLOCK), 0, s, m.n, m.ids, m.pos, m.lam, m.mass, x, rho, g);
}
void launch_mdbc_hessian(const MdbcView& m, const int* ia, double rho, double* a, hipStream_t s)
{
    if (m.n) hipLaunchKernelGGL(k_mdbc_hessian, dim3(nblk(3LL * m.n)), dim3(BLOCK), 0, s, m.n, m.ids, m.mass, ia, rho, a);
}
void launch_mdbc_lambda(const MdbcView& m, const double* x, double rho, hipStream_t s)
{
    if (m.n) hipLaunchKernelGGL(k_mdbc_lambda, dim3(nblk(3LL * m.n)), dim3(BLOCK), 0, s, m.n, m.ids, m.pos, m.lam, m.mass, x, rho);
}
void launch_target_positions(int n, const int* ids, const double* x, const double* p, double* pos, double* pOut, hipStream_t s)
{
    if (n) hipLaunchKernelGGL(k_target_positions, dim3(nblk(3LL * n)), dim3(BLOCK), 0, s, n, ids, x, p, pos, pOut);
}
void launch_gather3(int n, const int* ids, const double* x, double* out, hipStream_t s)
{
    if (n) hipLaunchKernelGGL(k_gather3, dim3(nblk(3LL * n)), dim3(BLOCK), 0, s, n, ids, x, out);
}
void launch_dbc_motion(int n, const int* ids, const DbcMotion& m, const double* x, double* p, hipStream_t s)
{
    if (n) hipLaunchKernelGGL(k_dbc_motion, dim3(nblk(n)), dim3(BLOCK), 0, s, n, ids, m, x, p);
}
void launch_dbc_targets(int n, const int* ids, const double* target, const double* x, double* p, hipStream_t s)
{
    if (n) hipLaunchKernelGGL(k_dbc_targets, dim3(nblk(3LL * n)), dim3(BLOCK), 0, s, n, ids, target, x, p);
}

__global__ void k_publish(const unsigned* __restrict__ src, unsigned* __restrict__ dst, int n)
{
    const int i = threadIdx.x;
    if (i < n) dst[i] = src[i];
}
void launch_publish(const void* src_dev, void* dst_mapped, int nWords, hipStream_t s)
{
    hipLaunchKernelGGL(k_publish, dim3(1), dim3(64), 0, s, (const unsigned*)src_dev, (unsigned*)dst_mapped, nWords);
}

}
```

Measured before the change: 435.2.

## Fuse Newton tail kernels and fold negate, max-abs and pivot flag into solver

Combines the per-iteration tail into fewer launches. Inversion check, step filter and energy now run in one element kernel, and one publish kernel reduces the partial sums, copies scalars and flags to the host and re-arms the reset state for the next iteration. For the multifrontal solver, the gradient negation, the infinity norm of the solution and the pivot flag readback are folded into the solve launches, with the flag check deferred. This cuts kernel launch count and a small amount of memory traffic. In exchange it adds cross-call state (tailArmed) that must stay consistent, which is a correctness risk.

```diff
diff --git a/ipc_amd/csrc/hip_ipc.h b/ipc_amd/csrc/hip_ipc.h
--- a/ipc_amd/csrc/hip_ipc.h
+++ b/ipc_amd/csrc/hip_ipc.h
@@ -69,9 +69,12 @@
     int findEntry(int row, int col) const;
     void analyze_pattern(const HipMesh* meshForCoords);
     bool factorize();
-    bool solve(const double* rhs_dev, double* x_dev);
-    bool factorizeSolve(const double* rhs_dev, double* x_dev, bool wait = true);
+    bool solve(const double* rhs_dev, double* x_dev, double* maxAbsOut = nullptr, double rhsScale = 1.0);
+    bool factorizeSolve(const double* rhs_dev, double* x_dev, bool wait = true, double* maxAbsOut = nullptr, double rhsScale = 1.0, bool deferFlag = false);
     bool lastPivotsOk() const;
+    bool foldsTail() const { return solverType == 0; }
+    const int* pivotFlagDev() const { return num_.pivotFlagDev(); }
+    int* pivotFlagMapped() const { return num_.pivotFlagMapped(); }
     bool lastSyncOk_ = true;
     void multiply(const double* x_dev, double* y_dev);
     void precondition_diag(const double* in_dev, double* out_dev);
@@ -178,7 +181,7 @@
     void getDbcState(double* out4) const;
     void saveStatus(const std::string& path);
     void loadStatus(const std::string& path);
-    DevBuf<double> d_vel, d_xPrev, d_searchDir, d_gradient, d_minusG, d_x0, d_partial, d_scalar;
+    DevBuf<double> d_vel, d_xPrev, d_searchDir, d_gradient, d_minusG, d_x0, d_partial, d_partial2, d_scalar;
     DevBuf<double> d_damp, d_xDamp, d_zeroMass, d_dampDx, d_dampAdx;
     unsigned long long dampPatternVersion = ~0ULL;
     DevBuf<int> d_flag, d_handleIds;
@@ -244,6 +247,9 @@
     bool specAsmValid = false, specAsmOn = true;
     void speculativeAssembly();
     hipEvent_t evAsm0 = nullptr, evAsm1 = nullptr, evTail = nullptr;
+    bool tailArmed = false;
+    void presetScalar(int i, double v);
+    void clearFlags();
     bool evAsmPending = false;
     int evAsmWeight = 1;
     unsigned asmLaunches = 0;
diff --git a/ipc_amd/csrc/hip_linsys.hip b/ipc_amd/csrc/hip_linsys.hip
--- a/ipc_amd/csrc/hip_linsys.hip
+++ b/ipc_amd/csrc/hip_linsys.hip
@@ -304,23 +304,25 @@
     return f == 0;
 }
 
-bool HipLinSysSolver::factorizeSolve(const double* rhs_dev, double* x_dev, bool wait)
+bool HipLinSysSolver::factorizeSolve(const double* rhs_dev, double* x_dev, bool wait, double* maxAbsOut, double rhsScale, bool deferFlag)
 {
     if (!analyzed_) throw StateError("factorize before analyze_pattern");
     lastSyncOk_ = true;
-    if (solverType == 0) return lastSyncOk_ = num_.factorizeSolve(d_a.p, rhs_dev, x_dev, wait);
+    if (solverType == 0) return lastSyncOk_ = num_.factorizeSolve(d_a.p, rhs_dev, x_dev, wait, maxAbsOut, rhsScale, deferFlag);
+    if (maxAbsOut || rhsScale != 1.0 || deferFlag) throw StateError("only the multifrontal solver folds |x|_inf, a scaled right-hand side or a deferred pivot flag into its launches");
     const bool ok = factorize();
     return lastSyncOk_ = ok && solve(rhs_dev, x_dev);
 }
 bool HipLinSysSolver::lastPivotsOk() const { return lastSyncOk_ && (solverType != 0 || num_.lastPivotsOk()); }
 
-bool HipLinSysSolver::solve(const double* rhs_dev, double* x_dev)
+bool HipLinSysSolver::solve(const double* rhs_dev, double* x_dev, double* maxAbsOut, double rhsScale)
 {
     if (!analyzed_) throw StateError("solve before analyze_pattern");
     if (solverType == 0) {
-        num_.solve(rhs_dev, x_dev);
+        num_.solve(rhs_dev, x_dev, maxAbsOut, rhsScale);
         return true;
     }
+    if (maxAbsOut || rhsScale != 1.0) throw StateError("only the multifrontal solver folds |x|_inf or a scaled right-hand side into its launches");
     if (solverType == 2) {
         const bool jacobi = pcgPrecond == 0;
         if (!jacobi && !haveFactor_) throw StateError("solve before factorize");
diff --git a/ipc_amd/csrc/hip_optimizer.cpp b/ipc_amd/csrc/hip_optimizer.cpp
--- a/ipc_amd/csrc/hip_optimizer.cpp
+++ b/ipc_amd/csrc/hip_optimizer.cpp
@@ -78,6 +78,8 @@
     d_minusG.alloc(n3);
     d_x0.alloc(n3);
     d_partial.alloc((size_t)std::max(mesh.nT, mesh.nV) / 256 + 2);
+    d_partial2.alloc(d_partial.n);
+    tailArmed = false;
     d_scalar.alloc(8);
     d_flag.alloc(2);
     h_scalar.alloc(8);
@@ -405,7 +407,7 @@
     if (fric && fricDHat <= fricDHatTarget) {
         computePrecondMtr(true, true);
         computeSearchDir(true);
-        launch_fill(d_scalar.p + 3, 1, 0.0, stream);
+        presetScalar(3, 0.0);
         launch_max_abs(3 * mesh.nV, d_searchDir.p, d_scalar.p + 3, stream);
         if (readScalar(d_scalar.p + 3) < targetGRes) updateFricDHat = false;
         if (fricIterAmt > 0 && fricIterI >= fricIterAmt) updateFricDHat = false;
@@ -988,10 +990,22 @@
     if (!projectDBC && rhoDBC && !tpIds.empty()) launch_mdbc_hessian(mdbc(), lin.d_ia.p, rhoDBC, lin.d_a.p, stream);
 }
 
+void HipOptimizer::presetScalar(int i, double v)
+{
+    tailArmed = false;
+    launch_fill(d_scalar.p + i, 1, v, stream);
+}
+
+void HipOptimizer::clearFlags()
+{
+    tailArmed = false;
+    d_flag.zero(stream);
+}
+
 bool HipOptimizer::checkInversion()
 {
     if (mesh.energyType == 1) return true;
-    d_flag.zero(stream);
+    clearFlags();
     launch_check_inversion(view(), d_flag.p, stream);
     launch_publish(d_flag.p, h_flag.dev, 1, stream);
     HIP_CHECK(hipStreamSynchronize(stream));
@@ -1020,7 +1034,7 @@
 double HipOptimizer::filterStepSize(const double* p_dev, double stepSize)
 {
     if (mesh.energyType == 1) return stepSize;
-    launch_fill(d_scalar.p + 2, 1, 1e20, stream);
+    presetScalar(2, 1e20);
     launch_inversion_step(view(), p_dev, 0.2, stepSize, d_scalar.p + 2, stream);
     reduceMin(d_scalar.p + 2, 1);
     const double t = readScalar(d_scalar.p + 2);
@@ -1062,22 +1076,31 @@
     (void)projectDBC;
     bool ok;
     const bool twoCalls = false;
-    launch_negate(3 * mesh.nV, d_gradient.p, d_minusG.p, stream);
+    bool haveMinusG = false;
+    auto minusG = [&]() {
+        if (!haveMinusG) launch_negate(3 * mesh.nV, d_gradient.p, d_minusG.p, stream);
+        haveMinusG = true;
+        return d_minusG.p;
+    };
     const bool noSpec = false;
     cachedTrialValid = false;
     cachedDistValid = false;
     if (fastPath() && !twoCalls && !noSpec) {
         Tic t(timers[3], stream);
         const size_t bytes = 3 * (size_t)mesh.nV * sizeof(double);
-        if (lin.factorizeSolve(d_minusG.p, d_searchDir.p, false)) {
-            launch_iter_reset(d_scalar.p, d_flag.p, stream);
-            launch_max_abs(3 * mesh.nV, d_searchDir.p, d_scalar.p + 3, stream);
-            if (mesh.energyType != 1) launch_inversion_step(view(), d_searchDir.p, 0.2, 1.0, d_scalar.p + 2, stream);
-            launch_energy(view(), elasticCoef(), true, true, d_partial.p, (int)d_partial.n, d_scalar.p, stream);
-            launch_trial_step_fused(3 * mesh.nV, mesh.d_x.p, d_x0.p, d_searchDir.p, d_scalar.p + 2, mesh.energyType != 1, d_scalar.p + 6, stream);
-            if (mesh.energyType != 1) launch_check_inversion(view(), d_flag.p, stream);
-            launch_energy(view(), elasticCoef(), true, true, d_partial.p, (int)d_partial.n, d_scalar.p + 1, stream);
-            launch_publish2(d_flag.p, h_flag.dev, 1, d_scalar.p, h_scalar.dev, 14, stream);
+        const bool fold = lin.foldsTail();
+        const bool guard = mesh.energyType != 1;
+        if (!tailArmed) launch_iter_reset(d_scalar.p, d_flag.p, stream);
+        tailArmed = false;
+        if (fold ? lin.factorizeSolve(d_gradient.p, d_searchDir.p, false, d_scalar.p + 3, -1.0, true)
+                 : lin.factorizeSolve(minusG(), d_searchDir.p, false)) {
+            if (!fold) launch_max_abs(3 * mesh.nV, d_searchDir.p, d_scalar.p + 3, stream);
+            const int nA = launch_elem_tail(view(), false, guard ? d_searchDir.p : nullptr, true, elasticCoef(), d_scalar.p + 2, nullptr, d_partial.p, stream);
+            launch_trial_step_fused(3 * mesh.nV, mesh.d_x.p, d_x0.p, d_searchDir.p, d_scalar.p + 2, guard, d_scalar.p + 6, stream);
+            const int nB = launch_elem_tail(view(), guard, nullptr, true, elasticCoef(), nullptr, d_flag.p, d_partial2.p, stream);
+            launch_tail_publish(d_partial.p, nA, 0, d_partial2.p, nB, 1, d_scalar.p, h_scalar.dev, d_flag.p, h_flag.dev, 1, fold ? lin.pivotFlagDev() : nullptr,
+                fold ? lin.pivotFlagMapped() : nullptr, stream);
+            tailArmed = true;
             if (!evTail) HIP_CHECK(hipEventCreateWithFlags(&evTail, hipEventDisableTiming));
             HIP_CHECK(hipEventRecord(evTail, stream));
             speculativeAssembly();
@@ -1103,9 +1126,9 @@
         Tic t(timers[3], stream);
         if (twoCalls) ok = lin.factorize();
         else if (worldSize == 1) {
-            ok = lin.factorizeSolve(d_minusG.p, d_searchDir.p, false);
+            ok = lin.factorizeSolve(minusG(), d_searchDir.p, false);
             if (ok) {
-                launch_fill(d_scalar.p + 3, 1, 0.0, stream);
+                presetScalar(3, 0.0);
                 launch_max_abs(3 * mesh.nV, d_searchDir.p, d_scalar.p + 3, stream);
                 launch_publish(d_scalar.p + 3, h_scalar.dev + 3, 2, stream);
                 HIP_CHECK(hipStreamSynchronize(stream));
@@ -1116,18 +1139,18 @@
                 }
             }
         }
-        else ok = lin.factorizeSolve(d_minusG.p, d_searchDir.p);
+        else ok = lin.factorizeSolve(minusG(), d_searchDir.p);
     }
     Tic t(timers[4], stream);
     if (!ok) {
         completeMatrix();
-        lin.precondition_diag(d_minusG.p, d_searchDir.p);
-    }
-    else if (twoCalls) lin.solve(d_minusG.p, d_searchDir.p);
+        lin.precondition_diag(minusG(), d_searchDir.p);
+    }
+    else if (twoCalls) lin.solve(minusG(), d_searchDir.p);
     if (fastPath()) {
-        launch_fill(d_scalar.p + 3, 1, 0.0, stream);
+        presetScalar(3, 0.0);
         launch_max_abs(3 * mesh.nV, d_searchDir.p, d_scalar.p + 3, stream);
-        launch_fill(d_scalar.p + 2, 1, 1e20, stream);
+        presetScalar(2, 1e20);
         if (mesh.energyType != 1) launch_inversion_step(view(), d_searchDir.p, 0.2, 1.0, d_scalar.p + 2, stream);
         launch_energy(view(), elasticCoef(), true, true, d_partial.p, (int)d_partial.n, d_scalar.p, stream);
         launch_publish(d_scalar.p, h_scalar.dev, 8, stream);
@@ -1139,7 +1162,7 @@
     }
     else {
         if (!cachedDistValid) {
-            launch_fill(d_scalar.p + 3, 1, 0.0, stream);
+            presetScalar(3, 0.0);
             launch_max_abs(3 * mesh.nV, d_searchDir.p, d_scalar.p + 3, stream);
             launch_publish(d_scalar.p + 3, h_scalar.dev + 3, 2, stream);
             HIP_CHECK(hipStreamSynchronize(stream));
@@ -1189,7 +1212,7 @@
             stepForward(d_x0.p, stepSize);
             int inverted = 0;
             if (mesh.energyType != 1) {
-                d_flag.zero(stream);
+                clearFlags();
                 launch_check_inversion(view(), d_flag.p, stream);
                 launch_publish(d_flag.p, h_flag.dev, 1, stream);
             }
@@ -1287,20 +1310,22 @@
     const bool batched = BEGIN_BATCHED && fastPath() && nHandles && dbcGroups.empty() && !selfCollision && planes.empty() && !(warmStart >= 1 && warmStart <= 5);
     if (batched) {
         const bool guard = mesh.energyType != 1;
-        d_flag.zero(stream);
-        if (guard) launch_check_inversion(view(), d_flag.p, stream);
+        if (!tailArmed) {
+            clearFlags();
+            presetScalar(2, 1e20);
+        }
+        tailArmed = false;
         d_searchDir.zero(stream);
         stepStartTime = stepEndTime;
         stepEndTime += dt;
         setDBCVertices();
         launch_twist_dir(nHandles, d_handleIds.p, d_handleAng.p, rotCenter[1], rotCenter[2], mesh.d_x.p, d_searchDir.p, stream);
         buildTargetPositions(true);
-        launch_fill(d_scalar.p + 2, 1, 1e20, stream);
-        if (guard) launch_inversion_step(view(), d_searchDir.p, 0.2, 1.0, d_scalar.p + 2, stream);
+        if (guard) launch_elem_tail(view(), true, d_searchDir.p, false, 0.0, d_scalar.p + 2, d_flag.p, nullptr, stream);
         launch_trial_step_fused(3 * mesh.nV, mesh.d_x.p, d_x0.p, d_searchDir.p, d_scalar.p + 2, guard, d_scalar.p + 6, stream);
-        if (guard) launch_check_inversion(view(), d_flag.p + 1, stream);
-        launch_energy(view(), elasticCoef(), true, true, d_partial.p, (int)d_partial.n, d_scalar.p, stream);
-        launch_publish2(d_flag.p, h_flag.dev, 2, d_scalar.p, h_scalar.dev, 14, stream);
+        const int nE = launch_elem_tail(view(), guard, nullptr, true, elasticCoef(), nullptr, d_flag.p + 1, d_partial.p, stream);
+        launch_tail_publish(d_partial.p, nE, 0, nullptr, 0, 0, d_scalar.p, h_scalar.dev, d_flag.p, h_flag.dev, 2, nullptr, nullptr, stream);
+        tailArmed = true;
         HIP_CHECK(hipStreamSynchronize(stream));
         if (h_flag.p[0]) throw StateError("element inversion before scripted motion (Optimizer.cpp:517-522)");
         finishTolerance();
@@ -1469,7 +1494,7 @@
     if (completed > 1.0 - 1.0e-3) projDBC = true;
     else if (completed < lastMove && rhoDBC < 1.0e8) rhoDBC *= 2.0;
     else {
-        launch_fill(d_scalar.p + 3, 1, 0.0, stream);
+        presetScalar(3, 0.0);
         launch_max_abs(3 * mesh.nV, d_searchDir.p, d_scalar.p + 3, stream);
         if (readScalar(d_scalar.p + 3) < CN_MBC) {
             if (completed < 0.99 && rhoDBC < 1.0e8) rhoDBC *= 2.0;
@@ -1483,7 +1508,7 @@
     double distToOpt_PN;
     if (k && cachedDistValid) distToOpt_PN = cachedDist;
     else if (k) {
-        launch_fill(d_scalar.p + 3, 1, 0.0, stream);
+        presetScalar(3, 0.0);
         launch_max_abs(3 * mesh.nV, d_searchDir.p, d_scalar.p + 3, stream);
         distToOpt_PN = readScalar(d_scalar.p + 3);
     }
@@ -1543,7 +1568,7 @@
             if (batchedBounds) {
                 const bool filter = mesh.energyType != 1;
                 if (filter) {
-                    launch_fill(d_scalar.p + 2, 1, 1e20, stream);
+                    presetScalar(2, 1e20);
                     launch_inversion_step(view(), d_searchDir.p, 0.2, alpha, d_scalar.p + 2, stream);
                 }
                 contact->stepBounds(mesh.d_x.p, d_searchDir.p, slackness_m, alpha, filter ? d_scalar.p + 2 : nullptr, &alpha, lastCCDPair, &pMax);
diff --git a/ipc_amd/csrc/mf_numeric.h b/ipc_amd/csrc/mf_numeric.h
--- a/ipc_amd/csrc/mf_numeric.h
+++ b/ipc_amd/csrc/mf_numeric.h
@@ -59,9 +59,12 @@
     void criticalPath(double* out5) const;
     double sharedFlopFraction() const { return mp_.sharedFlops; }
     bool factorize(const double* a_dev);
-    void solve(const double* rhs_dev, double* x_dev);
-    bool factorizeSolve(const double* a_dev, const double* rhs_dev, double* x_dev, bool wait = true);
+    void solve(const double* rhs_dev, double* x_dev, double* maxAbsOut = nullptr, double rhsScale = 1.0);
+    bool factorizeSolve(const double* a_dev, const double* rhs_dev, double* x_dev, bool wait = true, double* maxAbsOut = nullptr, double rhsScale = 1.0,
+        bool deferFlag = false);
     bool lastPivotsOk() const { return pivotsOk(); }
+    const int* pivotFlagDev() const { return flag_.p; }
+    int* pivotFlagMapped() const { return hflag_.dev; }
     bool pivotsOk() const;
     bool ready() const { return ns_ > 0; }
     void entryDestinations(long long* out, size_t nnz) const { entryDst_.download(out, nnz, stream_); }
@@ -69,7 +72,7 @@
 
 private:
     void enqueueFactor(const double* a_dev, bool overlapForward = false);
-    void enqueueSolve(const double* rhs_dev, double* x_dev);
+    void enqueueSolve(const double* rhs_dev, double* x_dev, double* maxAbsOut, double rhsScale);
     typedef MfRange Range;
     typedef MfLevelPlan LevelPlan;
     typedef MfXinvLevel XinvLevel;
@@ -101,7 +104,7 @@
     void reduceSolution();
     void allreduceFlag();
     void configureSweepKernels(size_t maxSolveLds, size_t maxBwdLds, size_t maxTriLds);
-    void enqueuePermuteRhs(const double* rhs_dev, hipStream_t st);
+    void enqueuePermuteRhs(const double* rhs_dev, hipStream_t st, double rhsScale);
     const MfSymbolic* sym_ = nullptr;
     hipStream_t stream_ = nullptr;
     int ns_ = 0, nLevels_ = 0;
@@ -117,7 +120,7 @@
     hipEvent_t evRhs_ = nullptr, evFwdDone_ = nullptr;
     std::vector<hipEvent_t> evFactLevel_;
     void enqueueForwardLevel(int l, hipStream_t st);
-    void enqueueBackward(double* x_dev);
+    void enqueueBackward(double* x_dev, double* maxAbsOut);
     hipEvent_t evSide_ = nullptr;
     std::vector<hipEvent_t> evLevel_, evInvDone_;
     bool sidePending_ = false;
diff --git a/ipc_amd/csrc/mf_numeric.hip b/ipc_amd/csrc/mf_numeric.hip
--- a/ipc_amd/csrc/mf_numeric.hip
+++ b/ipc_amd/csrc/mf_numeric.hip
@@ -1490,23 +1490,23 @@
     return hflag_.p[0] == 0;
 }
 
-bool MfNumeric::factorizeSolve(const double* a_dev, const double* rhs_dev, double* x_dev, bool wait)
+bool MfNumeric::factorizeSolve(const double* a_dev, const double* rhs_dev, double* x_dev, bool wait, double* maxAbsOut, double rhsScale, bool deferFlag)
 {
     if (!sym_) throw StateError("factorize before analyze_pattern");
     if (world_ > 1 || !fwd_) {
         const bool ok = factorize(a_dev);
-        if (ok) solve(rhs_dev, x_dev);
+        if (ok) solve(rhs_dev, x_dev, maxAbsOut, rhsScale);
         return ok;
     }
     HIP_CHECK(hipEventRecord(evRhs_, stream_));
     HIP_CHECK(hipStreamWaitEvent(fwd_, evRhs_, 0));
-    enqueuePermuteRhs(rhs_dev, fwd_);
+    enqueuePermuteRhs(rhs_dev, fwd_, rhsScale);
     fwdJoined_ = false;
     enqueueFactor(a_dev, true);
     if (!fwdJoined_) HIP_CHECK(hipEventRecord(evFwdDone_, fwd_));
-    hipLaunchKernelGGL(k_publish_flag, dim3(1), dim3(1), 0, stream_, flag_.p, hflag_.dev);
+    if (!(deferFlag && !wait)) hipLaunchKernelGGL(k_publish_flag, dim3(1), dim3(1), 0, stream_, flag_.p, hflag_.dev);
     if (!fwdJoined_) HIP_CHECK(hipStreamWaitEvent(stream_, evFwdDone_, 0));
-    enqueueBackward(x_dev);
+    enqueueBackward(x_dev, maxAbsOut);
     if (!wait) return true;
     HIP_CHECK(hipStreamSynchronize(stream_));
     return pivotsOk();
diff --git a/ipc_amd/csrc/mf_sweeps.hip b/ipc_amd/csrc/mf_sweeps.hip
--- a/ipc_amd/csrc/mf_sweeps.hip
+++ b/ipc_amd/csrc/mf_sweeps.hip
@@ -14,20 +14,34 @@
 
 namespace {
 
-__global__ void k_permute_rhs(int nn, const int* __restrict__ newOf, const double* __restrict__ b, double* __restrict__ bp)
+__global__ void k_permute_rhs(int nn, const int* __restrict__ newOf, const double* __restrict__ b, double scale, double* __restrict__ bp)
 {
     int i = blockIdx.x * blockDim.x + threadIdx.x;
     if (i < 3 * nn) {
         int v = i / 3, d = i - 3 * v;
-        bp[3 * newOf[v] + d] = b[i];
-    }
-}
-__global__ void k_unpermute_x(int nn, const int* __restrict__ newOf, const double* __restrict__ xp, double* __restrict__ x)
-{
+        bp[3 * newOf[v] + d] = scale * b[i];
+    }
+}
+__global__ __launch_bounds__(256) void k_unpermute_x(int nn, const int* __restrict__ newOf, const double* __restrict__ xp, double* __restrict__ x,
+    unsigned long long* __restrict__ maxOut)
+{
+    __shared__ double sm[4];
     int i = blockIdx.x * blockDim.x + threadIdx.x;
+    double m = 0.0;
     if (i < 3 * nn) {
         int v = i / 3, d = i - 3 * v;
-        x[i] = xp[3 * newOf[v] + d];
+        const double xi = xp[3 * newOf[v] + d];
+        x[i] = xi;
+        m = fabs(xi);
+    }
+    if (!maxOut) return;
+#pragma unroll
+    for (int off = 32; off > 0; off >>= 1) m = fmax(m, __shfl_down(m, off, 64));
+    if ((threadIdx.x & 63) == 0) sm[threadIdx.x >> 6] = m;
+    __syncthreads();
+    if (threadIdx.x == 0) {
+        for (int w = 1; w < 4; ++w) m = fmax(m, sm[w]);
+        atomicMax(maxOut, (unsigned long long)__double_as_longlong(m));
     }
 }
 
@@ -482,28 +496,28 @@
     }
 }
 
-void MfNumeric::enqueuePermuteRhs(const double* rhs_dev, hipStream_t st)
+void MfNumeric::enqueuePermuteRhs(const double* rhs_dev, hipStream_t st, double rhsScale)
 {
     const int n3 = sym_->n;
-    hipLaunchKernelGGL(k_permute_rhs, dim3((n3 + 255) / 256), dim3(256), 0, st, sym_->nn, newOf_.p, rhs_dev, bperm_.p);
-}
-
-void MfNumeric::solve(const double* rhs_dev, double* x_dev)
+    hipLaunchKernelGGL(k_permute_rhs, dim3((n3 + 255) / 256), dim3(256), 0, st, sym_->nn, newOf_.p, rhs_dev, rhsScale, bperm_.p);
+}
+
+void MfNumeric::solve(const double* rhs_dev, double* x_dev, double* maxAbsOut, double rhsScale)
 {
     if (!sym_) throw StateError("solve before analyze_pattern");
-    enqueueSolve(rhs_dev, x_dev);
-}
-
-void MfNumeric::enqueueSolve(const double* rhs_dev, double* x_dev)
-{
-    enqueuePermuteRhs(rhs_dev, stream_);
+    enqueueSolve(rhs_dev, x_dev, maxAbsOut, rhsScale);
+}
+
+void MfNumeric::enqueueSolve(const double* rhs_dev, double* x_dev, double* maxAbsOut, double rhsScale)
+{
+    enqueuePermuteRhs(rhs_dev, stream_, rhsScale);
     for (int l = 0; l < nLevels_; ++l) {
         const LevelPlan& P = mp_.level[l];
         if (P.xinvFwd.cnt && sidePending_) HIP_CHECK(hipStreamWaitEvent(stream_, evInvDone_[l], 0));
         enqueueForwardLevel(l, stream_);
         if (world_ > 1) exchangeUpdateVectors(l);
     }
-    enqueueBackward(x_dev);
+    enqueueBackward(x_dev, maxAbsOut);
 }
 
 void MfNumeric::enqueueForwardLevel(int l, hipStream_t st)
@@ -529,7 +543,7 @@
         hipLaunchKernelGGL(k_big_fwd_rect, dim3(P.fwdRect.cnt), dim3(WG), 0, st, desc_.p + P.fwdRect.off, tv, wOff_.p, fronts_.p, w_.p, yperm_.p);
 }
 
-void MfNumeric::enqueueBackward(double* x_dev)
+void MfNumeric::enqueueBackward(double* x_dev, double* maxAbsOut)
 {
     const MfSymbolic& sym = *sym_;
     TreeView tv{ frontOff_.p, idxPtr_.p, firstNode_.p, childPtr_.p, child_.p, invPtr_.p, inv_.p, idx_.p, dinvOff_.p };
@@ -587,7 +601,8 @@
     }
 #endif
     if (world_ > 1) reduceSolution();
-    hipLaunchKernelGGL(k_unpermute_x, dim3((n3 + 255) / 256), dim3(256), 0, stream_, sym.nn, newOf_.p, xsol_.p, x_dev);
-}
-
-}
+    hipLaunchKernelGGL(k_unpermute_x, dim3((n3 + 255) / 256), dim3(256), 0, stream_, sym.nn, newOf_.p, xsol_.p, x_dev,
+        (unsigned long long*)maxAbsOut);
+}
+
+}
diff --git a/ipc_amd/csrc/nh_kernels.h b/ipc_amd/csrc/nh_kernels.h
--- a/ipc_amd/csrc/nh_kernels.h
+++ b/ipc_amd/csrc/nh_kernels.h
@@ -39,7 +39,9 @@
 void launch_max_abs(int n, const double* v, double* out , hipStream_t s);
 void launch_trial_step_fused(int n3, double* x, double* x0, const double* p, const double* filterMin, bool useFilter, double* alphaOut, hipStream_t s);
 void launch_iter_reset(double* scalar, int* flag, hipStream_t s);
-void launch_publish2(const void* a, void* da, int na, const void* b, void* db, int nb, hipStream_t s);
+int launch_elem_tail(const ElemView& v, bool check, const double* stepDir, bool energy, double coef, double* outMin, int* flag, double* partial, hipStream_t s);
+void launch_tail_publish(const double* partialA, int nA, int slotA, const double* partialB, int nB, int slotB, double* scalar, double* hscalar, int* flag, int* hflag,
+    int nFlag, const int* pivot, int* hpivot, hipStream_t s);
 void launch_fill(double* p, size_t n, double v, hipStream_t s);
 void launch_negate(int n, const double* in, double* out, hipStream_t s);
 void launch_publish(const void* src_dev, void* dst_mapped, int nWords, hipStream_t s);
diff --git a/ipc_amd/csrc/nh_kernels.hip b/ipc_amd/csrc/nh_kernels.hip
--- a/ipc_amd/csrc/nh_kernels.hip
+++ b/ipc_amd/csrc/nh_kernels.hip
@@ -8,6 +8,7 @@
 namespace {
 
 constexpr int BLOCK = 256;
+enum { TAIL_CHECK = 1, TAIL_STEP = 2, TAIL_ENERGY = 4 };
 
 using namespace dev;
 
@@ -112,6 +113,24 @@
     return fcr_psi(s, mu, lam);
 }
 
+__device__ __forceinline__ double elem_energy(const ElemView& v, int t, const d3& x0, const d3& x1, const d3& x2, const d3& x3, double coef)
+{
+    double A[9], F[9];
+    load_A(v, t, A);
+    deformation_gradient(x0, x1, x2, x3, A, F);
+    return coef * v.vol[t] * elem_psi(v, F, v.mu[t], v.lam[t]);
+}
+__device__ __forceinline__ double node_inertia(const ElemView& v, int n)
+{
+    double d2 = 0.0;
+#pragma unroll
+    for (int i = 0; i < 3; ++i) {
+        double d = v.x[3 * (size_t)n + i] - v.xTilde[3 * (size_t)n + i];
+        d2 += d * d;
+    }
+    return d2 * v.mass[n] / 2.0;
+}
+
 __global__ __launch_bounds__(BLOCK) void k_energy(ElemView v, double coef, int withInertia, int owner, double* __restrict__ partial)
 {
     __shared__ double sm[BLOCK / 64];
@@ -120,20 +139,9 @@
     const int t = v.tetBegin + gid;
     if (t < v.tetEnd) {
         const int4 tv = v.tet[t];
-        double A[9], F[9];
-        load_A(v, t, A);
-        deformation_gradient(ld3(v.x, tv.x), ld3(v.x, tv.y), ld3(v.x, tv.z), ld3(v.x, tv.w), A, F);
-        e = coef * v.vol[t] * elem_psi(v, F, v.mu[t], v.lam[t]);
-    }
-    if (withInertia && owner && gid < v.nV) {
-        double d2 = 0.0;
-#pragma unroll
-        for (int i = 0; i < 3; ++i) {
-            double d = v.x[3 * (size_t)gid + i] - v.xTilde[3 * (size_t)gid + i];
-            d2 += d * d;
-        }
-        e += d2 * v.mass[gid] / 2.0;
-    }
+        e = elem_energy(v, t, ld3(v.x, tv.x), ld3(v.x, tv.y), ld3(v.x, tv.z), ld3(v.x, tv.w), coef);
+    }
+    if (withInertia && owner && gid < v.nV) e += node_inertia(v, gid);
     double r = block_sum(e, sm);
     if (threadIdx.x == 0) partial[blockIdx.x] = r;
 }
@@ -158,16 +166,20 @@
     out[t] = v.vol[t] * elem_psi(v, F, v.mu[t], v.lam[t]);
 }
 
+__device__ __forceinline__ bool elem_inverted(const ElemView& v, int t, const d3& x0, const d3& x1, const d3& x2, const d3& x3)
+{
+    if (!(v.mu[t] != 0.0 && v.lam[t] != 0.0)) return false;
+    const double e[9] = { x1.x - x0.x, x1.y - x0.y, x1.z - x0.z, x2.x - x0.x, x2.y - x0.y, x2.z - x0.z, x3.x - x0.x,
+        x3.y - x0.y, x3.z - x0.z };
+    return det3(e) < 0.0;
+}
+
 __global__ __launch_bounds__(BLOCK) void k_check_inversion(ElemView v, int* flag)
 {
     const int t = v.tetBegin + blockIdx.x * BLOCK + threadIdx.x;
     if (t >= v.tetEnd) return;
-    if (!(v.mu[t] != 0.0 && v.lam[t] != 0.0)) return;
     const int4 tv = v.tet[t];
-    const d3 x0 = ld3(v.x, tv.x), x1 = ld3(v.x, tv.y), x2 = ld3(v.x, tv.z), x3 = ld3(v.x, tv.w);
-    const double e[9] = { x1.x - x0.x, x1.y - x0.y, x1.z - x0.z, x2.x - x0.x, x2.y - x0.y, x2.z - x0.z, x3.x - x0.x,
-        x3.y - x0.y, x3.z - x0.z };
-    if (det3(e) < 0.0) atomicOr(flag, 1);
+    if (elem_inverted(v, t, ld3(v.x, tv.x), ld3(v.x, tv.y), ld3(v.x, tv.z), ld3(v.x, tv.w))) atomicOr(flag, 1);
 }
 
 struct cplx {
@@ -235,6 +247,44 @@
     return t;
 }
 
+__device__ __forceinline__ double elem_inversion_root(const d3& x0, const d3& x1, const d3& x2, const d3& x3, const d3& p0, const d3& p1, const d3& p2,
+    const d3& p3, double slackness, double tMax)
+{
+    const double v0[3] = { x1.x - x0.x, x1.y - x0.y, x1.z - x0.z }, v1[3] = { x2.x - x0.x, x2.y - x0.y, x2.z - x0.z },
+                 v2[3] = { x3.x - x0.x, x3.y - x0.y, x3.z - x0.z };
+    const double q0[3] = { p1.x - p0.x, p1.y - p0.y, p1.z - p0.z }, q1[3] = { p2.x - p0.x, p2.y - p0.y, p2.z - p0.z },
+                 q2[3] = { p3.x - p0.x, p3.y - p0.y, p3.z - p0.z };
+    auto cross = [](const double* x, const double* y, double* z) {
+        z[0] = x[1] * y[2] - x[2] * y[1];
+        z[1] = x[2] * y[0] - x[0] * y[2];
+        z[2] = x[0] * y[1] - x[1] * y[0];
+    };
+    auto dot = [](const double* x, const double* y) { return x[0] * y[0] + x[1] * y[1] + x[2] * y[2]; };
+    double pxp[3], vxp[3], pxv[3], vxv[3], mix[3];
+    cross(q0, q1, pxp);
+    cross(v0, q1, vxp);
+    cross(q0, v1, pxv);
+    cross(v0, v1, vxv);
+    for (int c = 0; c < 3; ++c) mix[c] = vxp[c] + pxv[c];
+    const double a = dot(q2, pxp);
+    const double b = dot(v2, pxp) + dot(q2, mix);
+    const double c = dot(q2, vxv) + dot(v2, mix);
+    const double d = (1.0 - slackness) * dot(v2, vxv);
+    const double lower = d + tMax * (fmin(c, 0.0) + tMax * (fmin(b, 0.0) + tMax * fmin(a, 0.0)));
+    double res = 1e20;
+    if (!(lower > 0.01 * d)) {
+        const double r = cubic_root(a, b, c, d, 1.0e-6);
+        res = (r >= 0) ? r : 1e20;
+    }
+    return res;
+}
+__device__ __forceinline__ void wave_min_to(double res, unsigned long long* __restrict__ outMin)
+{
+#pragma unroll
+    for (int off = 32; off > 0; off >>= 1) res = fmin(res, __shfl_down(res, off, 64));
+    if ((threadIdx.x & 63) == 0 && res < 1e20) atomicMin(outMin, (unsigned long long)__double_as_longlong(res));
+}
+
 __global__ __launch_bounds__(BLOCK) void k_inversion_step(ElemView v, const double* __restrict__ p, double slackness, double tMax,
     unsigned long long* __restrict__ outMin)
 {
@@ -242,37 +292,61 @@
     double res = 1e20;
     if (t < v.tetEnd) {
         const int4 tv = v.tet[t];
+        res = elem_inversion_root(ld3(v.x, tv.x), ld3(v.x, tv.y), ld3(v.x, tv.z), ld3(v.x, tv.w), ld3(p, tv.x), ld3(p, tv.y), ld3(p, tv.z), ld3(p, tv.w),
+            slackness, tMax);
+    }
+    wave_min_to(res, outMin);
+}
+
+__global__ __launch_bounds__(BLOCK) void k_elem_tail(ElemView v, int ops, const double* __restrict__ p, double slackness, double tMax,
+    unsigned long long* __restrict__ outMin, int* __restrict__ flag, double coef, double* __restrict__ partial)
+{
+    __shared__ double sm[BLOCK / 64];
+    const int gid = blockIdx.x * BLOCK + threadIdx.x;
+    const int t = v.tetBegin + gid;
+    double e = 0.0, res = 1e20;
+    if (t < v.tetEnd) {
+        const int4 tv = v.tet[t];
         const d3 x0 = ld3(v.x, tv.x), x1 = ld3(v.x, tv.y), x2 = ld3(v.x, tv.z), x3 = ld3(v.x, tv.w);
-        const d3 p0 = ld3(p, tv.x), p1 = ld3(p, tv.y), p2 = ld3(p, tv.z), p3 = ld3(p, tv.w);
-        const double v0[3] = { x1.x - x0.x, x1.y - x0.y, x1.z - x0.z }, v1[3] = { x2.x - x0.x, x2.y - x0.y, x2.z - x0.z },
-                     v2[3] = { x3.x - x0.x, x3.y - x0.y, x3.z - x0.z };
-        const double q0[3] = { p1.x - p0.x, p1.y - p0.y, p1.z - p0.z }, q1[3] = { p2.x - p0.x, p2.y - p0.y, p2.z - p0.z },
-                     q2[3] = { p3.x - p0.x, p3.y - p0.y, p3.z - p0.z };
-        auto cross = [](const double* x, const double* y, double* z) {
-            z[0] = x[1] * y[2] - x[2] * y[1];
-            z[1] = x[2] * y[0] - x[0] * y[2];
-            z[2] = x[0] * y[1] - x[1] * y[0];
-        };
-        auto dot = [](const double* x, const double* y) { return x[0] * y[0] + x[1] * y[1] + x[2] * y[2]; };
-        double pxp[3], vxp[3], pxv[3], vxv[3], mix[3];
-        cross(q0, q1, pxp);
-        cross(v0, q1, vxp);
-        cross(q0, v1, pxv);
-        cross(v0, v1, vxv);
-        for (int c = 0; c < 3; ++c) mix[c] = vxp[c] + pxv[c];
-        const double a = dot(q2, pxp);
-        const double b = dot(v2, pxp) + dot(q2, mix);
-        const double c = dot(q2, vxv) + dot(v2, mix);
-        const double d = (1.0 - slackness) * dot(v2, vxv);
-        const double lower = d + tMax * (fmin(c, 0.0) + tMax * (fmin(b, 0.0) + tMax * fmin(a, 0.0)));
-        if (!(lower > 0.01 * d)) {
-            const double r = cubic_root(a, b, c, d, 1.0e-6);
-            res = (r >= 0) ? r : 1e20;
-        }
-    }
-#pragma unroll
-    for (int off = 32; off > 0; off >>= 1) res = fmin(res, __shfl_down(res, off, 64));
-    if ((threadIdx.x & 63) == 0 && res < 1e20) atomicMin(outMin, (unsigned long long)__double_as_longlong(res));
+        if ((ops & TAIL_CHECK) && elem_inverted(v, t, x0, x1, x2, x3)) atomicOr(flag, 1);
+        if (ops & TAIL_STEP) res = elem_inversion_root(x0, x1, x2, x3, ld3(p, tv.x), ld3(p, tv.y), ld3(p, tv.z), ld3(p, tv.w), slackness, tMax);
+        if (ops & TAIL_ENERGY) e = elem_energy(v, t, x0, x1, x2, x3, coef);
+    }
+    if (ops & TAIL_STEP) wave_min_to(res, outMin);
+    if (ops & TAIL_ENERGY) {
+        if (gid < v.nV) e += node_inertia(v, gid);
+        double r = block_sum(e, sm);
+        if (threadIdx.x == 0) partial[blockIdx.x] = r;
+    }
+}
+
+__global__ __launch_bounds__(BLOCK) void k_tail_publish(const double* __restrict__ partialA, int nA, int slotA, const double* __restrict__ partialB, int nB, int slotB,
+    double* __restrict__ scalar, double* __restrict__ hscalar, int* __restrict__ flag, int* __restrict__ hflag, int nFlag, const int* __restrict__ pivot,
+    int* __restrict__ hpivot)
+{
+    __shared__ double smA[BLOCK / 64], smB[BLOCK / 64];
+    double ea = 0.0, eb = 0.0;
+    if (nA) {
+        double x = 0.0;
+        for (int i = threadIdx.x; i < nA; i += BLOCK) x += partialA[i];
+        ea = block_sum(x, smA);
+    }
+    if (nB) {
+        double x = 0.0;
+        for (int i = threadIdx.x; i < nB; i += BLOCK) x += partialB[i];
+        eb = block_sum(x, smB);
+    }
+    if (threadIdx.x == 0) {
+        if (nA) scalar[slotA] = ea;
+        if (nB) scalar[slotB] = eb;
+        for (int i = 0; i < 7; ++i) hscalar[i] = scalar[i];
+        for (int i = 0; i < nFlag; ++i) hflag[i] = flag[i];
+        if (pivot) hpivot[0] = pivot[0];
+        scalar[3] = 0.0;
+        scalar[2] = 1e20;
+        flag[0] = 0;
+        flag[1] = 0;
+    }
 }
 
 __global__ void k_step_forward(int n, const double* __restrict__ x0, const double* __restrict__ p, double alpha, double* __restrict__ x)
@@ -313,12 +387,6 @@
     scalar[3] = 0.0;
     scalar[2] = 1e20;
     flag[0] = 0;
-}
-__global__ void k_publish2(const unsigned* __restrict__ a, unsigned* __restrict__ da, int na, const unsigned* __restrict__ b, unsigned* __restrict__ db, int nb)
-{
-    const int i = threadIdx.x;
-    if (i < na) da[i] = a[i];
-    if (i < nb) db[i] = b[i];
 }
 __global__ __launch_bounds__(BLOCK) void k_max_abs(int n, const double* __restrict__ v, unsigned long long* __restrict__ out)
 {
@@ -680,9 +748,18 @@
     hipLaunchKernelGGL(k_trial_step_fused, dim3(std::max(nblk(n3), 1)), dim3(BLOCK), 0, s, n3, x, x0, p, filterMin, useFilter ? 1 : 0, alphaOut);
 }
 void launch_iter_reset(double* scalar, int* flag, hipStream_t s) { hipLaunchKernelGGL(k_iter_reset, dim3(1), dim3(1), 0, s, scalar, flag); }
-void launch_publish2(const void* a, void* da, int na, const void* b, void* db, int nb, hipStream_t s)
-{
-    hipLaunchKernelGGL(k_publish2, dim3(1), dim3(64), 0, s, (const unsigned*)a, (unsigned*)da, na, (const unsigned*)b, (unsigned*)db, nb);
+int launch_elem_tail(const ElemView& v, bool check, const double* stepDir, bool energy, double coef, double* outMin, int* flag, double* partial, hipStream_t s)
+{
+    const int n = std::max(v.tetEnd - v.tetBegin, energy ? v.nV : 0);
+    const int nb = std::max(1, nblk(n));
+    const int ops = (check ? TAIL_CHECK : 0) | (stepDir ? TAIL_STEP : 0) | (energy ? TAIL_ENERGY : 0);
+    if (ops) hipLaunchKernelGGL(k_elem_tail, dim3(nb), dim3(BLOCK), 0, s, v, ops, stepDir, 0.2, 1.0, (unsigned long long*)outMin, flag, coef, partial);
+    return energy ? nb : 0;
+}
+void launch_tail_publish(const double* partialA, int nA, int slotA, const double* partialB, int nB, int slotB, double* scalar, double* hscalar, int* flag, int* hflag,
+    int nFlag, const int* pivot, int* hpivot, hipStream_t s)
+{
+    hipLaunchKernelGGL(k_tail_publish, dim3(1), dim3(BLOCK), 0, s, partialA, nA, slotA, partialB, nB, slotB, scalar, hscalar, flag, hflag, nFlag, pivot, hpivot);
 }
 void launch_max_abs(int n, const double* v, double* out, hipStream_t s)
 {
```

After: 439.2 (median of 4 runs). About the same (+0.9%).
